# gt1/daccord

Hardware: AMD Instinct MI355X
Metric: corrected Mbase/s (whole node), synthetic 20x PacBio piles (higher is better)
Workload: dtype u64+f64; 1 GPU; BASELINE.json configs[1] (10k A-reads x 10 kb x 20x, k=14, one MI355X): synthetic 10000 A-reads x 10000 b x 20x, 15% error (ins 80/del 13.3/sub 6.7), k=14, w=40, a=10, tspace=100; piles_total=10000, piles_rank0=10000, overlaps_rank0=319252, windows_rank0=9969965, trace_blocks_rank0=17906701, corrected_bases_total=90715992

## Files before the change

### daccord_amd/_structs.py

```python
import ctypes as C

U64MAX = 0xFFFFFFFFFFFFFFFF


class DaccParams(C.Structure):
    _fields_ = [
        ("w", C.c_uint32), ("a", C.c_uint32), ("klow", C.c_uint32), ("khigh", C.c_uint32),
        ("minfilterfreq", C.c_int32), ("maxfilterfreq", C.c_int32), ("minwindowcov", C.c_uint32),
        ("maxalign", C.c_uint64), ("eminrate", C.c_uint64), ("minlen", C.c_uint64),
        ("producefull", C.c_int32), ("tspace", C.c_int32), ("device", C.c_int32), ("verbose", C.c_int32),
    ]


class DaccOverlap(C.Structure):
    _fields_ = [
        ("aread", C.c_int32), ("bread", C.c_int32), ("flags", C.c_uint32),
        ("abpos", C.c_int32), ("aepos", C.c_int32), ("bbpos", C.c_int32), ("bepos", C.c_int32),
        ("diffs", C.c_int32), ("tlen", C.c_int32), ("reserved", C.c_uint32), ("trace_off", C.c_uint64),
    ]


class DaccPile(C.Structure):
    _fields_ = [("aread", C.c_int32), ("novl", C.c_uint32), ("first_ovl", C.c_uint64)]


class DaccFragment(C.Structure):
    _fields_ = [("aread", C.c_int32), ("first", C.c_uint32), ("last", C.c_uint32), ("len", C.c_uint32),
                ("seq_off", C.c_uint64)]


class DaccTiming(C.Structure):
    _fields_ = [("h2d_ms", C.c_float), ("trace_ms", C.c_float), ("window_ms", C.c_float), ("vote_ms", C.c_float),
                ("d2h_ms", C.c_float), ("total_ms", C.c_float), ("nwindows", C.c_uint64), ("nblocks", C.c_uint64),
                ("algo_bytes", C.c_uint64), ("tier_ms", C.c_float * 3), ("tier_out", C.c_uint32 * 3),
                ("first_tier", C.c_uint32), ("long_windows", C.c_uint32), ("tier0_ms", C.c_float), ("tier0_in", C.c_uint32),
                ("tier0_out", C.c_uint32), ("tier7_ms", C.c_float), ("tier7_in", C.c_uint32), ("tier7_out", C.c_uint32), ("pad_", C.c_uint32),
                ("long_first_tier", C.c_uint32), ("tier10_ms", C.c_float), ("tier10_out", C.c_uint32), ("tier10_ran", C.c_uint32), ("pad2_", C.c_uint32),
                ("deep_ms", C.c_float), ("deep_windows", C.c_uint32), ("deep_out", C.c_uint32), ("pad3_", C.c_uint32),
                ("last_ms", C.c_float), ("last_windows", C.c_uint32), ("last_out", C.c_uint32), ("pad4_", C.c_uint32),
                ("vdeep_ms", C.c_float), ("vdeep_windows", C.c_uint32), ("vdeep_out", C.c_uint32), ("pad5_", C.c_uint32)]


TIMING_SIZE_V1 = 128


class DaccWindowResult(C.Structure):
    _fields_ = [("pile", C.c_int32), ("y", C.c_int32), ("status", C.c_int32), ("mao", C.c_int32),
                ("elength", C.c_int32), ("k", C.c_int32), ("filterfreq", C.c_int32), ("conslen", C.c_int32),
                ("minrate", C.c_uint64), ("cons", C.c_char * 80)]


def default_params(**kw):
    p = DaccParams(w=40, a=10, klow=8, khigh=8, minfilterfreq=0, maxfilterfreq=2, minwindowcov=3,
                   maxalign=U64MAX, eminrate=U64MAX, minlen=0, producefull=0, tspace=100, device=0, verbose=0)
    for k, v in kw.items():
        if k == "k":
            p.klow = p.khigh = v
        else:
            setattr(p, k, v)
    return p
```

### daccord_amd/csrc/capi.hip

```cpp
#include <hip/hip_runtime.h>
#include <vector>
#include <string>
#include <cstring>
#include <cstdio>
#include <cstdlib>
#include <new>
#include "../../include/daccord_hip.h"
#include "batch_plan.hpp"
#include "host_tables.hpp"
#include "window_kernels.hpp"
#include "trace_kernel.hpp"
#include "vote_kernel.hpp"

using namespace dacc;


struct PrepBatch
{
	DevOvl const * ovl; uint64_t novl; uint8_t const * trace; uint32_t trace_bytes;
	uint32_t * blk_ovl; uint32_t * blk_b0;
};

__global__ void k_prep(PrepBatch B)
{
	uint64_t const o = static_cast<uint64_t>(blockIdx.x)*blockDim.x + threadIdx.x;
	if ( o >= B.novl ) return;
	DevOvl const ov = B.ovl[o];
	uint32_t b = ov.bbpos;
	for ( int32_t i = 0; i < ov.nblk; ++i )
	{
		B.blk_ovl[ov.blk0+i] = o; B.blk_b0[ov.blk0+i] = b;
		b += B.trace_bytes == 2 ? reinterpret_cast<uint16_t const *>(B.trace)[ov.trace_off+2*i+1] : B.trace[ov.trace_off+2*i+1];
	}
}

__global__ void __launch_bounds__(64) k_trace(TraceBatch B)
{
	extern __shared__ __attribute__((aligned(16))) uint8_t lds_trace[];
	TraceStoreGL st;
	st.g = B.slab + static_cast<size_t>(blockIdx.x)*traceSlabWords(B.maxcols);
	st.w = (LDSQ uint32_t *)lds_trace; st.lane = threadIdx.x;
	if ( B.work )
	{
		while ( true )
		{
			uint32_t b = 0;
			if ( threadIdx.x == 0 ) b = atomicAdd(B.work,64u);
			b = __builtin_amdgcn_readfirstlane(b);
			if ( b >= B.nblocks ) break;
			uint64_t const task = static_cast<uint64_t>(b) + threadIdx.x;
			if ( task < B.nblocks ) traceBlock(B,task,st);
		}
		return;
	}
	for ( uint64_t task = static_cast<uint64_t>(blockIdx.x)*64 + threadIdx.x; task < B.nblocks; task += static_cast<uint64_t>(gridDim.x)*64 )
		traceBlock(B,task,st);
}

template<int NW>
__global__ void __launch_bounds__(64) k_trace_wide(TraceBatch B, uint32_t const nl)
{
	extern __shared__ __attribute__((aligned(16))) uint8_t lds_trace[];
	uint32_t const slots = traceSlots(B.maxcols);
	TraceStoreW<NW> st;
	st.w = (LDSQ uint64_t *)lds_trace; st.sc = (LDSQ uint16_t *)(lds_trace + static_cast<size_t>(slots)*(2*NW)*nl*8); st.lane = threadIdx.x; st.nl = nl;
	if ( threadIdx.x < nl )
		for ( uint64_t task = static_cast<uint64_t>(blockIdx.x)*nl + threadIdx.x; task < B.nblocks; task += static_cast<uint64_t>(gridDim.x)*nl )
			traceBlockWide<NW>(B,task,st);
}

static inline uint32_t boundByArena(uint64_t grid, uint64_t const bytes, uint64_t const mingrid)
{
	uint64_t const budget = 32ull << 30;
	while ( grid > mingrid && grid*bytes > budget ) grid >>= 1;
	return static_cast<uint32_t>(grid < 1 ? 1 : grid);
}

__global__ void __launch_bounds__(256) k_prescan(DevOvl const * ovl, uint64_t novl, uint32_t const * ovl_pile, DevPile const * piles, uint32_t const * wt_b, uint32_t const * wt_e,
	uint32_t * pregen, uint32_t * pregen2, uint32_t const thr1)
{
	uint64_t const o = static_cast<uint64_t>(blockIdx.x)*4 + (threadIdx.x>>6);
	if ( o >= novl ) return;
	DevOvl const ov = ovl[o];
	uint64_t const winbase = piles[ovl_pile[o]].winbase;
	for ( uint32_t r = threadIdx.x & 63; r < ov.ny; r += 64 )
	{
		uint32_t const len = wt_e[ov.wtoff+r] - wt_b[ov.wtoff+r];
		if ( len > thr1 )
		{
			uint64_t const w = winbase + ov.y0 + r;
			uint32_t const bit = 1u << (w&31);
			atomicOr(pregen + (w>>5),bit);
			if ( len > 128u ) atomicOr(pregen2 + (w>>5),bit);
		}
	}
}
__global__ void __launch_bounds__(256) k_prescan_lists(uint32_t const * pregen, uint32_t const * pregen2, uint64_t nwindows, uint32_t * list128, uint32_t * slot1list, WindowOut * wout)
{
	uint64_t const wi = static_cast<uint64_t>(blockIdx.x)*256 + threadIdx.x;
	if ( wi*32 >= nwindows ) return;
	uint32_t m = pregen[wi]; uint32_t const m2 = pregen2[wi];
	while ( m )
	{
		uint32_t const b = static_cast<uint32_t>(__builtin_ctz(m)); m &= m-1;
		uint64_t const w = wi*32 + b;
		if ( w >= nwindows ) break;
		wout[w].status = WS_INSUFFICIENT;
		uint32_t * const dst = ((m2 >> b) & 1u) || !slot1list ? list128 : slot1list;
		uint32_t const q = atomicAdd(dst,1u); dst[1+q] = static_cast<uint32_t>(w);
	}
}

__global__ void k_check_done(WindowOut const * wout, uint64_t n, uint32_t * errflag, DevPile const * piles, uint32_t npiles, uint8_t * pilebad)
{
	uint64_t const i = static_cast<uint64_t>(blockIdx.x)*blockDim.x + threadIdx.x;
	if ( i >= n ) return;
	uint32_t const st = wout[i].status;
	if ( st == WS_RETRY ) atomicOr(errflag,1u);
	if ( st == WS_OVERFLOW )
	{
		uint32_t lo = 0, hi = npiles;
		while ( hi-lo > 1 ) { uint32_t const mid = (lo+hi)>>1; if ( piles[mid].winbase <= i ) lo = mid; else hi = mid; }
		pilebad[lo] = 1;
	}
}

__global__ void k_count_deeper(uint32_t const * in, uint32_t const * handon, WindowOut const * wout, uint32_t const mins, uint32_t * out)
{
	uint32_t const nin = in[0], nout = handon[0];
	uint32_t a = 0, b = 0;
	for ( uint32_t i = blockIdx.x*blockDim.x + threadIdx.x; i < nin; i += gridDim.x*blockDim.x ) a += static_cast<uint32_t>(wout[in[1+i]].mao) > mins;
	for ( uint32_t i = blockIdx.x*blockDim.x + threadIdx.x; i < nout; i += gridDim.x*blockDim.x ) b += static_cast<uint32_t>(wout[handon[1+i]].mao) > mins;
	if ( a ) atomicAdd(out,a);
	if ( b ) atomicAdd(out+1,b);
}
__global__ void k_collect_overflow(WindowOut const * wout, uint64_t n, uint32_t * list)
{
	uint64_t const i = static_cast<uint64_t>(blockIdx.x)*blockDim.x + threadIdx.x;
	if ( i < n && wout[i].status == WS_OVERFLOW ) { uint32_t const q = atomicAdd(list,1u); list[1+q] = static_cast<uint32_t>(i); }
}

template<bool MAXOP>
__device__ __forceinline__ uint32_t block_scan_excl(uint32_t const v, uint32_t * part4, uint32_t & total)
{
	uint32_t const wave = threadIdx.x >> 6;
	uint32_t x = v;
	if ( MAXOP ) { DACC_DPP_SCAN(x,DACC_OP_MAX,0u) } else { DACC_DPP_SCAN(x,DACC_OP_ADD,0u) }
	uint32_t excl = __shfl_up(x,1,64); if ( (threadIdx.x & 63) == 0 ) excl = 0;
	__syncthreads();
	if ( (threadIdx.x & 63) == 63 ) part4[wave] = x;
	__syncthreads();
	uint32_t base = 0, tot = 0;
	#pragma unroll
	for ( uint32_t i = 0; i < 4; ++i )
	{
		uint32_t const t = part4[i];
		if ( i < wave ) base = MAXOP ? (t > base ? t : base) : (base + t);
		tot = MAXOP ? (t > tot ? t : tot) : (tot + t);
	}
	total = tot;
	return MAXOP ? (excl > base ? excl : base) : (base + excl);
}

__global__ void __launch_bounds__(256) k_classify(WindowBatch B, uint32_t * small, uint32_t * mid, uint32_t * big, uint32_t const t0inst, uint32_t const t7inst)
{
	__shared__ uint32_t part4[4]; __shared__ uint32_t base3[3];
	uint64_t const w = static_cast<uint64_t>(blockIdx.x)*256 + threadIdx.x;
	uint32_t cls = 3;
	if ( w < B.nwindows && !(B.pregen && ((B.pregen[w>>5] >> (w&31)) & 1)) )
	{
		cls = classifyWindow(B,w,t0inst,t7inst);
		B.wout[w].status = WS_INSUFFICIENT;
	}
	uint32_t tot0, tot1, tot2;
	uint32_t const p0 = block_scan_excl<false>(cls == 0 ? 1u : 0u,part4,tot0);
	__syncthreads();
	uint32_t const p1 = block_scan_excl<false>(cls == 1 ? 1u : 0u,part4,tot1);
	__syncthreads();
	uint32_t const p2 = block_scan_excl<false>(cls == 2 ? 1u : 0u,part4,tot2);
	if ( threadIdx.x == 0 ) { base3[0] = tot0 ? atomicAdd(small,tot0) : 0u; base3[1] = tot1 ? atomicAdd(big,tot1) : 0u; base3[2] = tot2 ? atomicAdd(mid,tot2) : 0u; }
	__syncthreads();
	if ( cls == 0 ) small[1+base3[0]+p0] = static_cast<uint32_t>(w);
	if ( cls == 1 ) big[1+base3[1]+p1] = static_cast<uint32_t>(w);
	if ( cls == 2 ) mid[1+base3[2]+p2] = static_cast<uint32_t>(w);
}


enum { VOTE_STAGE = 48 };
__device__ __forceinline__ VoteTile vote_stage(VoteBatch const & B, DevPile const & pile, uint32_t const p0, uint32_t const np, uint8_t * lds)
{
	VoteTile VT; VT.stage = (LDSQ uint8_t const *)lds; VT.y0 = 0; VT.n = 0;
	uint32_t const a = B.P.a, w = B.P.w, nwin = pile.nwin;
	if ( ! nwin ) return VT;
	uint32_t const plast = (p0+255 < np) ? (p0+255) : (np-1);
	uint32_t const ylo = (p0 > w) ? ((p0-w + a-1)/a) : 0;
	uint32_t yhi = plast / a; if ( yhi > nwin-1 ) yhi = nwin-1;
	__syncthreads();
	if ( ylo <= yhi && yhi-ylo+1 <= VOTE_STAGE && !DACC_WIDE_W(w) )
	{
		VT.y0 = ylo; VT.n = yhi-ylo+1;
		uint4 const * src = reinterpret_cast<uint4 const *>(B.wrec + (pile.winbase+ylo)*WREC);
		uint4 * dst = reinterpret_cast<uint4 *>(lds);
		for ( uint32_t i = threadIdx.x; i < VT.n*(WREC/16); i += 256 ) dst[i] = src[i];
	}
	__syncthreads();
	return VT;
}
__global__ void __launch_bounds__(256) k_vote(VoteBatch B)
{
	__shared__ uint32_t part4[4];
	__shared__ __attribute__((aligned(16))) uint8_t stage[VOTE_STAGE*WREC];
	uint32_t const pi = blockIdx.x;
	DevPile const pile = B.piles[pi];
	uint32_t const np = pileNpos(pile);
	uint32_t const tid = threadIdx.x;
	if ( B.pilebad && B.pilebad[pi] ) { if ( tid == 0 ) B.nfrag[pi] = 0; return; }
	for ( uint32_t t0 = 0; t0 < np; t0 += 256 )
	{
		VoteTile const VT = vote_stage(B,pile,t0,np,stage);
		if ( t0+tid < np ) votePass1(B,pile,t0+tid,VT);
	}
	__syncthreads();
	uint32_t run0 = 0;
	for ( uint32_t t0 = 0; t0 < np; t0 += 256 )
	{
		VoteTile const VT = vote_stage(B,pile,t0,np,stage);
		uint32_t const p = t0+tid;
		uint32_t const n = p < np ? votePass2(B,pile,p,0,VT) : 0u;
		uint32_t tot; uint32_t const ex = block_scan_excl<false>(n,part4,tot);
		if ( p < np ) { B.oc[pile.posbase+p] = n; B.ocs[pile.posbase+p] = run0 + ex; }
		run0 += tot;
	}
	uint32_t const total = run0;
	bool const fits = total <= 2*np+64;
	if ( !fits && tid == 0 ) atomicOr(B.errflag,2u);
	uint64_t const symbase = 2*pile.posbase + 64ull*pi;
	if ( fits )
		for ( uint32_t t0 = 0; t0 < np; t0 += 256 )
		{
			VoteTile const VT = vote_stage(B,pile,t0,np,stage);
			uint32_t const p = t0+tid;
			if ( p < np ) votePass2(B,pile,p,B.outsym+symbase+B.ocs[pile.posbase+p],VT);
		}
	__syncthreads();
	uint32_t const chunk = (np + 255)/256;
	uint32_t const p0 = tid*chunk < np ? tid*chunk : np, p1 = (p0+chunk < np) ? (p0+chunk) : np;
	uint8_t const * has = B.has + pile.posbase;
	uint32_t laststart = 0; bool open = false;
	for ( uint32_t p = p0; p < p1; ++p )
		if ( has[p] && (p == 0 || !has[p-1]) ) laststart = p+1;
	uint32_t dummy;
	uint32_t const instart = block_scan_excl<true>(laststart,part4,dummy);
	(void)open;
	uint32_t cur = instart;
	uint32_t nfr = 0;
	for ( int pass = 0; pass < 2; ++pass )
	{
		uint32_t fbase = 0, ftot = 0;
		if ( pass == 1 ) { fbase = block_scan_excl<false>(nfr,part4,ftot); if ( tid == 0 ) B.nfrag[pi] = fits ? ftot : 0; if ( !fits ) break; }
		cur = instart; uint32_t k = 0;
		VoteFragment * F = B.frags + B.fragbase[pi];
		for ( uint32_t p = p0; p < p1; ++p )
		{
			if ( ! has[p] ) continue;
			if ( p == 0 || !has[p-1] ) cur = p+1;
			if ( p+1 == np || !has[p+1] )
			{
				uint32_t const first = cur-1, q = p;
				if ( q-first >= 100 )
				{
					uint32_t const so = B.ocs[pile.posbase+first];
					uint32_t const eo = B.ocs[pile.posbase+q] + B.oc[pile.posbase+q];
					uint32_t const len = eo-so;
					if ( B.P.producefull || len >= B.P.minlen )
					{
						if ( pass == 1 ) { VoteFragment & f = F[fbase+k]; f.first = first; f.last = q; f.len = len; f.pad = 0; f.off = symbase + so; }
						++k;
					}
				}
			}
		}
		nfr = k;
	}
}


namespace {

template<typename T>
struct DevBuf
{
	T * p; size_t cap;
	DevBuf() : p(0), cap(0) {}
	hipError_t ensure(size_t n)
	{
		if ( n <= cap ) return hipSuccess;
		if ( p ) { hipFree(p); p = 0; cap = 0; }
		hipError_t const e = hipMalloc(reinterpret_cast<void **>(&p),n*sizeof(T));
		if ( e == hipSuccess ) cap = n;
		return e;
	}
	void release() { if ( p ) hipFree(p); p = 0; cap = 0; }
};

template<typename T>
struct HostBuf
{
	T * p; size_t cap; bool pinned;
	HostBuf() : p(0), cap(0), pinned(false) {}
	hipError_t ensure(size_t n)
	{
		if ( n <= cap ) return hipSuccess;
		release();
		hipError_t e = hipHostMalloc(reinterpret_cast<void **>(&p),n*sizeof(T),hipHostMallocDefault);
		if ( e == hipSuccess ) { cap = n; pinned = true; return e; }
		(void)hipGetLastError();
		p = static_cast<T *>(std::malloc(n*sizeof(T)));
		if ( !p ) return hipErrorOutOfMemory;
		cap = n; pinned = false;
		return hipSuccess;
	}
	void release() { if ( p ) { if ( pinned ) hipHostFree(p); else std::free(p); } p = 0; cap = 0; pinned = false; }
};

}

struct dacc_ctx
{
	dacc_params par;
	int device;
	hipStream_t stream; hipStream_t stream2; hipEvent_t evFirstTier, evEarlyGeneric, evPrescan;
	hipEvent_t ev[6]; hipEvent_t evslot[TIER_NSLOTS];
	std::string err;
	bool haveprofile, havedb, havebatch;
	double est_cor;
	HostTables H;
	DevTables T; DevParams P;
	DevBuf<double> d_dpnorm, d_dpsq; DevBuf<uint64_t> d_vs; DevBuf<uint16_t> d_first, d_size, d_suplo, d_suphi; DevBuf<uint32_t> d_klim;
	DevBuf<uint8_t> d_bps; DevBuf<uint64_t> d_boff; DevBuf<uint32_t> d_rlen;
	std::vector<uint32_t> h_rlen;
	BatchPlan BP;
	DevBuf<DevPile> d_piles; DevBuf<DevOvl> d_ovl; DevBuf<uint32_t> d_ovl_pile; DevBuf<uint8_t> d_trace;
	DevBuf<uint32_t> d_blk_ovl, d_blk_b0, d_wt_b, d_wt_e;
	DevBuf<uint8_t> d_wrec; DevBuf<WindowOut> d_wout; DevBuf<uint8_t> d_arena;
	DevBuf<uint8_t> d_has, d_oc, d_outsym, d_pilebad; DevBuf<uint16_t> d_ld0; DevBuf<uint32_t> d_ocs, d_nfrag, d_err;
	DevBuf<VoteFragment> d_frags; DevBuf<uint64_t> d_fragbase; DevBuf<uint64_t> d_prof;
	DevBuf<uint64_t> d_vst; DevBuf<uint32_t> d_tab32; DevBuf<uint8_t> d_gslab, d_lastslab , d_vdeepslab ; DevBuf<uint32_t> d_retry[TIER_NSLOTS], d_work, d_gearly, d_pregen, d_pregen2, d_pregenlist; DevBuf<uint8_t> d_arena2; DevBuf<uint64_t> d_trslab; DevBuf<uint32_t> d_small; DevBuf<uint64_t> d_hand; DevBuf<uint32_t> d_handctr; uint32_t handcap; uint64_t handwant, nruns; bool nohand, oom; bool tier7_adapt_off; int env_t7adapt; int env_trdyn;
	TierSwitches sw; TierPipeline TP;
	struct Stage { bool ran; uint32_t grid; DevBuf<uint32_t> handon; hipEvent_t done; uint32_t const * in;  } st[TIER_NSTAGES];
	uint32_t nlong[2];
	uint32_t retry_grid, early_grid; int sched;
	uint32_t tr_grid, tr_lds, tr_words, tr_lanes, trace_bytes, win_grid;
	int env_sched, env_dbgretry;
	std::vector<uint32_t> retry_flags;
	std::vector<dacc_fragment> frags; std::string bases;
	std::vector<int32_t> pile_status; std::vector<std::string> pile_errors; std::string pile_errors_joined;
	std::vector<uint32_t> h_nfrag; std::vector<VoteFragment> h_frags; HostBuf<uint8_t> h_outsym;
	dacc_timing timing;
};

#define HIPCHK(call) do { hipError_t const e_ = (call); if ( e_ != hipSuccess ) { c->err = std::string(#call) + ": " + hipGetErrorString(e_); if ( e_ == hipErrorOutOfMemory ) c->oom = true; return DACC_EHIP; } } while (0)

template<typename T>
static int upload(dacc_ctx * c, DevBuf<T> & b, T const * src, size_t n)
{
	HIPCHK(b.ensure(n ? n : 1));
	if ( n ) HIPCHK(hipMemcpyAsync(b.p,src,n*sizeof(T),hipMemcpyHostToDevice,c->stream));
	return DACC_OK;
}

template<typename F> static int guarded(dacc_ctx * c, F const & f)
{
	try { return f(); }
	catch ( std::bad_alloc const & ) { if ( c ) { try { c->err = "out of host memory"; } catch ( ... ) {} } return DACC_ENOMEM; }
	catch ( std::exception const & ex ) { if ( c ) { try { c->err = std::string("host side failed: ") + ex.what(); } catch ( ... ) {} } return DACC_EINTERNAL; }
	catch ( ... ) { if ( c ) { try { c->err = "host side failed: unknown exception"; } catch ( ... ) {} } return DACC_EINTERNAL; }
}

extern "C" {

int dacc_device_count(void)
{
	int ndev = 0;
	if ( hipGetDeviceCount(&ndev) != hipSuccess || ndev < 0 ) return 0;
	return ndev;
}

int dacc_create(dacc_ctx ** out, dacc_params const * p)
{
	if ( !out || !p ) return DACC_EINVAL;
	*out = 0;
	if ( p->klow < 3 || p->khigh > 16 || p->klow > p->khigh || !p->w || !p->a || p->w > DACC_WMAX || p->minfilterfreq < 0 ||
	     p->maxfilterfreq < p->minfilterfreq || p->tspace <= 0 || p->tspace > 512 )
		return DACC_EINVAL;
	if ( readTierSwitches().conflict() ) return DACC_EINVAL;
	int ndev = 0;
	if ( hipGetDeviceCount(&ndev) != hipSuccess || ndev <= 0 || p->device < 0 || p->device >= ndev )
		return DACC_ENODEV;
	if ( hipSetDevice(p->device) != hipSuccess ) return DACC_ENODEV;
	dacc_ctx * c = new (std::nothrow) dacc_ctx;
	if ( !c ) return DACC_ENOMEM;
	c->par = *p; c->device = p->device; c->haveprofile = c->havedb = c->havebatch = false; c->est_cor = 0; c->nlong[0] = c->nlong[1] = 0; c->handcap = 0; c->handwant = 0; c->nruns = 0; c->nohand = false; c->oom = false;
	std::memset(&c->timing,0,sizeof(c->timing));
	c->retry_grid = c->early_grid = c->win_grid = 0; c->tier7_adapt_off = false; c->sched = 0;
	c->tr_grid = c->tr_lds = c->tr_words = c->tr_lanes = c->trace_bytes = 0;
	{
		c->sw = readTierSwitches();
		char const * sc = getenv("DACC_SCHED"); c->env_sched = sc ? atoi(sc) : 1;
		{ char const * td = getenv("DACC_TRACE_DYN"); c->env_trdyn = !(td && td[0] == '0'); }
		char const * ta = getenv("DACC_T7_ADAPT"); c->env_t7adapt = !(ta && ta[0] == '0');
		char const * dr = getenv("DACC_DEBUG_RETRY"); c->env_dbgretry = (dr && dr[0] == '1');
	}
	if ( hipStreamCreate(&c->stream) != hipSuccess ) { delete c; return DACC_EHIP; }
	{ int lo = 0, hi = 0; hipDeviceGetStreamPriorityRange(&lo,&hi); if ( hipStreamCreateWithPriority(&c->stream2,hipStreamNonBlocking,hi) != hipSuccess ) { delete c; return DACC_EHIP; } }
	hipEventCreateWithFlags(&c->evFirstTier,hipEventDisableTiming); hipEventCreateWithFlags(&c->evEarlyGeneric,hipEventDisableTiming); hipEventCreateWithFlags(&c->evPrescan,hipEventDisableTiming);
	for ( int i = 0; i < 6; ++i ) hipEventCreate(&c->ev[i]);
	for ( int i = 0; i < TIER_NSLOTS; ++i ) hipEventCreate(&c->evslot[i]);
	for ( int i = 0; i < TIER_NSTAGES; ++i ) { hipEventCreate(&c->st[i].done); c->st[i].ran = false; c->st[i].grid = 0; c->st[i].in = 0; }
	*out = c;
	return DACC_OK;
}

void dacc_destroy(dacc_ctx * c)
{
	if ( !c ) return;
	hipSetDevice(c->device);
	hipStreamSynchronize(c->stream); hipStreamSynchronize(c->stream2);
	c->d_dpnorm.release(); c->d_dpsq.release(); c->d_vs.release(); c->d_first.release(); c->d_size.release(); c->d_suplo.release(); c->d_suphi.release(); c->d_klim.release();
	c->d_bps.release(); c->d_boff.release(); c->d_rlen.release();
	c->d_piles.release(); c->d_ovl.release(); c->d_ovl_pile.release(); c->d_trace.release(); c->d_blk_ovl.release(); c->d_blk_b0.release(); c->d_wt_b.release(); c->d_wt_e.release();
	c->d_wrec.release(); c->d_wout.release(); c->d_arena.release();
	c->h_outsym.release(); c->d_pilebad.release(); c->d_has.release(); c->d_oc.release(); c->d_outsym.release(); c->d_ld0.release(); c->d_ocs.release(); c->d_nfrag.release(); c->d_err.release(); c->d_frags.release(); c->d_fragbase.release(); c->d_prof.release(); c->d_vst.release(); c->d_tab32.release(); c->d_gslab.release(); c->d_lastslab.release(); c->d_vdeepslab.release(); for ( int i = 0; i < 3; ++i ) c->d_retry[i].release(); c->d_work.release(); c->d_gearly.release(); c->d_pregen.release(); c->d_pregen2.release(); c->d_pregenlist.release(); c->d_arena2.release(); c->d_trslab.release(); c->d_hand.release(); c->d_handctr.release();
	for ( int i = 0; i < 6; ++i ) hipEventDestroy(c->ev[i]);
	hipStreamDestroy(c->stream); hipStreamDestroy(c->stream2); hipEventDestroy(c->evFirstTier); hipEventDestroy(c->evEarlyGeneric); hipEventDestroy(c->evPrescan); for ( int i = 0; i < TIER_NSLOTS; ++i ) hipEventDestroy(c->evslot[i]);
	c->d_small.release(); for ( int i = 0; i < TIER_NSTAGES; ++i ) { hipEventDestroy(c->st[i].done); c->st[i].handon.release(); }
	delete c;
}

char const * dacc_last_error(dacc_ctx * c) { return c ? c->err.c_str() : "null context"; }

static int dacc_set_error_profile_body(dacc_ctx * c, double p_i, double p_d, double est_cor)
{
	if ( !c ) return DACC_EINVAL;
	if ( !(p_i >= 0 && p_i < 1 && p_d >= 0 && p_d < 1 && est_cor >= 0 && est_cor <= 1) ) { c->err = "error profile out of range"; return DACC_EINVAL; }
	hipSetDevice(c->device);
	buildHostTables(c->H,c->par.w,p_i,p_d,est_cor,c->par.klow,c->par.khigh,4200);
	c->est_cor = est_cor;
	int rc;
	if ( (rc = upload(c,c->d_dpnorm,c->H.dpnorm.data(),c->H.dpnorm.size())) ) return rc;
	if ( (rc = upload(c,c->d_dpsq,c->H.dpsq.data(),c->H.dpsq.size())) ) return rc;
	if ( (rc = upload(c,c->d_vs,c->H.dpsq_vs.data(),c->H.dpsq_vs.size())) ) return rc;
	if ( (rc = upload(c,c->d_vst,c->H.dpsq_vst.data(),c->H.dpsq_vst.size())) ) return rc;
	if ( (rc = upload(c,c->d_tab32,c->H.tab32.data(),c->H.tab32.size())) ) return rc;
	if ( (rc = upload(c,c->d_first,c->H.dpsq_first.data(),c->H.dpsq_first.size())) ) return rc;
	if ( (rc = upload(c,c->d_size,c->H.dpsq_size.data(),c->H.dpsq_size.size())) ) return rc;
	if ( (rc = upload(c,c->d_suplo,c->H.suplo.data(),c->H.suplo.size())) ) return rc;
	if ( (rc = upload(c,c->d_suphi,c->H.suphi.data(),c->H.suphi.size())) ) return rc;
	if ( (rc = upload(c,c->d_klim,c->H.klim.data(),c->H.klim.size())) ) return rc;
	HIPCHK(hipStreamSynchronize(c->stream));
	DevTables & T = c->T;
	T.nrows = c->H.nrows; T.nsup = c->H.nsup; T.kln = c->H.kln; T.pad = 0;
	T.dpnorm = c->d_dpnorm.p; T.dpsq = c->d_dpsq.p; T.dpsq_vs = c->d_vs.p; T.dpsq_first = c->d_first.p; T.dpsq_size = c->d_size.p;
	T.suplo = c->d_suplo.p; T.suphi = c->d_suphi.p; T.klim = c->d_klim.p;
	dacc_params const & p = c->par;
	DevParams & P = c->P;
	P.w = p.w; P.a = p.a; P.klow = p.klow; P.khigh = p.khigh; P.minff = p.minfilterfreq; P.maxff = p.maxfilterfreq;
	P.minwindowcov = p.minwindowcov; P.checklim = (est_cor != 0.0); P.maxalign = p.maxalign; P.eminrate = p.eminrate;
	P.tspace = p.tspace; P.producefull = p.producefull; P.minlen = p.minlen;
	c->haveprofile = true;
	return DACC_OK;
}

int dacc_debug_tables(dacc_ctx * c, uint64_t * out, uint64_t cap, uint64_t * n, uint64_t klimit_n)
{
	if ( !c || !n ) return DACC_EINVAL;
	if ( !c->haveprofile ) return DACC_ESTATE;
	std::vector<uint64_t> B; serialiseHostTables(c->H,B,klimit_n);
	*n = B.size();
	if ( out ) std::memcpy(out,B.data(),8*std::min<uint64_t>(cap,B.size()));
	return DACC_OK;
}

static int dacc_load_db_body(dacc_ctx * c, uint8_t const * bps, uint64_t bps_bytes, uint64_t const * boff, uint32_t const * rlen, uint64_t nreads)
{
	if ( !c || !bps || !boff || !rlen || !nreads ) return DACC_EINVAL;
	hipSetDevice(c->device);
	for ( uint64_t i = 0; i < nreads; ++i )
		if ( boff[i] + (rlen[i]+3)/4 > bps_bytes ) { c->err = "read store offsets exceed the buffer"; return DACC_EINVAL; }
	int rc;
	HIPCHK(c->d_bps.ensure(bps_bytes+16));
	HIPCHK(hipMemsetAsync(c->d_bps.p,0,bps_bytes+16,c->stream));
	HIPCHK(hipMemcpyAsync(c->d_bps.p,bps,bps_bytes,hipMemcpyHostToDevice,c->stream));
	if ( (rc = upload(c,c->d_boff,boff,nreads)) ) return rc;
	if ( (rc = upload(c,c->d_rlen,rlen,nreads)) ) return rc;
	HIPCHK(hipStreamSynchronize(c->stream));
	c->h_rlen.assign(rlen,rlen+nreads);
	c->havedb = true;
	return DACC_OK;
}

static int runDevice(dacc_ctx * c)
{
	BatchPlan & BP = c->BP; TierPipeline & TP = c->TP;
	hipStream_t const s = c->stream;
	static bool const dbgsync = getenv("DACC_DEBUG_SYNC") && getenv("DACC_DEBUG_SYNC")[0] == '1';
	auto const mark = [&](char const * what) { if ( dbgsync ) { hipError_t const e = hipStreamSynchronize(s); std::fprintf(stderr,"[dacc] %s: %s\n",what,hipGetErrorString(e)); std::fflush(stderr); } };
	if ( c->nruns && c->handwant > c->handcap && !c->nohand )
	{
		uint64_t cap = c->handwant;
		{ size_t fr = 0, tot = 0; if ( hipMemGetInfo(&fr,&tot) == hipSuccess ) { uint64_t const lim = (static_cast<uint64_t>(fr)/2) / (static_cast<uint64_t>(c->TP.handwords)*8ull); if ( cap > lim ) cap = lim; } else (void)hipGetLastError(); }
		while ( cap && c->d_hand.ensure(static_cast<size_t>(cap)*c->TP.handwords) != hipSuccess ) { (void)hipGetLastError(); cap = cap > 65536 ? cap/2 : 0; }
		c->handcap = static_cast<uint32_t>(cap); c->handwant = cap;
	}
	++c->nruns;
	HIPCHK(hipMemsetAsync(c->d_err.p,0,4*sizeof(uint32_t),s));
	HIPCHK(hipEventRecord(c->ev[0],s));
	if ( BP.ovl.size() )
	{
		PrepBatch PB; PB.ovl = c->d_ovl.p; PB.novl = BP.ovl.size(); PB.trace = c->d_trace.p; PB.trace_bytes = c->trace_bytes; PB.blk_ovl = c->d_blk_ovl.p; PB.blk_b0 = c->d_blk_b0.p;
		hipLaunchKernelGGL(k_prep,dim3((BP.ovl.size()+255)/256),dim3(256),0,s,PB);
	}
	if ( BP.nblocks )
	{
		TraceBatch TB;
		TB.P = c->P; TB.bps = c->d_bps.p; TB.boff = c->d_boff.p; TB.rlen = c->d_rlen.p;
		TB.piles = c->d_piles.p; TB.ovl = c->d_ovl.p; TB.ovl_pile = c->d_ovl_pile.p; TB.trace = c->d_trace.p;
		TB.blk_ovl = c->d_blk_ovl.p; TB.blk_b0 = c->d_blk_b0.p; TB.nblocks = BP.nblocks; TB.wt_b = c->d_wt_b.p; TB.wt_e = c->d_wt_e.p;
		TB.maxcols = BP.maxcols; TB.trace_bytes = c->trace_bytes; TB.errflag = c->d_err.p + 2; TB.slab = c->d_trslab.p;
		TB.work = (c->env_trdyn && BP.nblocks < 0xFFFFFF00ull) ? c->d_work.p + WORK_TRACE : static_cast<uint32_t *>(0);
		if ( TB.work ) HIPCHK(hipMemsetAsync(TB.work,0,sizeof(uint32_t),s));
		if ( c->tr_words == 2 ) hipLaunchKernelGGL(k_trace,dim3(c->tr_grid),dim3(64),c->tr_lds,s,TB);
		else if ( c->tr_words == 4 ) hipLaunchKernelGGL(k_trace_wide<4>,dim3(c->tr_grid),dim3(64),c->tr_lds,s,TB,c->tr_lanes);
		else hipLaunchKernelGGL(k_trace_wide<8>,dim3(c->tr_grid),dim3(64),c->tr_lds,s,TB,c->tr_lanes);
	}
	mark("prep + trace");
	HIPCHK(hipEventRecord(c->ev[1],s));
	if ( BP.nwindows )
	{
		WindowBatch WB;
		WB.P = c->P; WB.T = c->T; WB.C = BP.caps; WB.bps = c->d_bps.p; WB.boff = c->d_boff.p; WB.rlen = c->d_rlen.p;
		WB.piles = c->d_piles.p; WB.npiles = BP.piles.size(); WB.ovl = c->d_ovl.p; WB.wt_b = c->d_wt_b.p; WB.wt_e = c->d_wt_e.p;
		WB.nwindows = BP.nwindows; WB.wrec = c->d_wrec.p; WB.wout = c->d_wout.p; WB.arena = c->d_arena.p; WB.prof = c->d_prof.p;
		WB.pregen = 0;
		for ( uint32_t i = 0; i < TIER_NSTAGES; ++i ) c->st[i].ran = false;
		if ( TP.usefast && TP.anytier() )
		{
			HIPCHK(hipMemsetAsync(c->d_pregen.p,0,((BP.nwindows+31)/32+1)*sizeof(uint32_t),s));
			HIPCHK(hipMemsetAsync(c->d_pregen2.p,0,((BP.nwindows+31)/32+1)*sizeof(uint32_t),s));
			HIPCHK(hipMemsetAsync(c->d_pregenlist.p,0,sizeof(uint32_t),s));
			for ( int i = 0; i < TIER_NSLOTS; ++i ) HIPCHK(hipMemsetAsync(c->d_retry[i].p,0,sizeof(uint32_t),s));
			if ( BP.ovl.size() )
			{
				hipLaunchKernelGGL(k_prescan,dim3((BP.ovl.size()+3)/4),dim3(256),0,s,c->d_ovl.p,static_cast<uint64_t>(BP.ovl.size()),c->d_ovl_pile.p,c->d_piles.p,c->d_wt_b.p,c->d_wt_e.p,c->d_pregen.p,c->d_pregen2.p,TP.widetier ? 128u : 64u);
				hipLaunchKernelGGL(k_prescan_lists,dim3(((BP.nwindows+31)/32+255)/256),dim3(256),0,s,c->d_pregen.p,c->d_pregen2.p,static_cast<uint64_t>(BP.nwindows),c->d_pregenlist.p,
					TP.slot1_long ? c->d_retry[0].p : static_cast<uint32_t *>(0),c->d_wout.p);
			}
			HIPCHK(hipEventRecord(c->evPrescan,s));
			FastBatch FL; FL.W = WB; FL.W.arena = c->d_arena2.p; FL.W.prof = 0; FL.W.pregen = 0; FL.F = BP.ftierL; FL.dpsq_vst = c->d_vst.p; FL.retry = 0; FL.gearly = 0; FL.gslab = 0; FL.gstride = 0; FL.tab32 = c->d_tab32.p; FL.hand = 0; FL.handctr = 0; FL.handcap = 0; FL.handwords = 0;
#if defined(DACC_LEDGER)
			FL.ledger = 0;
#endif
			if ( !TP.ok[ID_LONG] ) FL.F.ldsbytes = 0;
			auto const launchLong = [&](uint32_t const * const lst, uint32_t & nlist, hipEvent_t const filled) -> int
			{
				nlist = 0;
				HIPCHK(hipStreamWaitEvent(c->stream2,filled,0));
				HIPCHK(hipMemcpyAsync(&nlist,lst,sizeof(uint32_t),hipMemcpyDeviceToHost,c->stream2));
				HIPCHK(hipStreamSynchronize(c->stream2));
				if ( !nlist ) return DACC_OK;
				uint32_t const grid = nlist < c->early_grid ? nlist : c->early_grid;
				(void)hipGetLastError();
				hipLaunchKernelGGL(k_window_long,dim3(grid),dim3(64),FL.F.ldsbytes,c->stream2,FL,c->d_err.p,lst);
				if ( FL.F.ldsbytes && hipGetLastError() != hipSuccess )
				{
					TP.ok[ID_LONG] = false; FL.F.ldsbytes = 0;
					hipLaunchKernelGGL(k_window_long,dim3(grid),dim3(64),0,c->stream2,FL,c->d_err.p,lst);
				}
				return DACC_OK;
			};
			c->nlong[0] = c->nlong[1] = 0;
			WB.pregen = c->d_pregen.p;
			HIPCHK(hipMemsetAsync(c->d_gearly.p,0,sizeof(uint32_t),s));
			HIPCHK(hipMemsetAsync(c->d_handctr.p,0,sizeof(uint32_t),s));
			bool early = false;
			HIPCHK(hipMemsetAsync(c->d_work.p,0,WORK_WORDS*sizeof(uint32_t),s));
			auto const work = [&](uint32_t const off) { return (c->sched&1) ? c->d_work.p+off : static_cast<uint32_t *>(0); };
			uint32_t const * list = 0; int lastslot = -1;
			FastBatch FZ;
			for ( uint32_t slot = 0; slot < TIER_NSLOTS; ++slot )
			{
				if ( TP.slotok(slot) )
				{
					int const m = TIER_MAIN[slot];
					FastBatch FB; FB.W = WB; FB.F = BP.stageCaps(m); FB.dpsq_vst = c->d_vst.p; FB.retry = c->d_retry[slot].p;
					if ( (slot > 0 && TP.late_long) || TP.widetier ) FB.W.pregen = c->d_pregen2.p;
					FB.gslab = c->d_gslab.p; FB.gstride = FB.F.gbytes; FB.tab32 = c->d_tab32.p;
					FB.hand = c->handcap ? c->d_hand.p : static_cast<uint64_t *>(0); FB.handctr = c->d_handctr.p; FB.handcap = c->handcap; FB.handwords = TP.handwords;
#if defined(DACC_LEDGER)
					{ char const * lm = getenv("DACC_LEDGER_MASK"); FB.ledger = lm ? static_cast<uint32_t>(strtoul(lm,0,0)) : 0u; }
#endif
					FB.gearly = early ? static_cast<uint32_t *>(0) : c->d_gearly.p;
					int fr[TIER_NSTAGES]; uint32_t nfr = 0;
					for ( int i = 0; i < m; ++i ) if ( TIER_CHAIN[i].slot == slot && TP.ok[i] && !((TIER_CHAIN[i].flags & STAGE_ADAPTIVE) && c->tier7_adapt_off) ) fr[nfr++] = i;
					bool const classed = nfr && (TIER_CHAIN[fr[0]].flags & STAGE_PREPASS);
					if ( classed ) HIPCHK(hipMemsetAsync(c->d_small.p,0,sizeof(uint32_t),s));
					for ( uint32_t k = 0; k < nfr; ++k ) HIPCHK(hipMemsetAsync(c->st[fr[k]].handon.p,0,sizeof(uint32_t),s));
					uint32_t const * in = list;
					if ( classed )
					{
						uint32_t * const mid = c->st[fr[0]].handon.p, * const big = c->st[fr[nfr-1]].handon.p;
						hipLaunchKernelGGL(k_classify,dim3((BP.nwindows+255)/256),dim3(256),0,s,WB,c->d_small.p,mid,big,c->sw.t0inst,nfr > 1 ? c->sw.t7inst : 0u);
						if ( nfr > 1 ) { HIPCHK(hipMemcpyAsync(c->d_work.p+WORK_PRE_MID,mid,sizeof(uint32_t),hipMemcpyDeviceToDevice,s)); HIPCHK(hipMemcpyAsync(c->d_work.p+WORK_PRE_BIG,big,sizeof(uint32_t),hipMemcpyDeviceToDevice,s)); }
						in = c->d_small.p;
					}
					for ( uint32_t k = 0; k < nfr; ++k )
					{
						dacc_ctx::Stage & S = c->st[fr[k]];
						FastBatch FF = FB; FF.F = BP.stageCaps(fr[k]); FF.retry = S.handon.p; FF.gstride = FF.F.gbytes;
						hipLaunchKernelGGL(fastKernel(TP.tier[fr[k]]),dim3(S.grid),dim3(64),FF.F.gmem ? 0u : FF.F.ldsbytes,s,FF,in,work(TIER_CHAIN[fr[k]].work));
						HIPCHK(hipEventRecord(S.done,s)); S.ran = true; S.in = in;
						in = S.handon.p;
					}
					hipLaunchKernelGGL(fastKernel(TP.tier[m]),dim3(c->st[m].grid),dim3(64),FB.F.gmem ? 0u : FB.F.ldsbytes,s,FB,in,work(TIER_CHAIN[m].work));
					list = c->d_retry[slot].p; lastslot = static_cast<int>(slot);
					if ( !early )
					{
						early = true;
						HIPCHK(hipEventRecord(c->evFirstTier,s));
					}
					FZ = FB;
				}
				hipEventRecord(c->evslot[slot],s);
			}
			uint32_t const * const slotlist = list;
			if ( TP.ok[ID_LAST] && list && lastslot >= 0 )
			{
				dacc_ctx::Stage & S = c->st[ID_LAST];
				FZ.F = BP.stageCaps(ID_LAST); FZ.retry = S.handon.p; FZ.gearly = 0; FZ.gslab = c->d_lastslab.p; FZ.gstride = FZ.F.gbytes;
				FZ.W.pregen = (TP.late_long || TP.widetier) ? c->d_pregen2.p : c->d_pregen.p;
				HIPCHK(hipMemsetAsync(S.handon.p,0,sizeof(uint32_t),s));
				hipLaunchKernelGGL(fastKernel(TP.tier[ID_LAST]),dim3(S.grid),dim3(64),0,s,FZ,list,work(TIER_CHAIN[ID_LAST].work));
				HIPCHK(hipEventRecord(S.done,s)); S.ran = true; S.in = list;
				list = S.handon.p;
			}
			if ( TP.ok[ID_VDEEP] && list && lastslot >= 0 )
			{
				dacc_ctx::Stage & S = c->st[ID_VDEEP];
				FZ.F = BP.stageCaps(ID_VDEEP); FZ.retry = S.handon.p; FZ.gearly = 0; FZ.gslab = c->d_vdeepslab.p; FZ.gstride = FZ.F.gbytes;
				FZ.W.pregen = (TP.late_long || TP.widetier) ? c->d_pregen2.p : c->d_pregen.p;
				HIPCHK(hipMemsetAsync(S.handon.p,0,sizeof(uint32_t),s));
				hipLaunchKernelGGL(fastKernel(TP.tier[ID_VDEEP]),dim3(S.grid),dim3(64),0,s,FZ,list,work(TIER_CHAIN[ID_VDEEP].work));
				HIPCHK(hipEventRecord(S.done,s)); S.ran = true; S.in = list;
				list = S.handon.p;
			}
			if ( c->env_dbgretry && slotlist )
			{
				uint32_t const * const list = slotlist;
				HIPCHK(hipStreamSynchronize(s));
				uint32_t n = 0; HIPCHK(hipMemcpy(&n,list,sizeof(uint32_t),hipMemcpyDeviceToHost));
				std::vector<uint32_t> idx(n); if ( n ) HIPCHK(hipMemcpy(idx.data(),list+1,n*sizeof(uint32_t),hipMemcpyDeviceToHost));
				c->retry_flags.clear();
				for ( uint32_t i = 0; i < n; ++i ) { WindowOut o; HIPCHK(hipMemcpy(&o,c->d_wout.p+idx[i],sizeof(WindowOut),hipMemcpyDeviceToHost)); c->retry_flags.push_back(idx[i]); c->retry_flags.push_back(o.flags); c->retry_flags.push_back(o.mao); c->retry_flags.push_back(static_cast<uint32_t>(o.filterfreq)); }
			}
			hipLaunchKernelGGL(k_window,dim3(c->retry_grid),dim3(64),0,s,WB,c->d_err.p,list,(c->sched&2) ? c->d_work.p+WORK_GENERIC : static_cast<uint32_t *>(0));
			{ int const rc = launchLong(static_cast<uint32_t const *>(c->d_pregenlist.p),c->nlong[0],c->evPrescan); if ( rc ) return rc; }
			if ( early ) { int const rc = launchLong(static_cast<uint32_t const *>(c->d_gearly.p),c->nlong[1],c->evFirstTier); if ( rc ) return rc; }
			HIPCHK(hipEventRecord(c->evEarlyGeneric,c->stream2));
			HIPCHK(hipStreamWaitEvent(s,c->evEarlyGeneric,0));
		}
		else
			{ HIPCHK(hipMemsetAsync(c->d_work.p,0,WORK_WORDS*sizeof(uint32_t),s)); hipLaunchKernelGGL(k_window,dim3(c->win_grid),dim3(64),0,s,WB,c->d_err.p,static_cast<uint32_t const *>(0),(c->sched&2) ? c->d_work.p+WORK_GENERIC : static_cast<uint32_t *>(0)); mark("k_window (all windows)"); }
	}
	HIPCHK(hipEventRecord(c->ev[2],s));
	uint32_t herr[4] = {0,0,0,0};
	size_t const symbytes = 2*BP.npos + 64*BP.piles.size() + 64;
	c->h_nfrag.resize(BP.piles.size()); c->h_frags.resize(BP.nfragslots+1); HIPCHK(c->h_outsym.ensure(symbytes));
	auto voteAndFetch = [&]() -> int
	{
		HIPCHK(hipMemsetAsync(c->d_pilebad.p,0,BP.piles.size()+1,s));
		if ( BP.nwindows ) hipLaunchKernelGGL(k_check_done,dim3((BP.nwindows+255)/256),dim3(256),0,s,c->d_wout.p,BP.nwindows,c->d_err.p+3,c->d_piles.p,static_cast<uint32_t>(BP.piles.size()),c->d_pilebad.p);
		if ( BP.piles.size() )
		{
			VoteBatch VB;
			VB.P = c->P; VB.bps = c->d_bps.p; VB.boff = c->d_boff.p; VB.rlen = c->d_rlen.p; VB.piles = c->d_piles.p; VB.npiles = BP.piles.size();
			VB.wrec = c->d_wrec.p; VB.has = c->d_has.p; VB.ld0 = c->d_ld0.p; VB.oc = c->d_oc.p; VB.ocs = c->d_ocs.p; VB.outsym = c->d_outsym.p;
			VB.frags = c->d_frags.p; VB.fragbase = c->d_fragbase.p; VB.nfrag = c->d_nfrag.p; VB.errflag = c->d_err.p + 1; VB.pilebad = c->d_pilebad.p;
			mark("k_check_done");
			hipLaunchKernelGGL(k_vote,dim3(BP.piles.size()),dim3(256),0,s,VB);
			mark("k_vote");
		}
		HIPCHK(hipEventRecord(c->ev[3],s));
		HIPCHK(hipGetLastError());
		HIPCHK(hipMemcpyAsync(herr,c->d_err.p,sizeof(herr),hipMemcpyDeviceToHost,s));
		if ( BP.piles.size() )
		{
			HIPCHK(hipMemcpyAsync(c->h_nfrag.data(),c->d_nfrag.p,BP.piles.size()*sizeof(uint32_t),hipMemcpyDeviceToHost,s));
			HIPCHK(hipMemcpyAsync(c->h_frags.data(),c->d_frags.p,BP.nfragslots*sizeof(VoteFragment),hipMemcpyDeviceToHost,s));
			HIPCHK(hipMemcpyAsync(c->h_outsym.p,c->d_outsym.p,symbytes,hipMemcpyDeviceToHost,s));
		}
		HIPCHK(hipEventRecord(c->ev[4],s));
		HIPCHK(hipStreamSynchronize(s));
		return DACC_OK;
	};
	{ int const rc = voteAndFetch(); if ( rc ) return rc; }
	auto const ranOf = [&](TierId const id) { return c->st[id].ran ? &c->st[id] : static_cast<dacc_ctx::Stage *>(0); };
	dacc_ctx::Stage * const f0 = ranOf(ID_T0), * const f7 = ranOf(ID_T7), * const fD = ranOf(ID_DENSE), * const fX = ranOf(ID_DEEP);
	for ( int i = 0; i < 3; ++i ) c->timing.tier_out[i] = 0;
	if ( TP.usefast && BP.nwindows ) for ( int i = 0; i < 3; ++i ) if ( TP.slotok(i) ) HIPCHK(hipMemcpy(&c->timing.tier_out[i],c->d_retry[i].p,sizeof(uint32_t),hipMemcpyDeviceToHost));
	c->timing.tier10_out = 0;
	if ( fD ) HIPCHK(hipMemcpy(&c->timing.tier10_out,fD->handon.p,sizeof(uint32_t),hipMemcpyDeviceToHost));
	c->timing.tier0_in = 0; c->timing.tier0_out = 0; c->timing.tier7_in = 0; c->timing.tier7_out = 0;
	if ( TP.usefast && BP.nwindows && TP.anytier() )
	{
		uint32_t const n1 = c->nlong[0], n2 = c->nlong[1];
		c->timing.long_windows = n1 + n2; c->timing.long_first_tier = n2;
		if ( f0 )
		{
			uint32_t nsmall = 0, nbig = 0, nmid = 0;
			HIPCHK(hipMemcpy(&nsmall,c->d_small.p,sizeof(uint32_t),hipMemcpyDeviceToHost)); HIPCHK(hipMemcpy(&nbig,(f7 ? f7 : f0)->handon.p,sizeof(uint32_t),hipMemcpyDeviceToHost));
			if ( f7 ) HIPCHK(hipMemcpy(&nmid,f0->handon.p,sizeof(uint32_t),hipMemcpyDeviceToHost));
			c->timing.tier0_in = nsmall;
			if ( !f7 )
			{
				uint64_t const big0 = BP.nwindows - std::min<uint64_t>(BP.nwindows,static_cast<uint64_t>(nsmall) + n1);
				c->timing.tier0_out = nbig > big0 ? static_cast<uint32_t>(nbig - big0) : 0u;
			}
			else
			{
				uint32_t pre[2] = {0,0};
				HIPCHK(hipMemcpy(pre,c->d_work.p+WORK_PRE_MID,2*sizeof(uint32_t),hipMemcpyDeviceToHost));
				uint32_t const t7out = nbig > pre[1] ? nbig - pre[1] : 0u;
				c->timing.tier0_out = nmid > pre[0] ? nmid - pre[0] : 0u;
				c->timing.tier7_in = nmid; c->timing.tier7_out = t7out;
				if ( c->env_t7adapt && nmid >= 4096 && static_cast<uint64_t>(t7out)*5 > nmid ) c->tier7_adapt_off = true;
			}
		}
	}
	for ( int attempt = 0; herr[0] && !herr[1] && !herr[2] && attempt < 3; ++attempt )
	{
		growArenaCaps(BP.caps,c->par.w);
		Arena Atmp; BP.caps.bytes = arena_carve(Atmp,0,BP.caps,c->par.w);
		uint32_t const g = boundByArena(c->retry_grid < 64 ? c->retry_grid : 64,BP.caps.bytes,4);
		c->retry_grid = g; c->win_grid = g; if ( c->early_grid > g ) c->early_grid = g;
		HIPCHK(c->d_arena.ensure(static_cast<size_t>(g)*BP.caps.bytes));
		if ( TP.usefast ) HIPCHK(c->d_arena2.ensure(static_cast<size_t>(c->early_grid)*BP.caps.bytes));
		HIPCHK(c->d_gearly.ensure(BP.nwindows+2)); HIPCHK(c->d_pregenlist.ensure(BP.nwindows+2)); HIPCHK(c->d_pregen.ensure((BP.nwindows+31)/32+2)); HIPCHK(c->d_pregen2.ensure((BP.nwindows+31)/32+2));
		HIPCHK(hipMemsetAsync(c->d_err.p,0,4*sizeof(uint32_t),s));
		HIPCHK(hipMemsetAsync(c->d_gearly.p,0,sizeof(uint32_t),s));
		hipLaunchKernelGGL(k_collect_overflow,dim3((BP.nwindows+255)/256),dim3(256),0,s,c->d_wout.p,BP.nwindows,c->d_gearly.p);
		mark("k_collect_overflow");
		if ( dbgsync ) std::fprintf(stderr,"[dacc] scratch retry %d: grid %u, arena %llu bytes per wavefront\n",attempt,g,static_cast<unsigned long long>(BP.caps.bytes));
		WindowBatch WB;
		WB.P = c->P; WB.T = c->T; WB.C = BP.caps; WB.bps = c->d_bps.p; WB.boff = c->d_boff.p; WB.rlen = c->d_rlen.p;
		WB.piles = c->d_piles.p; WB.npiles = BP.piles.size(); WB.ovl = c->d_ovl.p; WB.wt_b = c->d_wt_b.p; WB.wt_e = c->d_wt_e.p;
		WB.nwindows = BP.nwindows; WB.wrec = c->d_wrec.p; WB.wout = c->d_wout.p; WB.arena = c->d_arena.p; WB.prof = 0; WB.pregen = 0;
		hipLaunchKernelGGL(k_window,dim3(g),dim3(64),0,s,WB,c->d_err.p,static_cast<uint32_t const *>(c->d_gearly.p),static_cast<uint32_t *>(0));
		mark("k_window (scratch retry)");
		int const rc = voteAndFetch(); if ( rc ) return rc;
	}
	c->timing.deep_windows = 0; c->timing.deep_out = 0; c->timing.pad3_ = 0;
	c->timing.last_windows = 0; c->timing.last_out = 0; c->timing.pad4_ = 0;
	if ( dacc_ctx::Stage const * const fZ = ranOf(ID_LAST) )
	{
		uint32_t nin = 0, nout = 0;
		HIPCHK(hipMemcpy(&nin,fZ->in,sizeof(uint32_t),hipMemcpyDeviceToHost)); HIPCHK(hipMemcpy(&nout,fZ->handon.p,sizeof(uint32_t),hipMemcpyDeviceToHost));
		c->timing.last_out = nout; c->timing.last_windows = nin > nout ? nin - nout : 0u;
	}
	c->timing.vdeep_windows = 0; c->timing.vdeep_out = 0; c->timing.pad5_ = 0;
	if ( dacc_ctx::Stage const * const fV = ranOf(ID_VDEEP) )
	{
		HIPCHK(hipMemsetAsync(c->d_work.p+WORK_VDEEP_COUNT,0,2*sizeof(uint32_t),s));
		hipLaunchKernelGGL(k_count_deeper,dim3(64),dim3(256),0,s,fV->in,static_cast<uint32_t const *>(fV->handon.p),c->d_wout.p,static_cast<uint32_t>(VDEEP_MINS),c->d_work.p+WORK_VDEEP_COUNT);
		uint32_t cnt[2] = {0,0};
		HIPCHK(hipMemcpyAsync(cnt,c->d_work.p+WORK_VDEEP_COUNT,sizeof(cnt),hipMemcpyDeviceToHost,s));
		HIPCHK(hipStreamSynchronize(s));
		c->timing.vdeep_out = cnt[1]; c->timing.vdeep_windows = cnt[0] > cnt[1] ? cnt[0] - cnt[1] : 0u;
	}
	if ( fX && fX->in )
	{
		HIPCHK(hipMemsetAsync(c->d_work.p+WORK_DEEP_COUNT,0,2*sizeof(uint32_t),s));
		hipLaunchKernelGGL(k_count_deeper,dim3(64),dim3(256),0,s,fX->in,static_cast<uint32_t const *>(fX->handon.p),c->d_wout.p,static_cast<uint32_t>(FastTier<12>::mins),c->d_work.p+WORK_DEEP_COUNT);
		uint32_t cnt[2] = {0,0};
		HIPCHK(hipMemcpyAsync(cnt,c->d_work.p+WORK_DEEP_COUNT,sizeof(cnt),hipMemcpyDeviceToHost,s));
		HIPCHK(hipStreamSynchronize(s));
		c->timing.deep_out = cnt[1]; c->timing.deep_windows = cnt[0] > cnt[1] ? cnt[0] - cnt[1] : 0u;
	}
	c->pile_status = BP.pile_status; c->pile_errors = BP.pile_errors;
	if ( herr[0] && BP.piles.size() )
	{
		std::vector<uint8_t> bad(BP.piles.size());
		HIPCHK(hipMemcpy(bad.data(),c->d_pilebad.p,bad.size(),hipMemcpyDeviceToHost));
		for ( size_t pi = 0; pi < bad.size(); ++pi )
			if ( bad[pi] )
			{
				c->pile_status[pi] = DACC_ENOTSUP;
				if ( c->pile_errors.size() < 64 ) c->pile_errors.push_back("read " + std::to_string(BP.piles[pi].aread) + ": window kernel scratch capacity exceeded (depth / graph size), read skipped");
			}
	}
	if ( herr[3] ) { c->err = "internal error: a window was handed on between engines and never processed"; return DACC_EHIP; }
	if ( herr[1] ) { c->err = "vote kernel capacity exceeded"; return DACC_ENOTSUP; }
	if ( herr[2] ) { c->err = "trace kernel capacity exceeded (a tspace block longer than the column vectors or a B span beyond the column store)"; return DACC_ENOTSUP; }
	c->frags.clear(); c->bases.clear();
	uint64_t nbases = 0;
	for ( uint64_t pi = 0; pi < BP.piles.size(); ++pi )
		for ( uint32_t f = 0; f < c->h_nfrag[pi]; ++f ) nbases += c->h_frags[BP.fragbase[pi]+f].len;
	c->bases.reserve(nbases);
	for ( uint64_t pi = 0; pi < BP.piles.size(); ++pi )
		for ( uint32_t f = 0; f < c->h_nfrag[pi]; ++f )
		{
			VoteFragment const & F = c->h_frags[BP.fragbase[pi]+f];
			dacc_fragment g; g.aread = BP.piles[pi].aread; g.first = F.first; g.last = F.last; g.len = F.len; g.seq_off = c->bases.size();
			c->bases.append(reinterpret_cast<char const *>(c->h_outsym.p)+F.off,F.len);
			c->frags.push_back(g);
		}
	float ms = 0;
	hipEventElapsedTime(&ms,c->ev[0],c->ev[1]); c->timing.trace_ms = ms;
	hipEventElapsedTime(&ms,c->ev[1],c->ev[2]); c->timing.window_ms = ms;
	for ( int i = 0; i < 3; ++i ) c->timing.tier_ms[i] = 0;
	if ( TP.usefast && BP.nwindows ) for ( int i = 0; i < 3; ++i ) { hipEventElapsedTime(&ms,i ? c->evslot[i-1] : c->ev[1],c->evslot[i]); c->timing.tier_ms[i] = ms; }
	c->timing.tier0_ms = 0; c->timing.tier7_ms = 0; c->timing.pad_ = 0; c->timing.tier10_ms = 0; c->timing.tier10_ran = fD ? 1u : 0u;
	if ( f0 ) { hipEventElapsedTime(&ms,c->ev[1],f0->done); c->timing.tier0_ms = ms; }
	if ( f7 ) { hipEventElapsedTime(&ms,f0->done,f7->done); c->timing.tier7_ms = ms; }
	if ( fD ) { hipEventElapsedTime(&ms,c->evslot[1],fD->done); c->timing.tier10_ms = ms; }
	c->timing.deep_ms = 0; c->timing.last_ms = 0; c->timing.vdeep_ms = 0;
	if ( dacc_ctx::Stage const * const fZ = ranOf(ID_LAST) ) { hipEventElapsedTime(&ms,c->evslot[TIER_NSLOTS-1],fZ->done); c->timing.last_ms = ms; }
	if ( dacc_ctx::Stage const * const fV = ranOf(ID_VDEEP) ) { dacc_ctx::Stage const * const fZ = ranOf(ID_LAST); hipEventElapsedTime(&ms,fZ ? fZ->done : c->evslot[TIER_NSLOTS-1],fV->done); c->timing.vdeep_ms = ms; }
	if ( fX ) { hipEventElapsedTime(&ms,fD ? fD->done : c->evslot[1],fX->done); c->timing.deep_ms = ms; }
	hipEventElapsedTime(&ms,c->ev[2],c->ev[3]); c->timing.vote_ms = ms;
	hipEventElapsedTime(&ms,c->ev[3],c->ev[4]); c->timing.d2h_ms = ms;
	hipEventElapsedTime(&ms,c->ev[0],c->ev[3]); c->timing.total_ms = ms;
	c->timing.first_tier = (TP.usefast && BP.deep) ? 4u : 1u;
	c->timing.nwindows = BP.nwindows; c->timing.nblocks = BP.nblocks; c->timing.algo_bytes = BP.algo_bytes + nbases;
	return DACC_OK;
}

static int dacc_submit_piles_body(dacc_ctx * c, dacc_pile const * piles, uint64_t npiles, dacc_overlap const * ovl, uint64_t novl,
	void const * trace, uint64_t ntrace, int trace_bytes)
{
	if ( !c ) return DACC_EINVAL;
	if ( !c->haveprofile || !c->havedb ) { c->err = "dacc_set_error_profile and dacc_load_db must precede dacc_submit_piles"; return DACC_ESTATE; }
	if ( (npiles && !piles) || (novl && (!ovl || !trace)) ) return DACC_EINVAL;
	hipSetDevice(c->device);
	c->havebatch = false;
	BatchPlan & BP = c->BP;
	int rc = BP.plan(c->par,piles,npiles,ovl,novl,trace,ntrace,trace_bytes,c->h_rlen.data(),c->h_rlen.size(),c->err,c->H.nrows,c->H.nsup);
	if ( rc ) return rc;
	hipStream_t const s = c->stream;
	HIPCHK(c->d_err.ensure(4));
	HIPCHK(c->d_prof.ensure(DACC_PROFW*4096)); HIPCHK(hipMemsetAsync(c->d_prof.p,0,DACC_PROFW*4096*sizeof(uint64_t),s));
	HIPCHK(hipEventRecord(c->ev[5],s));
	if ( (rc = upload(c,c->d_piles,BP.piles.data(),BP.piles.size())) ) return rc;
	if ( (rc = upload(c,c->d_ovl,BP.ovl.data(),BP.ovl.size())) ) return rc;
	if ( (rc = upload(c,c->d_ovl_pile,BP.ovl_pile.data(),BP.ovl_pile.size())) ) return rc;
	if ( (rc = upload(c,c->d_trace,static_cast<uint8_t const *>(trace),ntrace*trace_bytes)) ) return rc;
	if ( (rc = upload(c,c->d_fragbase,BP.fragbase.data(),BP.fragbase.size())) ) return rc;
	HIPCHK(c->d_blk_ovl.ensure(BP.nblocks+1)); HIPCHK(c->d_blk_b0.ensure(BP.nblocks+1));
	HIPCHK(c->d_wt_b.ensure(BP.nwt+1)); HIPCHK(c->d_wt_e.ensure(BP.nwt+1));
	{
		c->trace_bytes = trace_bytes;
		c->tr_words = (c->par.tspace <= 128 && BP.maxcols <= 928) ? 2 : (c->par.tspace <= 256 ? 4 : 8);
		c->tr_lanes = 64;
		if ( c->tr_words == 2 ) c->tr_lds = TRACE2_LDS;
		else
		{
			uint32_t const perlane = c->tr_words == 4 ? traceWideBytesPerLane<4>(BP.maxcols) : traceWideBytesPerLane<8>(BP.maxcols);
			while ( c->tr_lanes > 8 && static_cast<uint64_t>(c->tr_lanes)*perlane > 160*1024 ) c->tr_lanes >>= 1;
			c->tr_lds = c->tr_lanes*perlane;
		}
		if ( c->tr_lds > 160*1024 ) { c->err = "a trace block spans too many B bases for the trace kernel's LDS column store"; return DACC_ENOTSUP; }
		if ( c->tr_lds > 64*1024 )
		{
			if ( c->tr_words == 2 ) HIPCHK(hipFuncSetAttribute(reinterpret_cast<const void *>(k_trace),hipFuncAttributeMaxDynamicSharedMemorySize,c->tr_lds));
			else if ( c->tr_words == 4 ) HIPCHK(hipFuncSetAttribute(reinterpret_cast<const void *>(k_trace_wide<4>),hipFuncAttributeMaxDynamicSharedMemorySize,c->tr_lds));
			else HIPCHK(hipFuncSetAttribute(reinterpret_cast<const void *>(k_trace_wide<8>),hipFuncAttributeMaxDynamicSharedMemorySize,c->tr_lds));
		}
		uint64_t percu = (160*1024) / ((((c->tr_lds ? c->tr_lds : 1) + 1279u)/1280u)*1280u); if ( percu > (c->tr_words == 2 ? 20u : 8u) ) percu = (c->tr_words == 2 ? 20u : 8u); if ( percu < 1 ) percu = 1;
		if ( char const * e = getenv("DACC_TR_PERCU") ) { uint64_t const v = strtoull(e,0,10); if ( v >= 1 && v <= 32 ) percu = v; }
		uint64_t g = (BP.nblocks+c->tr_lanes-1)/c->tr_lanes, gmax = 256*percu*(c->tr_words == 2 ? 1 : 4);
		if ( g > gmax ) g = gmax;
		if ( g < 1 ) g = 1;
		c->tr_grid = g;
		if ( c->tr_words == 2 )
		{
			uint64_t const slabbytes = static_cast<uint64_t>(traceSlabWords(BP.maxcols))*sizeof(uint64_t);
			while ( g > 256 && g*slabbytes > (192ull<<20) ) g -= 256;
			c->tr_grid = g;
			HIPCHK(c->d_trslab.ensure(static_cast<size_t>(g)*traceSlabWords(BP.maxcols)));
		}
	}
	Arena Atmp; BP.caps.bytes = arena_carve(Atmp,0,BP.caps,c->par.w);
	uint64_t wg = ((BP.nwindows+7)/8)*8;
	uint64_t const maxwg = 256*8;
	if ( wg > maxwg ) wg = maxwg;
	if ( wg < 8 ) wg = 8;
	c->sched = c->env_sched;
	bool fits32 = true;
	for ( size_t i = 0; i < c->H.dpsq_vst.size(); ++i ) if ( c->H.dpsq_vst[i] >> 32 ) fits32 = false;
	c->TP = resolveTiers(c->sw,!c->sw.nofast && fits32,BP.deep,BP.wide,c->H.nrows,c->H.nsup,c->par.w,[&](uint32_t const id) -> FastCaps & { return BP.stageCaps(id); },BP.maxstrings(c->par));
	TierPipeline const & TP = c->TP;
	if ( TP.usefast )
	{
		for ( int t = 0; t < TIER_NSLOTS; ++t ) HIPCHK(c->d_retry[t].ensure(BP.nwindows+2));
		for ( uint32_t i = 0; i < TIER_NSTAGES; ++i )
		{
			FastCaps const & F = BP.stageCaps(i);
			c->st[i].grid = F.gmem ? tierGridGmem(F.gbytes,BP.nwindows) : tierGrid(F.ldsbytes,BP.nwindows);
			if ( !TP.ok[i] || TIER_CHAIN[i].role == ROLE_LONG ) continue;
			if ( TIER_CHAIN[i].role == ROLE_LAST )
			{
				DevBuf<uint8_t> & slab = i == ID_VDEEP ? c->d_vdeepslab : c->d_lastslab;
				hipError_t e = c->st[i].handon.ensure(BP.nwindows+2);
				if ( e == hipSuccess ) e = slab.ensure(static_cast<size_t>(c->st[i].grid)*F.gbytes + 256);
				if ( e == hipErrorOutOfMemory ) { (void)hipGetLastError(); slab.release(); c->TP.ok[i] = false; }
				else HIPCHK(e);
				continue;
			}
			if ( TIER_CHAIN[i].role == ROLE_FRONT ) HIPCHK(c->st[i].handon.ensure(BP.nwindows+2));
			if ( TIER_CHAIN[i].flags & STAGE_PREPASS ) HIPCHK(c->d_small.ensure(BP.nwindows+2));
			if ( F.gbytes ) HIPCHK(c->d_gslab.ensure(static_cast<size_t>(c->st[i].grid)*F.gbytes + 256));
			if ( !F.gmem && F.ldsbytes > 64*1024 ) HIPCHK(hipFuncSetAttribute(reinterpret_cast<const void *>(fastKernel(TP.tier[i])),hipFuncAttributeMaxDynamicSharedMemorySize,F.ldsbytes));
		}
		{
			uint64_t cap = BP.nwindows/3 + 4096; uint64_t const maxcap = (16ull<<30) / (static_cast<uint64_t>(TP.handwords)*8ull);
			if ( cap > maxcap ) cap = maxcap;
			if ( c->par.klow != c->par.khigh ) cap = 0;
			if ( c->nohand ) cap = 0;
			if ( !TP.handover ) cap = 0;
			c->handwant = cap;
			HIPCHK(c->d_handctr.ensure(4));
			if ( c->d_hand.cap < static_cast<size_t>(cap)*TP.handwords ) c->handcap = static_cast<uint32_t>(c->d_hand.cap / TP.handwords);
			else c->handcap = static_cast<uint32_t>(cap);
		}
		if ( TP.ok[ID_LONG] && BP.ftierL.ldsbytes > 64*1024 ) HIPCHK(hipFuncSetAttribute(reinterpret_cast<const void *>(k_window_long),hipFuncAttributeMaxDynamicSharedMemorySize,BP.ftierL.ldsbytes));
		c->retry_grid = boundByArena(wg < 512 ? wg : 512,BP.caps.bytes,8);
		c->win_grid = c->retry_grid;
		c->early_grid = c->retry_grid < 256 ? c->retry_grid : 256;
		while ( c->early_grid > 16 && static_cast<uint64_t>(c->early_grid)*BP.caps.bytes > (8ull<<30) ) c->early_grid >>= 1;
		HIPCHK(c->d_gearly.ensure(BP.nwindows+2)); HIPCHK(c->d_pregenlist.ensure(BP.nwindows+2)); HIPCHK(c->d_pregen.ensure((BP.nwindows+31)/32+2)); HIPCHK(c->d_pregen2.ensure((BP.nwindows+31)/32+2));
		HIPCHK(c->d_arena2.ensure(static_cast<size_t>(c->early_grid)*BP.caps.bytes));
		HIPCHK(c->d_work.ensure(WORK_WORDS));
		HIPCHK(c->d_arena.ensure(static_cast<size_t>(c->retry_grid)*BP.caps.bytes));
	}
	else
	{
		c->win_grid = boundByArena(wg,BP.caps.bytes,8);
		c->retry_grid = c->win_grid; c->early_grid = 0;
		HIPCHK(c->d_work.ensure(WORK_WORDS));
		HIPCHK(c->d_arena.ensure(static_cast<size_t>(c->win_grid)*BP.caps.bytes));
	}
	HIPCHK(c->d_wrec.ensure((BP.nwindows+1)*static_cast<size_t>(DACC_WREC_OF(c->par.w)))); HIPCHK(c->d_wout.ensure(BP.nwindows+1));
	HIPCHK(c->d_has.ensure(BP.npos+1)); HIPCHK(c->d_oc.ensure(BP.npos+1)); HIPCHK(c->d_ld0.ensure(BP.npos+1)); HIPCHK(c->d_ocs.ensure(BP.npos+1));
	HIPCHK(c->d_outsym.ensure(2*BP.npos + 64*BP.piles.size() + 64));
	HIPCHK(c->d_nfrag.ensure(BP.piles.size()+1)); HIPCHK(c->d_frags.ensure(BP.nfragslots+1)); HIPCHK(c->d_pilebad.ensure(BP.piles.size()+1));
	hipEvent_t h2dend; hipEventCreate(&h2dend); hipEventRecord(h2dend,s);
	rc = runDevice(c);
	float ms = 0; hipEventElapsedTime(&ms,c->ev[5],h2dend); c->timing.h2d_ms = ms; hipEventDestroy(h2dend);
	if ( rc ) return rc;
	c->havebatch = true;
	return DACC_OK;
}

static int dacc_rerun_resident_body(dacc_ctx * c)
{
	if ( !c ) return DACC_EINVAL;
	if ( !c->havebatch ) { c->err = "no resident batch"; return DACC_ESTATE; }
	hipSetDevice(c->device);
	return runDevice(c);
}

int dacc_collect(dacc_ctx * c, dacc_fragment const ** frags, uint64_t * nfrags, char const ** bases, uint64_t * nbases)
{
	if ( !c || !frags || !nfrags || !bases || !nbases ) return DACC_EINVAL;
	if ( !c->havebatch ) return DACC_ESTATE;
	*frags = c->frags.data(); *nfrags = c->frags.size(); *bases = c->bases.data(); *nbases = c->bases.size();
	return DACC_OK;
}

void dacc_release(dacc_ctx * c) { if ( c ) { c->frags.clear(); c->bases.clear(); } }

static_assert(offsetof(dacc_timing,deep_ms) == DACC_TIMING_SIZE_V1,"dacc_last_timing fills the record in front of deep_ms");
static_assert(offsetof(dacc_timing,vdeep_ms) == 160 && sizeof(dacc_timing) == 176,"the very deep stage's fields are appended behind last_*");
int dacc_last_timing(dacc_ctx * c, dacc_timing * t)
{
	if ( !c || !t ) return DACC_EINVAL;
	std::memcpy(static_cast<void *>(t),&c->timing,DACC_TIMING_SIZE_V1);
	return DACC_OK;
}
int dacc_last_timing2(dacc_ctx * c, dacc_timing * t, size_t size)
{
	if ( !c || !t ) return DACC_EINVAL;
	std::memcpy(static_cast<void *>(t),&c->timing,size < sizeof(dacc_timing) ? size : sizeof(dacc_timing));
	return DACC_OK;
}

static int dacc_debug_profile_rows(dacc_ctx * c, uint64_t * out, int const from, int const n)
{
	if ( !c || !out ) return DACC_EINVAL;
	if ( !c->havebatch ) return DACC_ESTATE;
	hipSetDevice(c->device);
	{
		std::vector<uint64_t> H(DACC_PROFW*4096);
		HIPCHK(hipMemcpy(H.data(),c->d_prof.p,DACC_PROFW*4096*sizeof(uint64_t),hipMemcpyDeviceToHost));
		for ( int i = 0; i < n; ++i ) out[i] = 0;
		for ( int b = 0; b < 4096; ++b ) for ( int i = 0; i < n; ++i ) { uint64_t const v = H[DACC_PROFW*b+from+i]; if ( from+i == 29 ) out[i] = std::max(out[i],v); else out[i] += v; }
	}
	return DACC_OK;
}
int dacc_debug_profile(dacc_ctx * c, uint64_t * out32) { return dacc_debug_profile_rows(c,out32,0,32); }
int dacc_debug_profile_fine(dacc_ctx * c, uint64_t * out96) { return dacc_debug_profile_rows(c,out96,32,96); }

int dacc_debug_retry(dacc_ctx * c, uint32_t * out, uint64_t cap, uint64_t * n)
{
	if ( !c || !n ) return DACC_EINVAL;
	*n = c->retry_flags.size();
	if ( out ) std::memcpy(out,c->retry_flags.data(),sizeof(uint32_t)*std::min<uint64_t>(cap,c->retry_flags.size()));
	return DACC_OK;
}

int dacc_pile_status(dacc_ctx * c, int32_t * out, uint64_t cap, uint64_t * n)
{
	if ( !c || !n ) return DACC_EINVAL;
	*n = c->pile_status.size();
	if ( out ) std::memcpy(out,c->pile_status.data(),sizeof(int32_t)*std::min<uint64_t>(cap,c->pile_status.size()));
	return DACC_OK;
}
char const * dacc_pile_errors(dacc_ctx * c)
{
	if ( !c ) return "";
	c->pile_errors_joined.clear();
	for ( size_t i = 0; i < c->pile_errors.size(); ++i ) { c->pile_errors_joined += c->pile_errors[i]; c->pile_errors_joined += '\n'; }
	return c->pile_errors_joined.c_str();
}

int dacc_debug_windows(dacc_ctx * c, dacc_window_result * out, uint64_t cap, uint64_t * nwin)
{
	if ( !c || !nwin ) return DACC_EINVAL;
	if ( !c->havebatch ) return DACC_ESTATE;
	BatchPlan & BP = c->BP;
	*nwin = BP.nwindows;
	if ( !out ) return DACC_OK;
	hipSetDevice(c->device);
	size_t const wrecb = DACC_WREC_OF(c->par.w);
	std::vector<WindowOut> wout(BP.nwindows); std::vector<uint8_t> wrec(BP.nwindows*wrecb);
	if ( BP.nwindows )
	{
		HIPCHK(hipMemcpy(wout.data(),c->d_wout.p,BP.nwindows*sizeof(WindowOut),hipMemcpyDeviceToHost));
		HIPCHK(hipMemcpy(wrec.data(),c->d_wrec.p,BP.nwindows*wrecb,hipMemcpyDeviceToHost));
	}
	uint64_t i = 0;
	for ( uint64_t pi = 0; pi < BP.piles.size() && i < cap; ++pi )
		for ( uint32_t y = 0; y < BP.piles[pi].nwin && i < cap; ++y, ++i )
		{
			uint64_t const wdx = BP.piles[pi].winbase+y;
			WindowOut const & o = wout[wdx];
			dacc_window_result r; std::memset(&r,0,sizeof(r));
			r.pile = pi; r.y = y; r.status = o.status; r.mao = o.mao; r.elength = o.elength; r.k = o.k;
			r.filterfreq = (o.status == WS_OK) ? o.filterfreq : 0; r.conslen = o.conslen; r.minrate = o.minrate;
			if ( o.status == WS_OK )
			{
				uint8_t const * rec = wrec.data() + wdx*wrecb;
				uint32_t const w = c->P.w; bool const wide = DACC_WIDE_W(w);
				uint8_t const * sym = wide ? rec+2+2*(w+2) : rec+1+(w+2);
				uint32_t const nsym = wide ? (rec[2+2*(w+1)] | (static_cast<uint32_t>(rec[3+2*(w+1)])<<8)) : rec[1+(w+1)];
				uint32_t cl = 0;
				for ( uint32_t q = 0; q < nsym && cl < 79; ++q ) if ( sym[q] < 4 ) r.cons[cl++] = "ACGT"[sym[q]];
			}
			out[i] = r;
		}
	return DACC_OK;
}


int dacc_set_error_profile(dacc_ctx * c, double p_i, double p_d, double est_cor) { return guarded(c,[&]() { return dacc_set_error_profile_body(c,p_i,p_d,est_cor); }); }
int dacc_load_db(dacc_ctx * c, uint8_t const * bps, uint64_t bps_bytes, uint64_t const * boff, uint32_t const * rlen, uint64_t nreads) { return guarded(c,[&]() { return dacc_load_db_body(c,bps,bps_bytes,boff,rlen,nreads); }); }
int dacc_plan_only(dacc_params const * par, uint32_t const * rlen, uint64_t nreads, dacc_pile const * piles, uint64_t npiles, dacc_overlap const * ovl, uint64_t novl,
	void const * trace, uint64_t ntrace, int trace_bytes, uint64_t * nwindows, uint64_t * nblocks)
{
	if ( !par || !rlen || (!piles && npiles) ) return DACC_EINVAL;
	try
	{
		BatchPlan BP; std::string err;
		int const rc = BP.plan(*par,piles,npiles,ovl,novl,trace,ntrace,trace_bytes,rlen,nreads,err);
		if ( nwindows ) *nwindows = BP.nwindows;
		if ( nblocks ) *nblocks = BP.nblocks;
		return rc;
	}
	catch ( std::bad_alloc const & ) { return DACC_ENOMEM; }
	catch ( ... ) { return DACC_EINTERNAL; }
}

static bool dacc_drop_hand(dacc_ctx * c)
{
	if ( !c || !c->oom ) return false;
	c->oom = false;
	if ( !c->d_hand.p ) return false;
	(void)hipGetLastError(); hipSetDevice(c->device); (void)hipDeviceSynchronize(); (void)hipGetLastError();
	c->d_hand.release(); c->handcap = 0; c->handwant = 0; c->nohand = true;
	return true;
}
int dacc_submit_piles(dacc_ctx * c, dacc_pile const * piles, uint64_t npiles, dacc_overlap const * ovl, uint64_t novl, void const * trace, uint64_t ntrace, int trace_bytes)
{
	if ( c ) c->oom = false;
	int rc = guarded(c,[&]() { return dacc_submit_piles_body(c,piles,npiles,ovl,novl,trace,ntrace,trace_bytes); });
	if ( rc == DACC_EHIP && dacc_drop_hand(c) ) rc = guarded(c,[&]() { return dacc_submit_piles_body(c,piles,npiles,ovl,novl,trace,ntrace,trace_bytes); });
	return rc;
}
int dacc_rerun_resident(dacc_ctx * c)
{
	if ( c ) c->oom = false;
	int rc = guarded(c,[&]() { return dacc_rerun_resident_body(c); });
	if ( rc == DACC_EHIP && dacc_drop_hand(c) ) rc = guarded(c,[&]() { return dacc_rerun_resident_body(c); });
	return rc;
}

}
```

### daccord_amd/csrc/daccord_hip_main.cpp

```cpp
#include <cstdio>
#include <cstdlib>
#include <cstring>
#include <cmath>
#include <cstdint>
#include <string>
#include <vector>
#include <algorithm>
#include <fstream>
#include <sstream>
#include <iostream>
#include <thread>
#include <mutex>
#include <condition_variable>
#include <deque>
#include <chrono>
#include <sys/stat.h>
#include <unistd.h>
#include "../../include/daccord_hip.h"
#include "../../include/daccord_io.h"

namespace {

struct Options
{
// ... 162 lines not shown

	Db A, B2; openDb(o.pos[1],A);
	bool const twodb = o.pos.size() > 2;
	if ( twodb && o.vard ) die("vard option is not supported for asymmetric (DB1 != DB2) alignments");
	std::vector<uint8_t> bps; std::vector<uint64_t> boff; std::vector<uint32_t> rlen;
	uint64_t nA = 0;
	if ( twodb )
	{
		openDb(o.pos[2],B2);
		bps.assign(A.bps,A.bps+A.nbytes); bps.insert(bps.end(),B2.bps,B2.bps+B2.nbytes);
		boff.assign(A.boff,A.boff+A.n); for ( uint64_t i = 0; i < B2.n; ++i ) boff.push_back(B2.boff[i]+A.nbytes);
		rlen.assign(A.rlen,A.rlen+A.n); rlen.insert(rlen.end(),B2.rlen,B2.rlen+B2.n);
		nA = A.n;
	}
	uint8_t const * const pbps = twodb ? bps.data() : A.bps; uint64_t const nbps = twodb ? bps.size() : A.nbytes;
	uint64_t const * const pboff = twodb ? boff.data() : A.boff; uint32_t const * const prlen = twodb ? rlen.data() : A.rlen;
	uint64_t const nreads = twodb ? rlen.size() : A.n;
	Db const & DB2 = twodb ? B2 : A;
	uint64_t tot = 0; for ( uint64_t i = 0; i < DB2.n; ++i ) tot += DB2.rlen[i];
	uint64_t const avgrl = DB2.n ? tot/DB2.n : 0;

	int64_t minaread = 0, toparead = 0;
	{
		char ebuf[256]; ebuf[0] = 0;
		if ( dacc_read_interval(lasmin,lasmax,o.haveJ ? o.Jtext.c_str() : 0,o.haveI ? o.Itext.c_str() : 0,&minaread,&toparead,ebuf,sizeof(ebuf)) ) die(ebuf);
	}
	int64_t const maxaread = toparead - 1;
	if ( o.V ) std::fprintf(stderr,"[V] minaread=%lld toparead=%lld\n",static_cast<long long>(minaread),static_cast<long long>(toparead));

	if ( novl && lasmax >= static_cast<int64_t>(A.n) )
		die("A read id " + std::to_string(lasmax) + " of " + lasfn + " is beyond the " + std::to_string(A.n) + " reads of " + o.pos[1] + ": the .las does not belong to this database");
	if ( o.vard && !avgrl ) die("--vard needs a database with reads (average read length is zero)");
	uint64_t const nB = twodb ? B2.n : A.n;

	struct Batch { std::vector<dacc_overlap> sel; std::vector<dacc_pile> spiles; std::vector<uint8_t> trace; uint64_t ntrace = 0; bool end = false; std::string err; uint64_t seq = 0; };
	std::vector<dacc_overlap> tmp;
	auto loadBatch = [&](int64_t const b0, int64_t const b1, bool const lowest, Batch & B) -> void
	{
		dacc_pile const * piles = 0; uint64_t npiles = 0; dacc_overlap const * ovl = 0; uint64_t no = 0; void const * trace = 0; uint64_t ntrace = 0;
		B.sel.clear(); B.spiles.clear(); B.trace.clear(); B.ntrace = 0; B.err.clear();
		if ( dacc_las_piles(las,b0,b1,&piles,&npiles,&ovl,&no,&trace,&ntrace) ) { B.err = std::string("las: ") + dacc_las_error(las); return; }
		for ( uint64_t z = 0; z < no; ++z )
			if ( static_cast<uint64_t>(ovl[z].bread) >= nB )
			{ B.err = "B read id " + std::to_string(ovl[z].bread) + " (A read " + std::to_string(ovl[z].aread) + ") is beyond the " + std::to_string(nB) + " reads of the database"; return; }
		for ( uint64_t i = 0; i < npiles; ++i )
		{
			uint64_t const rl = prlen[piles[i].aread];
			uint64_t const lmaxinput = o.vard ? std::max<uint64_t>(std::max<uint64_t>(2*o.vard,1),
				static_cast<uint64_t>((2.0*static_cast<double>(o.vard)*static_cast<double>(rl)/static_cast<double>(avgrl))+0.5)) : o.D;
			tmp.resize(std::max<uint64_t>(piles[i].novl,1)); uint64_t nout = 0;
			int const rc = lowest ? dacc_pile_select_lowest(ovl+piles[i].first_ovl,piles[i].novl,tbytes,lmaxinput,tmp.data(),&nout)
			                      : dacc_pile_select(ovl+piles[i].first_ovl,piles[i].novl,tbytes,lmaxinput,tmp.data(),&nout);
			if ( rc ) { B.err = "pile selection failed"; return; }
			dacc_pile q; q.aread = piles[i].aread; q.novl = nout; q.first_ovl = B.sel.size();
			for ( uint64_t z = 0; z < nout; ++z ) { dacc_overlap v = tmp[z]; v.bread += nA; B.sel.push_back(v); }
			B.spiles.push_back(q);
		}
		B.trace.assign(static_cast<uint8_t const *>(trace),static_cast<uint8_t const *>(trace) + ntrace*static_cast<uint64_t>(tbytes));
		B.ntrace = ntrace;
	};

	double prof[3] = {0,0,0};
	std::string const eproffn = o.E.empty() ? (lasfn + ".eprof") : o.E;
	bool have = false;
	if ( !o.eprof.empty() )
	{
		std::string s = o.eprof; for ( size_t i = 0; i < s.size(); ++i ) if ( s[i] == ',' ) s[i] = ' ';
		std::istringstream is(s); if ( !(is >> prof[0] >> prof[1] >> prof[2]) ) die("--eprof needs three numbers: p_i,p_d,est_cor");
		have = true;
	}
	else
	{
		struct stat se, sl;
		bool const exists = ::stat(eproffn.c_str(),&se) == 0;
		bool const older = exists && ::stat(lasfn.c_str(),&sl) == 0 &&
			( se.st_mtim.tv_sec < sl.st_mtim.tv_sec || (se.st_mtim.tv_sec == sl.st_mtim.tv_sec && se.st_mtim.tv_nsec < sl.st_mtim.tv_nsec) );
		if ( exists && !(older && !o.keepeprof) )
		{
			bool bin = false;
			if ( !readProfile(eproffn,prof,&bin) ) die("cannot parse the error profile " + eproffn + " (three numbers p_i p_d est_cor as text, or the reference's 48-byte binary profile)");
			if ( o.V ) std::fprintf(stderr,"[V] error profile %s read (%s)\n",eproffn.c_str(),bin ? "reference binary form" : "text");
			have = true;
		}
	}
	if ( o.deepprofileonly )
	{
		int64_t const top = std::min<int64_t>(toparead,minaread+4096);
		dacc_eprof * ep = 0;
		if ( dacc_eprof_create(&ep,tspace,pbps,pboff,prlen,nreads,twodb ? 1 : 0) ) die("error distribution estimate: out of memory");
		dacc_eprof_set_deep(ep,1);
		unsigned int hw = std::thread::hardware_concurrency(); if ( !hw ) hw = 1; if ( hw > 64 ) hw = 64;
		Batch EB;
		for ( int64_t b0 = minaread; b0 < top; b0 += 256 )
		{
			loadBatch(b0,std::min<int64_t>(top,b0+256),true,EB);
			if ( !EB.err.empty() ) die(EB.err);
			if ( EB.spiles.empty() ) continue;
			if ( dacc_eprof_add(ep,EB.spiles.data(),EB.spiles.size(),EB.sel.data(),EB.sel.size(),EB.trace.data(),EB.ntrace,tbytes,o.d,hw) ) die("error distribution estimate failed (out of memory)");
		}
		uint32_t const * dv = 0; uint64_t dn = 0;
		dacc_eprof_deep(ep,&dv,&dn);
		double const dcnt = static_cast<double>(dn);
		uint64_t i = 0;
		while ( i < dn )
		{
			uint64_t j = i; while ( j < dn && dv[j] == dv[i] ) ++j;
			std::printf("[deep]\t%g\t%g\n",dv[i]/4294967295.0,static_cast<double>(j)/dcnt);
			i = j;
		}
		dacc_eprof_destroy(ep);
		dacc_las_close(las); dacc_db_close(A.h); if ( twodb ) dacc_db_close(B2.h);
		return EXIT_SUCCESS;
	}
	if ( !have && !(minaread <= maxaread) )
	{
		if ( o.V ) std::fprintf(stderr,"[V] empty read interval, nothing to do\n");
		dacc_las_close(las); dacc_db_close(A.h); if ( twodb ) dacc_db_close(B2.h);
		return EXIT_SUCCESS;
	}
	if ( !have )
	{
		auto const te0 = std::chrono::steady_clock::now();
		int64_t const top = std::min<int64_t>(toparead,minaread+1024);
		uint64_t counts[4] = {0,0,0,0}; uint64_t usable = 0, unusable = 0; double eavg = 0, edif = 0;
		dacc_eprof * ep = 0;
		if ( dacc_eprof_create(&ep,tspace,pbps,pboff,prlen,nreads,twodb ? 1 : 0) ) die("error profile estimation: out of memory");
		unsigned int hw = std::thread::hardware_concurrency(); if ( !hw ) hw = 1; if ( hw > 64 ) hw = 64;
		Batch EB;
		for ( int64_t b0 = minaread; b0 < top; b0 += 256 )
		{
			loadBatch(b0,std::min<int64_t>(top,b0+256),true,EB);
			if ( !EB.err.empty() ) die(EB.err);
			if ( EB.spiles.empty() ) continue;
			if ( dacc_eprof_add(ep,EB.spiles.data(),EB.spiles.size(),EB.sel.data(),EB.sel.size(),EB.trace.data(),EB.ntrace,tbytes,o.d,hw) ) die("error profile estimation failed (out of memory)");
		}
		{
			uint64_t nskip = 0, nseen = 0;
			dacc_eprof_skipped(ep,&nskip,&nseen);
			if ( nskip ) std::fprintf(stderr,"[E] error profile estimation: %llu of %llu piles left out (malformed overlap or trace records)\n",static_cast<unsigned long long>(nskip),static_cast<unsigned long long>(nseen));
			if ( nseen && 2*nskip > nseen ) die("error profile estimation: most piles of the sample have malformed overlap records -- does the .las belong to this database?");
		}
		if ( dacc_eprof_finish(ep,counts,&usable,&unusable,&eavg,&edif,prof) ) die("error profile estimation found no usable window; give --eprof<p_i,p_d,est_cor>");
		dacc_eprof_destroy(ep);
		std::fprintf(stderr,"usable=%llu unusable=%llu eavg=%g edif=%g\n",static_cast<unsigned long long>(usable),static_cast<unsigned long long>(unusable),eavg,edif);
		std::fprintf(stderr,"AlignmentStatistics(matches=%llu,mismatches=%llu,insertions=%llu,deletions=%llu)\n",
			static_cast<unsigned long long>(counts[0]),static_cast<unsigned long long>(counts[1]),static_cast<unsigned long long>(counts[2]),static_cast<unsigned long long>(counts[3]));
		if ( o.V ) std::fprintf(stderr,"[V] error profile estimated on %u host threads in %.2f s\n",hw,std::chrono::duration<double>(std::chrono::steady_clock::now()-te0).count());
		std::string const tmpfn = eproffn + ".tmp." + std::to_string(static_cast<long long>(::getpid()));
		{
			std::ofstream out(tmpfn.c_str(),std::ios::binary);
			if ( o.binaryeprof ) out << encodeProfileBinary(counts,eavg,edif);
			else { char buf[128]; std::snprintf(buf,sizeof(buf),"%.17g %.17g %.17g\n",prof[0],prof[1],prof[2]); out << buf; }
			out.flush();
			if ( !out ) { std::remove(tmpfn.c_str()); die("cannot write the error profile " + tmpfn); }
		}
		if ( std::rename(tmpfn.c_str(),eproffn.c_str()) != 0 ) { std::remove(tmpfn.c_str()); die("cannot rename " + tmpfn + " to " + eproffn); }
	}
	if ( o.V ) std::fprintf(stderr,"[V] p_i=%.17g p_d=%.17g est_cor=%.17g\n",prof[0],prof[1],prof[2]);
	if ( o.eprofonly ) return EXIT_SUCCESS;

	dacc_params p; std::memset(&p,0,sizeof(p));
	p.w = o.w; p.a = o.a; p.klow = o.klow; p.khigh = o.khigh; p.minfilterfreq = o.minff; p.maxfilterfreq = o.maxff; p.minwindowcov = o.m;
	p.maxalign = o.d; p.eminrate = o.e; p.minlen = o.l; p.producefull = o.f ? 1 : 0; p.tspace = tspace; p.device = o.device; p.verbose = o.V;
	if ( o.loaderonly )
	{
		int const nwork = o.gpus;
		int64_t const batch = static_cast<int64_t>(o.batch);
		std::mutex mu; std::condition_variable cv; std::deque<Batch *> loaded, freeb; std::vector<Batch> bslots(2*nwork);
		for ( size_t i = 0; i < bslots.size(); ++i ) freeb.push_back(&bslots[i]);
		double load_s = 0, wait_s = 0, plan_s = 0; uint64_t npl = 0, nov = 0, abases = 0, nwin = 0, nbat = 0; std::string fatal;
		auto const t0 = std::chrono::steady_clock::now();
		std::thread loader([&]() {
			uint64_t seq = 0;
			for ( int64_t b0 = minaread; ; b0 += batch )
			{
				Batch * B;
				auto const tw = std::chrono::steady_clock::now();
				{ std::unique_lock<std::mutex> lk(mu); cv.wait(lk,[&]{ return !freeb.empty(); }); B = freeb.front(); freeb.pop_front(); }
				auto const tl = std::chrono::steady_clock::now();
				B->end = !(b0 < toparead); B->seq = seq++;
				if ( !B->end ) loadBatch(b0,std::min(toparead,b0+batch),false,*B);
				auto const te = std::chrono::steady_clock::now();
				bool const stop = B->end || !B->err.empty();
				{
					std::lock_guard<std::mutex> lk(mu);
					wait_s += std::chrono::duration<double>(tl-tw).count(); load_s += std::chrono::duration<double>(te-tl).count();
					if ( !B->end ) { npl += B->spiles.size(); nov += B->sel.size(); for ( size_t i = 0; i < B->spiles.size(); ++i ) abases += prlen[B->spiles[i].aread]; }
					loaded.push_back(B);
				}
				cv.notify_all();
				if ( stop ) break;
			}
		});
		bool stopall = false;
		auto const consumer = [&]()
		{
			while ( true )
			{
				Batch * B = 0;
				{
					std::unique_lock<std::mutex> lk(mu);
					cv.wait(lk,[&]{ return stopall || !loaded.empty(); });
					if ( stopall && loaded.empty() ) return;
					B = loaded.front(); loaded.pop_front();
					if ( B->end || !B->err.empty() ) { stopall = true; if ( !B->err.empty() && fatal.empty() ) fatal = B->err; }
				}
				cv.notify_all();
				if ( !B->end && B->err.empty() && !B->spiles.empty() )
				{
					auto const tp = std::chrono::steady_clock::now();
					uint64_t w = 0, nb = 0;
					int const rc = dacc_plan_only(&p,prlen,nreads,B->spiles.data(),B->spiles.size(),B->sel.data(),B->sel.size(),B->trace.data(),B->ntrace,tbytes,&w,&nb);
					double const dt = std::chrono::duration<double>(std::chrono::steady_clock::now()-tp).count();
					std::lock_guard<std::mutex> lk(mu);
					if ( rc && fatal.empty() ) fatal = "planner failed (" + std::to_string(rc) + ")";
					plan_s += dt; nwin += w; ++nbat;
				}
				{ std::lock_guard<std::mutex> lk(mu); freeb.push_back(B); }
				cv.notify_all();
			}
		};
		std::vector<std::thread> cons; for ( int g = 0; g < nwork; ++g ) cons.emplace_back(consumer);
		loader.join(); for ( size_t g = 0; g < cons.size(); ++g ) cons[g].join();
		double const tot = std::chrono::duration<double>(std::chrono::steady_clock::now()-t0).count();
		if ( !fatal.empty() ) die(fatal);
		std::fprintf(stderr,"[L] host side only: %llu piles (%llu selected overlaps, %llu A-read bases, %llu windows) in %llu batches of %llu A reads, %.3f s wall\n"
			"[L] loader thread: %.3f s reading + selecting = %.0f piles/s = %.1f Mbase/s of A reads; %.3f s waiting for a free batch slot\n"
			"[L] %d planner thread(s) standing in for the device workers: %.3f s in dacc_plan_only in total = %.0f piles/s per worker\n",
			static_cast<unsigned long long>(npl),static_cast<unsigned long long>(nov),static_cast<unsigned long long>(abases),static_cast<unsigned long long>(nwin),
			static_cast<unsigned long long>(nbat),static_cast<unsigned long long>(o.batch),tot,
			load_s,load_s > 0 ? npl/load_s : 0.0,load_s > 0 ? abases/load_s/1e6 : 0.0,wait_s,
			nwork,plan_s,plan_s > 0 ? npl/plan_s : 0.0);
		return EXIT_SUCCESS;
	}

	int const nwork = o.gpus;
	std::vector<dacc_ctx *> ctxs(nwork,static_cast<dacc_ctx *>(0));
	{
		int const ndev = dacc_device_count();
		if ( ndev <= 0 || o.device >= ndev ) die("no usable HIP device " + std::to_string(o.device) + " (" + std::to_string(ndev) + " visible)");
		int const span = ndev - o.device;
		for ( int g = 0; g < nwork; ++g )
		{
			dacc_params pg = p; pg.device = o.device + g % span;
			int const rc = dacc_create(&ctxs[g],&pg);
			if ( rc ) die("dacc_create failed (" + std::to_string(rc) + ") for worker " + std::to_string(g) + " on device " + std::to_string(pg.device) + " of " + std::to_string(ndev));
			if ( dacc_load_db(ctxs[g],pbps,nbps,pboff,prlen,nreads) ) die(std::string("load db: ") + dacc_last_error(ctxs[g]));
			if ( dacc_set_error_profile(ctxs[g],prof[0],prof[1],prof[2]) ) die(std::string("error profile: ") + dacc_last_error(ctxs[g]));
			if ( o.V && nwork > 1 ) std::fprintf(stderr,"[V] device worker %d on HIP device %d\n",g,pg.device);
		}
	}

	int64_t const batch = static_cast<int64_t>(o.batch);
	struct Out { std::vector<dacc_fragment> fr; std::string bases; uint64_t seq = 0; bool end = false; };
	std::mutex mu; std::condition_variable cv;
	std::deque<Batch *> loaded; std::deque<Batch *> freeb; std::deque<Out *> outs; std::deque<Out *> freeo;
	std::vector<Batch> bslots(2*nwork); std::vector<Out> oslots(2*nwork+1);
	for ( size_t i = 0; i < bslots.size(); ++i ) freeb.push_back(&bslots[i]);
	for ( size_t i = 0; i < oslots.size(); ++i ) freeo.push_back(&oslots[i]);
	auto const t0 = std::chrono::steady_clock::now();
	std::thread loader([&]() {
		uint64_t seq = 0;
		for ( int64_t b0 = minaread; ; b0 += batch )
		{
			Batch * B;
			{ std::unique_lock<std::mutex> lk(mu); cv.wait(lk,[&]{ return !freeb.empty(); }); B = freeb.front(); freeb.pop_front(); }
			B->end = !(b0 < toparead); B->seq = seq++;
			if ( !B->end ) loadBatch(b0,std::min(toparead,b0+batch),false,*B);
			bool const stop = B->end || !B->err.empty();
			{ std::lock_guard<std::mutex> lk(mu); loaded.push_back(B); }
			cv.notify_all();
			if ( stop ) break;
		}
	});
	uint64_t well = 0, totalbases = 0;
	std::thread writer([&]() {
		std::string rec; uint64_t nextseq = 0;
		while ( true )
		{
			Out * O = 0;
			{
				std::unique_lock<std::mutex> lk(mu);
				cv.wait(lk,[&]{ for ( size_t i = 0; i < outs.size(); ++i ) if ( outs[i]->seq == nextseq ) return true; return false; });
				for ( size_t i = 0; i < outs.size(); ++i ) if ( outs[i]->seq == nextseq ) { O = outs[i]; outs.erase(outs.begin()+i); break; }
			}
			++nextseq;
			if ( O->end ) break;
			rec.clear();
			for ( size_t i = 0; i < O->fr.size(); ++i )
			{
				dacc_fragment const & f = O->fr[i];
				char hdr[160];
				std::snprintf(hdr,sizeof(hdr),">%d/%llu/%u_%u A=[%u,%u]\n",f.aread+1,static_cast<unsigned long long>(well++),f.first,f.first+f.len,f.first,f.last);
				rec += hdr;
				for ( uint32_t q = 0; q < f.len; q += 80 ) { rec.append(O->bases.data()+f.seq_off+q,std::min<uint32_t>(80,f.len-q)); rec += '\n'; }
			}
			std::fwrite(rec.data(),1,rec.size(),stdout);
			{ std::lock_guard<std::mutex> lk(mu); freeo.push_back(O); }
			cv.notify_all();
		}
	});
	std::string fatal; bool stopall = false;
	double gpu_s = 0; uint64_t nbatches = 0;
	struct { uint64_t nwindows, tier_out[3], deep_windows, deep_out, last_windows, last_out, vdeep_windows, vdeep_out; double window_ms, tier_ms[3], deep_ms, last_ms, vdeep_ms; } tstat = {};
	auto const deviceWorker = [&](int const g)
	{
		dacc_ctx * const ctx = ctxs[g];
		while ( true )
		{
			Batch * B = 0;
			{
				std::unique_lock<std::mutex> lk(mu);
				cv.wait(lk,[&]{ return stopall || !loaded.empty(); });
				if ( stopall ) return;
				B = loaded.front();
				if ( B->end || !B->err.empty() ) stopall = true;
				loaded.pop_front();
			}
			cv.notify_all();
			std::string err = B->err;
			bool const end = B->end; uint64_t const seq = B->seq;
			Out * O;
			{ std::unique_lock<std::mutex> lk(mu); cv.wait(lk,[&]{ return !freeo.empty(); }); O = freeo.front(); freeo.pop_front(); }
			O->fr.clear(); O->bases.clear(); O->seq = seq; O->end = end || !err.empty();
			if ( err.empty() && !end && !B->spiles.empty() )
			{
				auto const tb0 = std::chrono::steady_clock::now();
				if ( dacc_submit_piles(ctx,B->spiles.data(),B->spiles.size(),B->sel.data(),B->sel.size(),B->trace.data(),B->ntrace,tbytes) )
					err = std::string("batch failed: ") + dacc_last_error(ctx);
				else
				{
					double const dt = std::chrono::duration<double>(std::chrono::steady_clock::now()-tb0).count();
					{ char const * pe = dacc_pile_errors(ctx); if ( pe && *pe ) std::fprintf(stderr,"[E] skipped reads:\n%s",pe); }
					dacc_fragment const * fr = 0; uint64_t nf = 0; char const * bases = 0; uint64_t nb = 0;
					if ( dacc_collect(ctx,&fr,&nf,&bases,&nb) ) err = std::string("collect: ") + dacc_last_error(ctx);
					else
					{
						O->fr.assign(fr,fr+nf); O->bases.assign(bases,nb);
						dacc_release(ctx);
						dacc_timing tm; std::memset(&tm,0,sizeof(tm));
						bool const havetm = dacc_last_timing2(ctx,&tm,sizeof(tm)) == DACC_OK;
						std::lock_guard<std::mutex> lk(mu); gpu_s += dt; ++nbatches; totalbases += nb;
						if ( havetm )
						{
							tstat.nwindows += tm.nwindows; tstat.window_ms += tm.window_ms; tstat.deep_ms += tm.deep_ms; tstat.deep_windows += tm.deep_windows; tstat.deep_out += tm.deep_out;
							tstat.last_ms += tm.last_ms; tstat.last_windows += tm.last_windows; tstat.last_out += tm.last_out;
							tstat.vdeep_ms += tm.vdeep_ms; tstat.vdeep_windows += tm.vdeep_windows; tstat.vdeep_out += tm.vdeep_out;
							for ( int i = 0; i < 3; ++i ) { tstat.tier_out[i] += tm.tier_out[i]; tstat.tier_ms[i] += tm.tier_ms[i]; }
						}
					}
				}
			}
			bool last;
			{
				std::lock_guard<std::mutex> lk(mu);
				if ( !err.empty() ) { if ( fatal.empty() ) fatal = err; stopall = true; O->end = true; O->fr.clear(); O->bases.clear(); }
				last = O->end;
				outs.push_back(O); freeb.push_back(B);
			}
			cv.notify_all();
			if ( last ) return;
		}
	};
	std::vector<std::thread> workers;
	for ( int g = 1; g < nwork; ++g ) workers.emplace_back(deviceWorker,g);
	deviceWorker(0);
	for ( size_t i = 0; i < workers.size(); ++i ) workers[i].join();
	writer.join();
	if ( !fatal.empty() ) { std::fflush(stdout); std::fprintf(stderr,"[E] %s\n",fatal.c_str()); std::_Exit(EXIT_FAILURE); }
	loader.join();
	std::fflush(stdout);
	if ( o.V )
	{
		double const el = std::chrono::duration<double>(std::chrono::steady_clock::now()-t0).count();
		std::fprintf(stderr,"[V] %llu corrected bases in %.2f s end to end (load + select + plan + GPU + FASTA) = %.3f Mbase/s; %llu batches, %.2f s in dacc_submit_piles%s\n",
			static_cast<unsigned long long>(totalbases),el,el > 0 ? totalbases/el/1e6 : 0.0,static_cast<unsigned long long>(nbatches),gpu_s,
			nwork > 1 ? (" (summed over " + std::to_string(nwork) + " device workers)").c_str() : "");
		std::fprintf(stderr,"[V] %llu windows, window kernels %.1f ms: tier slots %.1f / %.1f / %.1f ms handed on %llu / %llu / %llu windows (the last to the last stage); "
			"deep-window tier (97 ... 250 strings) %.1f ms, %llu windows finished, %llu handed on; "
			"last stage (layout in device memory) %.1f ms, %llu windows finished, %llu handed on; "
			"very deep stage (251 ... 1000 strings) %.1f ms, %llu windows finished, %llu handed on to the generic engine\n",
			static_cast<unsigned long long>(tstat.nwindows),tstat.window_ms,tstat.tier_ms[0],tstat.tier_ms[1],tstat.tier_ms[2],
			static_cast<unsigned long long>(tstat.tier_out[0]),static_cast<unsigned long long>(tstat.tier_out[1]),static_cast<unsigned long long>(tstat.tier_out[2]),
			tstat.deep_ms,static_cast<unsigned long long>(tstat.deep_windows),static_cast<unsigned long long>(tstat.deep_out),
			tstat.last_ms,static_cast<unsigned long long>(tstat.last_windows),static_cast<unsigned long long>(tstat.last_out),
			tstat.vdeep_ms,static_cast<unsigned long long>(tstat.vdeep_windows),static_cast<unsigned long long>(tstat.vdeep_out));
	}
	for ( int g = 0; g < nwork; ++g ) dacc_destroy(ctxs[g]);
	dacc_las_close(las); dacc_db_close(A.h); if ( twodb ) dacc_db_close(B2.h);
	return EXIT_SUCCESS;
}
```

### daccord_amd/csrc/dev_types.hpp

```cpp
#ifndef DACC_DEV_TYPES_HPP
#define DACC_DEV_TYPES_HPP
#include <stdint.h>

namespace dacc {

struct DevTables
{
	int32_t nrows;
	int32_t nsup;
	int32_t kln;
	int32_t pad;
	double const * dpnorm;
	double const * dpsq;
	uint64_t const * dpsq_vs;
	uint16_t const * dpsq_first;
	uint16_t const * dpsq_size;
	uint16_t const * suplo;
	uint16_t const * suphi;
	uint32_t const * klim;
};

struct DevParams
{
	uint32_t w, a, klow, khigh;
	int32_t minff, maxff;
	uint32_t minwindowcov;
	int32_t checklim;
	uint64_t maxalign, eminrate;
	int32_t tspace;
	int32_t producefull;
	uint64_t minlen;
};

struct DevOvl
{
	int32_t bread; uint32_t flags;
	int32_t abpos, aepos, bbpos, bepos;
	uint32_t ekey;
	int32_t y0, ny;
	int32_t nblk;
	uint64_t wtoff;
	uint64_t blk0;
	uint64_t trace_off;
};

struct DevPile
{
	int32_t aread; uint32_t novl;
	uint64_t first_ovl;
	uint32_t l;
	uint32_t nwin;
	uint64_t winbase;
	uint64_t posbase;
	uint32_t rl;
	uint32_t pad;
};

struct ArenaCaps
{
	uint32_t maxs;
	uint32_t precap;
	uint32_t nodecap;
	uint32_t fcap;
	uint32_t strcap;
	uint32_t linkcap;
	uint32_t sfcap;
	uint32_t rlcap;
	uint32_t poolcap;
	uint32_t blcap;
	uint32_t conscap;
	uint32_t lstr;
	uint64_t bytes;
};

enum { LSTR = 256 };
enum { LPW = LSTR/64 };
enum { LSTRMAX = 4096 };
enum { WREC = 256 };
enum { MAXCONS = 96 };
enum { WRECW = 640 };
enum { MAXCONSW = 224 };
#define DACC_WIDE_W(w_) ((w_) > 64u)
#define DACC_WREC_OF(w_) (DACC_WIDE_W(w_) ? static_cast<uint32_t>(::dacc::WRECW) : static_cast<uint32_t>(::dacc::WREC))
#define DACC_MAXCONS_OF(w_) (DACC_WIDE_W(w_) ? static_cast<uint32_t>(::dacc::MAXCONSW) : static_cast<uint32_t>(::dacc::MAXCONS))
#define DACC_WMAX 128u

enum { WS_INSUFFICIENT = 0, WS_OK = 1, WS_FAILED = 2, WS_OVERFLOW = 3 };

}
#endif
```

### daccord_amd/csrc/fast_window.hpp

```cpp
#ifndef DACC_FAST_WINDOW_HPP
#define DACC_FAST_WINDOW_HPP
#include "wave.hpp"
#include "dev_types.hpp"
#include "arena.hpp"
#include "window_main.hpp"
#include "tier_pipeline.hpp"

namespace dacc {

enum { WS_RETRY = 4 };
enum { FNOPAR = 0xFF };
enum { FSEQCAP = 48 };

struct FSI { uint64_t w; uint16_t left, right, current, path; };
struct FCC { uint64_t w; uint32_t o, l; };

template<int TIER> struct FastTier;
#if !defined(DACC_RCH01)
#define DACC_RCH01 2
#endif
template<> struct FastTier<1> { typedef uint8_t id_t; typedef uint8_t sid_t; enum : uint32_t { smax = 250, gw = 1, wcapg = 1024, rch = DACC_RCH01, fch = 4, fnw = 2, fnc = 40, idmax = 250, rpstcap = 256, lstr = 64, maxs = 32, precap = 1024, ncap = 776, scap = 112, lcap = 960, wcap = 1024, rccap = 144, fcap = 192, siqcap = 56, blcap = 96, seqcap = 32, psiq = 8, consrow = 64, lscrids = 2048, wide = 0, mins = 0, gmem = 0 }; };
template<> struct FastTier<0> { typedef uint8_t id_t; typedef uint8_t sid_t; enum : uint32_t { smax = 250, gw = 1, wcapg = 768, rch = DACC_RCH01, fch = 4, fnw = 2, fnc = 32, idmax = 250, rpstcap = 256, lstr = 64, maxs = 28, precap = 576, ncap = 524, scap = 88, lcap = 640, wcap = 768, rccap = 96, fcap = 128, siqcap = 56, blcap = 96, seqcap = 32, psiq = 8, consrow = 64, lscrids = 2048, wide = 0, mins = 0, gmem = 0 }; };
template<> struct FastTier<7> { typedef uint8_t id_t; typedef uint8_t sid_t; enum : uint32_t { smax = 250, gw = 1, wcapg = 896, rch = DACC_RCH01, fch = 4, fnw = 2, fnc = 32, idmax = 250, rpstcap = 256, lstr = 64, maxs = 28, precap = 704, ncap = 640, scap = 104, lcap = 800, wcap = 896, rccap = 112, fcap = 148, siqcap = 56, blcap = 96, seqcap = 32, psiq = 8, consrow = 64, lscrids = 2048, wide = 0, mins = 0, gmem = 0 }; };
#if !defined(DACC_T2_NCAP)
#define DACC_T2_NCAP 1536
#endif
#if !defined(DACC_T2_LCAP)
#define DACC_T2_LCAP 2032
#endif
template<> struct FastTier<2> { typedef uint8_t id_t; typedef uint8_t sid_t; enum : uint32_t { smax = 250, gw = 1, wcapg = 3072, rch = 4, fch = 4, fnw = 4, fnc = 64, idmax = 250, rpstcap = 256, lstr = 64, maxs = 96, precap = 2048, ncap = DACC_T2_NCAP, scap = 232, lcap = DACC_T2_LCAP, wcap = 3072, rccap = 256, fcap = 192, siqcap = 96, blcap = 96, seqcap = 48, psiq = 10, consrow = 96, lscrids = 2560, wide = 0, mins = 0, gmem = 0 }; };
template<> struct FastTier<6> { typedef uint8_t id_t; typedef uint8_t sid_t; enum : uint32_t { smax = 250, gw = 1, wcapg = 2048, rch = 2, fch = 8, fnw = 3, fnc = 40, idmax = 250, rpstcap = 256, lstr = 128, maxs = 40, precap = 1024, ncap = 1024, scap = 248, lcap = 1280, wcap = 2048, rccap = 256, fcap = 256, siqcap = 96, blcap = 96, seqcap = 48, psiq = 10, consrow = 96, lscrids = 2560, wide = 0, mins = 0, gmem = 0 }; };

template<> struct FastTier<3> { typedef uint16_t id_t; typedef uint16_t sid_t; enum : uint32_t { smax = 1000, gw = 1, wcapg = 8192, rch = 8, fch = 16, fnw = 4, fnc = 72, idmax = 4000, rpstcap = 768, lstr = 128, maxs = 96, precap = 4096, ncap = 2048, scap = 1024, lcap = 4096, wcap = 8192, rccap = 2048, fcap = 512, siqcap = 256, blcap = 128, seqcap = 48, psiq = 10, consrow = 96, lscrids = 2560, wide = 0, mins = 0, gmem = 0 }; };

template<> struct FastTier<4> { typedef uint8_t id_t; typedef uint8_t sid_t; enum : uint32_t { smax = 250, gw = 1, wcapg = 608, rch = 4, fch = 4, fnw = 2, fnc = 40, idmax = 250, rpstcap = 256, lstr = 64, maxs = 96, precap = 2048, ncap = 256, scap = 48, lcap = 256, wcap = 608, rccap = 128, fcap = 96, siqcap = 56, blcap = 96, seqcap = 48, psiq = 10, consrow = 96, lscrids = 2560, wide = 0, mins = 0, gmem = 0 }; };

template<> struct FastTier<5> { typedef uint16_t id_t; typedef uint8_t sid_t; enum : uint32_t { smax = 250, gw = 0, wcapg = 0, rch = 8, fch = 16, fnw = 4, fnc = 72, idmax = 4000, rpstcap = 768, lstr = 128, maxs = 64, precap = 4096, ncap = 1792, scap = 250, lcap = 2048, wcap = 2040, rccap = 512, fcap = 512, siqcap = 256, blcap = 128, seqcap = 48, psiq = 10, consrow = 96, lscrids = 2560, wide = 0, mins = 0, gmem = 0 }; };

template<> struct FastTier<8> { typedef uint16_t id_t; typedef uint8_t sid_t; enum : uint32_t { smax = 250, gw = 1, wcapg = 6144, rch = 4, fch = 8, fnw = 4, fnc = 64, idmax = 4000, rpstcap = 768, lstr = 128, maxs = 40, precap = 3072, ncap = 2304, scap = 248, lcap = 3072, wcap = 6144, rccap = 640, fcap = 512, siqcap = 96, blcap = 128, seqcap = 96, psiq = 10, consrow = 128, lscrids = 2560, wide = 1, mins = 0, gmem = 0 }; };

template<> struct FastTier<9> { typedef uint16_t id_t; typedef uint16_t sid_t; enum : uint32_t { smax = 500, gw = 1, wcapg = 8192, rch = 16, fch = 16, fnw = 4, fnc = 72, idmax = 4000, rpstcap = 768, lstr = 128, maxs = 64, precap = 4096, ncap = 3072, scap = 512, lcap = 4096, wcap = 8192, rccap = 2048, fcap = 1024, siqcap = 256, blcap = 128, seqcap = 96, psiq = 10, consrow = 128, lscrids = 2560, wide = 1, mins = 0, gmem = 0 }; };

template<> struct FastTier<10> { typedef uint16_t id_t; typedef uint8_t sid_t; enum : uint32_t { smax = 250, gw = 1, wcapg = 6144, rch = 4, fch = 8, fnw = 4, fnc = 64, idmax = 4000, rpstcap = 768, lstr = 128, maxs = 64, precap = 2560, ncap = 2048, scap = 248, lcap = 3072, wcap = 6144, rccap = 896, fcap = 512, siqcap = 128, blcap = 128, seqcap = 48, psiq = 10, consrow = 96, lscrids = 2560, wide = 0, mins = 0, gmem = 0 }; };

template<> struct FastTier<11> { typedef uint16_t id_t; typedef uint8_t sid_t; enum : uint32_t { smax = 250, gw = 1, wcapg = 4096, rch = 4, fch = 8, fnw = 4, fnc = 72, idmax = 4000, rpstcap = 768, lstr = 128, maxs = 96, precap = 4096, ncap = 1536, scap = 248, lcap = 2048, wcap = 4096, rccap = 640, fcap = 384, siqcap = 128, blcap = 128, seqcap = 48, psiq = 10, consrow = 96, lscrids = 2560, wide = 0, mins = 0, gmem = 0 }; };

template<> struct FastTier<12> { typedef uint16_t id_t; typedef uint16_t sid_t; enum : uint32_t { smax = 1000, gw = 1, wcapg = 8192, rch = 8, fch = 16, fnw = 4, fnc = 72, idmax = 4000, rpstcap = 768, lstr = 128, maxs = 250, precap = 8192, ncap = 2048, scap = 1024, lcap = 4096, wcap = 8192, rccap = 2048, fcap = 512, siqcap = 256, blcap = 128, seqcap = 48, psiq = 10, consrow = 96, lscrids = 2560, wide = 0, mins = 96, gmem = 0 }; };

template<> struct FastTier<13> { typedef uint16_t id_t; typedef uint16_t sid_t; enum : uint32_t { smax = 2000, gw = 1, wcapg = 16384, rch = 16, fch = 16, fnw = 4, fnc = 72, idmax = 4000, rpstcap = 768, lstr = 128, maxs = 250, precap = 16384, ncap = 4096, scap = 2048, lcap = 8192, wcap = 16384, rccap = 4096, fcap = 1024, siqcap = 512, blcap = 128, seqcap = 48, psiq = 10, consrow = 96, lscrids = 4096, wide = 0, mins = 0, gmem = 1 }; };
template<> struct FastTier<14> { typedef uint16_t id_t; typedef uint16_t sid_t; enum : uint32_t { smax = 1000, gw = 1, wcapg = 16384, rch = 16, fch = 16, fnw = 4, fnc = 72, idmax = 4000, rpstcap = 768, lstr = 128, maxs = 250, precap = 16384, ncap = 6144, scap = 1024, lcap = 8192, wcap = 16384, rccap = 4096, fcap = 2048, siqcap = 512, blcap = 128, seqcap = 96, psiq = 10, consrow = 128, lscrids = 4096, wide = 1, mins = 0, gmem = 1 }; };
template<> struct FastTier<15> { typedef uint16_t id_t; typedef uint16_t sid_t; enum : uint32_t { smax = 2000, gw = 1, wcapg = 32768, rch = 16, fch = 16, fnw = 4, fnc = 72, idmax = 4000, rpstcap = 768, lstr = 128, maxs = 1000, precap = 16384, ncap = 4096, scap = 2048, lcap = 8192, wcap = 32768, rccap = 4096, fcap = 1024, siqcap = 512, blcap = 128, seqcap = 48, psiq = 10, consrow = 96, lscrids = 4096, wide = 0, mins = 250, gmem = 1 }; };

static_assert(FastTier<15>::mins == VDEEP_MINS && FastTier<13>::maxs == VDEEP_MINS,"the very deep stage takes what the last stage refuses at its string count");

HDEV constexpr uint32_t fcpow2(uint32_t v) { uint32_t p = 1; while ( p < v ) p <<= 1; return p; }
HDEV constexpr uint32_t fcmax(uint32_t a, uint32_t b) { return a > b ? a : b; }
template<bool W, typename A, typename B> struct FWideSel { typedef A type; };
template<typename A, typename B> struct FWideSel<false,A,B> { typedef B type; };

#define FLD(name,type,count,start) \
	static constexpr uint32_t o_##name = (start); \
	static constexpr uint32_t e_##name = (o_##name + static_cast<uint32_t>(sizeof(type))*static_cast<uint32_t>(count) + 7u) & ~7u; \
	HDEV LDSQ type * name() const { return reinterpret_cast<LDSQ type *>(base + o_##name); }

template<typename CT, bool GW = (CT::gw != 0)> struct FastLds;

template<typename CT>
struct FastLds<CT,false>
{
	LDSQ uint8_t * base;
	static constexpr uint32_t keycap = fcpow2(CT::maxs < 2 ? 2 : CT::maxs);
	static constexpr bool wides = false; static constexpr uint32_t fqmax = 255u, icap = CT::precap;
	static_assert(CT::maxs <= 256,"the legacy layout has 8 bit node frequencies and string ids");
	static_assert((CT::precap & (CT::precap-1)) == 0,"precap must be a power of two: the bitonic sorts pad to one");
	static_assert(sizeof(typename CT::id_t) > 1 || (CT::fcap <= 256 && CT::rccap <= 256),"pool slots are recorded as id_t (pout)");
	static_assert(CT::blcap <= 128 && (CT::blcap & 7) == 0,"base length buckets: two 64 bit occupancy words, cleared 8 at a time");
	static_assert(CT::lstr == 64 || CT::lstr == 128,"string stride: one or two 64 bit words per pattern mask");
	static constexpr uint32_t pw = CT::lstr/64;
	typedef uint8_t sid_t;
	static_assert(sizeof(typename CT::sid_t) == 1,"16 bit stretch ids need the gw layout");
	FLD(str,uint8_t,CT::maxs*CT::lstr,0)
	FLD(slen,uint8_t,CT::maxs,e_str)
	FLD(peq,uint64_t,CT::maxs*4*pw,e_slen)
	FLD(ipos,uint8_t,CT::precap,e_peq)
	FLD(irpos,uint8_t,CT::precap,e_ipos)
	FLD(nv,uint32_t,CT::ncap,e_irpos)
	FLD(nps,uint16_t,CT::ncap+1,e_nv)
	FLD(nfreq,uint8_t,CT::ncap,e_nps)
	FLD(succ0,uint16_t,CT::ncap,e_nfreq)
	FLD(sinfo,uint16_t,CT::ncap,e_succ0)
	FLD(npred,uint8_t,CT::ncap,e_sinfo)
	FLD(nrange,uint32_t,CT::ncap,e_npred)
	FLD(mfirst,uint64_t,keycap,e_nrange)
	FLD(mlast,uint64_t,keycap,e_mfirst)
	FLD(suplo8,uint8_t,FSUPCAP,e_mlast)
	FLD(suphi8,uint8_t,FSUPCAP,e_suplo8)
	FLD(vrem,uint8_t,8,e_suphi8)
	FLD(vadd,uint8_t,8,e_vrem)
	FLD(vapos,uint8_t,8,e_vadd)
	FLD(vfn,uint16_t,8,e_vapos)
	FLD(vln,uint16_t,8,e_vfn)
	FLD(sstack,uint16_t,3*24,e_vln)
	FLD(chain,uint8_t,64,e_sstack)
	FLD(midpar,uint16_t,8,e_chain)
	FLD(midA,uint8_t,8,e_midpar)
	FLD(midB,uint8_t,8,e_midA)
	static constexpr uint32_t ubase = e_midB;
	FLD(pre,uint64_t,CT::precap,ubase)
	FLD(lastk,uint64_t,keycap,e_pre)
	static constexpr uint32_t uA = e_lastk;
	FLD(sfirst,uint16_t,CT::scap,ubase)
	FLD(slast,uint16_t,CT::scap,e_sfirst)
	FLD(sslen,uint16_t,CT::scap,e_slast)
	FLD(slink,uint16_t,CT::scap,e_sslen)
	FLD(maskF,uint64_t,CT::scap,e_slink)
	FLD(maskR,uint64_t,CT::scap,e_maskF)
	FLD(woffF,uint16_t,CT::scap,e_maskR)
	FLD(woffR,uint16_t,CT::scap,e_woffF)
	FLD(links,uint16_t,CT::lcap,e_woffR)
	FLD(wF_lo,uint32_t,CT::wcap,e_links)
	FLD(wF1_lo,uint32_t,CT::wcap,e_wF_lo)
	FLD(wFl_lo,uint32_t,CT::wcap,e_wF1_lo)
	FLD(wR_lo,uint32_t,CT::wcap,e_wFl_lo)
	FLD(wR1_lo,uint32_t,CT::wcap,e_wR_lo)
	FLD(wF_hi,uint16_t,CT::wcap,e_wR1_lo)
	FLD(wR_hi,uint16_t,CT::wcap,e_wF_hi)
	FLD(wF1_hi,uint8_t,CT::wcap,e_wR_hi)
	FLD(wFl_hi,uint8_t,CT::wcap,e_wF1_hi)
	FLD(wR1_hi,uint8_t,CT::wcap,e_wFl_hi)
	FLD(lhead,uint8_t,CT::ncap,e_wR1_hi)
	FLD(lord,uint32_t,CT::scap,e_lhead)
	FLD(ppos,uint8_t,CT::scap,e_lord)
	FLD(fkmer,uint32_t,CT::fnc,e_ppos)
	FLD(lkmer,uint32_t,CT::fnc,e_fkmer)
	FLD(fnode,uint16_t,CT::fnc,e_lkmer)
	FLD(lnode,uint16_t,CT::fnc,e_fnode)
	FLD(parF,uint8_t,CT::fnc,e_lnode)
	FLD(posF,uint8_t,CT::fnc,e_parF)
	FLD(parL,uint8_t,CT::fnc,e_posF)
	FLD(posL,uint8_t,CT::fnc,e_parL)
	FLD(pieF,uint8_t,CT::fnc,e_posL)
	FLD(pieL,uint8_t,CT::fnc,e_pieF)
	static constexpr uint32_t consmax = MAXCONS;
	static_assert(CT::wide == 0,"the wide tier needs the gw layout");
	FLD(bestL,uint8_t,MAXCONS,e_pieL)
	FLD(cdh,FCC,16,e_bestL)
	static_assert(uA <= o_cdh,"the model table copy (from o_cdh on) is loaded for gap filling while the instance array is live");
	FLD(cseq,uint8_t,18*CT::seqcap,e_cdh)
	FLD(ch,FCC,16,e_cseq)
	FLD(acc,FCC,16,e_ch)
	FLD(accerr,uint32_t,16,e_acc)
	FLD(canderr,uint8_t,16*CT::maxs,e_accerr)
	FLD(consL,uint8_t,16*CT::consrow,e_canderr)
	static constexpr uint32_t lscrbytes = static_cast<uint32_t>(CT::lscrids)*static_cast<uint32_t>(sizeof(typename CT::id_t));
	FLD(lscr,uint8_t,lscrbytes,e_cseq)
	FLD(siq,FSI,CT::siqcap,e_cseq)
	static_assert(sizeof(FSI)*CT::siqcap <= lscrbytes,"the serial score interval heap shares the lane scratch");
	static constexpr uint32_t pbase = fcmax(e_consL,e_lscr);
	FLD(rc_w,uint64_t,CT::rccap,pbase)
	FLD(rc_parent,typename CT::id_t,CT::rccap,e_rc_w)
	FLD(rc_stretch,uint8_t,CT::rccap,e_rc_parent)
	FLD(rc_pos,uint8_t,CT::rccap,e_rc_stretch)
	FLD(rc_len,uint8_t,CT::rccap,e_rc_pos)
	FLD(rc_baselen,uint8_t,CT::rccap,e_rc_len)
	FLD(rc_acc,typename CT::id_t,CT::rccap,e_rc_baselen)
	FLD(rc_ord,typename CT::id_t,CT::rccap,e_rc_acc)
	FLD(rc_arw,typename CT::id_t,CT::rccap,e_rc_ord)
	FLD(rc_sbl,uint8_t,CT::rccap,e_rc_arw)
	FLD(rc_front,uint32_t,CT::rccap,e_rc_sbl)
	FLD(rbase,uint16_t,CT::fnc+1,e_rc_front)
	FLD(rn,uint16_t,CT::fnc+1,e_rbase)
	FLD(rmaxw,uint64_t,CT::fnc+1,e_rn)
	FLD(rtmask,uint64_t,CT::fnc+1,e_rmaxw)
	FLD(rfmask,uint64_t,CT::fnc+1,e_rtmask)
	FLD(f_w,uint64_t,CT::fcap,e_rfmask)
	FLD(f_parent,typename CT::id_t,CT::fcap,e_f_w)
	FLD(f_stretch,uint8_t,CT::fcap,e_f_parent)
	FLD(f_pos,uint8_t,CT::fcap,e_f_stretch)
	FLD(f_baselen,uint8_t,CT::fcap,e_f_pos)
	FLD(f_len,uint8_t,CT::fcap,e_f_baselen)
	FLD(fp_id,typename CT::id_t,CT::fcap,e_f_len)
	FLD(fp_cl,uint8_t,CT::fcap,e_fp_id)
	FLD(fp_front,uint32_t,CT::fcap,e_fp_cl)
	FLD(fp_adj,uint64_t,CT::fcap,e_fp_front)
	FLD(fchb,uint8_t,8*CT::fnw*(CT::fnc+1),e_fp_adj)
	FLD(fnp,uint16_t,CT::fnc+1,e_fchb)
	FLD(ffm,uint64_t,CT::fnc+1,e_fnp)
	FLD(ftm,uint64_t,CT::fnc+1,e_ffm)
	FLD(fmx,uint64_t,CT::fnc+1,e_ftm)
	FLD(pout,typename CT::id_t,32*32,e_fmx)
	FLD(poutn,uint8_t,64,e_pout)
	FLD(ctr,uint32_t,4,e_poutn)
	FLD(rchx,uint8_t,32,e_ctr)
	static constexpr uint32_t upool = e_rchx;
	FLD(rchb,uint8_t,(CT::fnc < 64 ? CT::fnc : 64u)*32,o_fchb)
	static_assert(e_rchb <= o_pout,"reverse chunk lists must fit the per first k-mer tables");
	FLD(tfirst,uint16_t,CT::scap,pbase)
	FLD(tlast,uint16_t,CT::scap,e_tfirst)
	FLD(tslen,uint16_t,CT::scap,e_tlast)
	FLD(tlink,uint16_t,CT::scap,e_tslen)
	FLD(skey,uint64_t,fcpow2(CT::scap),e_tlink)
	static constexpr uint32_t uraw = e_skey;
	FLD(alpv,uint64_t,MAXCONS+1,pbase)
	FLD(almv,uint64_t,MAXCONS+1,e_alpv)
	FLD(albot,uint16_t,MAXCONS+1,e_almv)
	FLD(alops,uint8_t,2*MAXCONS+2*64+8,e_albot)
	static constexpr uint32_t ualn = e_alops;
	static constexpr uint32_t uend = fcmax(fcmax(uA,uraw),fcmax(upool,ualn));
	FLD(gfbuf,uint64_t,(pbase-uA)/8,uA)
	static constexpr uint32_t gfcap = (pbase-uA)/8;
	static constexpr uint32_t taskbytes = ((2*CT::scap+2)*2 + 2*(2*CT::scap) + 15u) & ~15u;
	FLD(toff,uint16_t,2*CT::scap+2,upool-taskbytes)
	FLD(ulo,uint8_t,2*CT::scap,e_toff)
	FLD(uhi,uint8_t,2*CT::scap,e_ulo)
	FLD(tab,uint32_t,(upool-taskbytes-o_cdh)/4,o_cdh)
	static constexpr uint32_t tabcap = (upool-taskbytes-o_cdh)/4;
	HDEV static uint32_t bytes(uint32_t const, uint32_t const) { return (uend + 15u) & ~15u; }
	static_assert(6u*CT::ncap + 16u <= e_wR1_hi - o_wF_lo,"scratch tables of the stretch walk must fit the weight arrays");
	static_assert(CT::wcap*4 >= CT::ncap*2,"interior node table must fit the weight array it borrows");
	static_assert(2u*CT::ncap + CT::scap + 8u <= 4u*CT::wcap,"reachability scratch must fit the first weight array");
	HDEV LDSQ uint32_t * xcnt32() const { return reinterpret_cast<LDSQ uint32_t *>(base + o_wF_lo); }
	HDEV LDSQ uint16_t * xstep() const { return reinterpret_cast<LDSQ uint16_t *>(base + ((e_wR1_hi - 2u*CT::ncap) & ~7u)); }
	HDEV LDSQ uint16_t * xwtmp() const { return reinterpret_cast<LDSQ uint16_t *>(base + o_wF_lo); }
	static constexpr uint32_t xnslot = (((e_wR1_hi - 2u*CT::ncap) & ~7u) - o_wF_lo) / 128u;
	HDEV LDSQ uint16_t * xsid() const { return reinterpret_cast<LDSQ uint16_t *>(base + o_wR_lo); }
	HDEV LDSQ uint8_t * xspos() const { return reinterpret_cast<LDSQ uint8_t *>(base + o_wR1_lo); }
	HDEV LDSQ uint8_t * xreach() const { return reinterpret_cast<LDSQ uint8_t *>(base + o_wF_lo); }
};

template<typename CT>
struct FastLds<CT,true>
{
	LDSQ uint8_t * base;
	static constexpr uint32_t keycap = fcpow2(CT::maxs < 2 ? 2 : CT::maxs);
	static_assert(sizeof(typename CT::id_t) > 1 || (CT::fcap <= 256 && CT::rccap <= 256),"pool slots are recorded as id_t (pout)");
	static_assert(CT::blcap <= 128 && (CT::blcap & 7) == 0,"base length buckets: two 64 bit occupancy words, cleared 8 at a time");
	static_assert(CT::lstr == 64 || CT::lstr == 128,"the gw layout holds strings of up to 64 bases in one word per pattern mask, of up to 128 in two (round 6)");
	static constexpr uint32_t pw = CT::lstr/64;
	typedef typename CT::sid_t sid_t;
	static constexpr bool wides = CT::maxs > 256;
	static constexpr uint32_t fqmax = wides ? 1023u : 255u;
	static constexpr uint32_t icap = wides ? 4u*CT::precap : CT::precap;
	typedef typename FWideSel<wides,uint16_t,uint8_t>::type nfreq_t;
	typedef typename FWideSel<wides,uint32_t,uint16_t>::type nps_t;
	static_assert(fqmax <= (1u << (8u*sizeof(nfreq_t))) - 1u,"a node frequency holds fqmax");
	static_assert(icap <= (sizeof(nps_t) == 2 ? 65535u : 0xFFFFFFFFu),"nps[nn] = npre <= icap must fit a first-instance offset");
	FLD(slen,uint8_t,CT::maxs,0)
	static constexpr uint32_t supcap = CT::wide ? static_cast<uint32_t>(FSUPCAPW) : static_cast<uint32_t>(FSUPCAP);
	FLD(suplo8,uint8_t,supcap,e_slen)
	FLD(suphi8,uint8_t,supcap,e_suplo8)
	FLD(vrem,uint8_t,8,e_suphi8)
	FLD(vadd,uint8_t,8,e_vrem)
	FLD(vapos,uint8_t,8,e_vadd)
	FLD(vfn,uint16_t,8,e_vapos)
	FLD(vln,uint16_t,8,e_vfn)
	FLD(sstack,uint16_t,3*24,e_vln)
	FLD(chain,uint8_t,64,e_sstack)
	FLD(midpar,uint16_t,8,e_chain)
	FLD(midA,uint8_t,8,e_midpar)
	FLD(midB,uint8_t,8,e_midA)
	FLD(nv,uint32_t,CT::ncap,e_midB)
	FLD(npred,sid_t,CT::ncap,e_nv)
	static constexpr uint32_t consmax = CT::wide ? 128u : static_cast<uint32_t>(MAXCONS);
	static constexpr uint32_t alw = CT::wide ? 2u : 1u;
	FLD(bestL,uint8_t,consmax,e_npred)
	static constexpr uint32_t sbase = (e_bestL + 15u) & ~15u;
	FLD(peq,uint64_t,CT::maxs*4*pw,sbase)
	FLD(ipos,uint8_t,icap,e_peq)
	FLD(irpos,uint8_t,icap,e_ipos)
	FLD(nps,nps_t,CT::ncap+1,e_irpos)
	FLD(nfreq,nfreq_t,CT::ncap,e_nps)
	FLD(succ0,uint16_t,CT::ncap,e_nfreq)
	FLD(sinfo,uint16_t,CT::ncap,e_succ0)
	FLD(nrange,uint32_t,CT::ncap,e_sinfo)
	FLD(mfirst,uint64_t,keycap,e_nrange)
	FLD(mlast,uint64_t,keycap,e_mfirst)
	static constexpr uint32_t send = (e_mlast + 15u) & ~15u;
	static constexpr uint32_t sbytes = send - sbase;
	FLD(rc_w,uint64_t,CT::rccap,sbase)
	FLD(rc_parent,typename CT::id_t,CT::rccap,e_rc_w)
	FLD(rc_stretch,sid_t,CT::rccap,e_rc_parent)
	FLD(rc_pos,uint8_t,CT::rccap,e_rc_stretch)
	FLD(rc_len,uint8_t,CT::rccap,e_rc_pos)
	FLD(rc_baselen,uint8_t,CT::rccap,e_rc_len)
	FLD(rc_acc,typename CT::id_t,CT::rccap,e_rc_baselen)
	FLD(rc_ord,typename CT::id_t,CT::rccap,e_rc_acc)
	FLD(rc_arw,typename CT::id_t,CT::rccap,e_rc_ord)
	FLD(rc_sbl,uint8_t,CT::rccap,e_rc_arw)
	FLD(rc_front,uint32_t,CT::rccap,e_rc_sbl)
	FLD(rbase,uint16_t,CT::fnc+1,e_rc_front)
	FLD(rn,uint16_t,CT::fnc+1,e_rbase)
	FLD(rmaxw,uint64_t,CT::fnc+1,e_rn)
	FLD(rtmask,uint64_t,CT::fnc+1,e_rmaxw)
	FLD(rfmask,uint64_t,CT::fnc+1,e_rtmask)
	FLD(f_w,uint64_t,CT::fcap,e_rfmask)
	FLD(f_parent,typename CT::id_t,CT::fcap,e_f_w)
	FLD(f_stretch,sid_t,CT::fcap,e_f_parent)
	FLD(f_pos,uint8_t,CT::fcap,e_f_stretch)
	FLD(f_baselen,uint8_t,CT::fcap,e_f_pos)
	FLD(f_len,uint8_t,CT::fcap,e_f_baselen)
	FLD(fp_id,typename CT::id_t,CT::fcap,e_f_len)
	FLD(fp_cl,uint8_t,CT::fcap,e_fp_id)
	FLD(fp_front,uint32_t,CT::fcap,e_fp_cl)
	FLD(fp_adj,uint64_t,CT::fcap,e_fp_front)
	FLD(fchb,uint8_t,8*CT::fnw*(CT::fnc+1),e_fp_adj)
	FLD(fnp,uint16_t,CT::fnc+1,e_fchb)
	FLD(ffm,uint64_t,CT::fnc+1,e_fnp)
	FLD(ftm,uint64_t,CT::fnc+1,e_ffm)
	FLD(fmx,uint64_t,CT::fnc+1,e_ftm)
// ... 2826 lines not shown
							else mode = PM_PEND | (nm <= PSIQ ? nm : 15u);
						}
						L.poutn()[t] = mode;
					}
					uint32_t tot; wv_scan_excl(((mode & 0xF0u) == PM_PEND && (mode & 0x0Fu) != 15u) ? (mode & 0x0Fu) : 0u,tot);
					ntask += tot;
				}
				wv_sync();
				LDSQ uint16_t * const TL = reinterpret_cast<LDSQ uint16_t *>(L.pout());
				enum : uint32_t { TLCAP = 32u*32u*static_cast<uint32_t>(sizeof(id_t))/2u };
				bool const flat = ntask != 0 && ntask <= TLCAP;
				if ( flat )
				{
					uint32_t tb = 0;
					for ( uint32_t t0 = 0; t0 < nround; t0 += WSZ )
					{
						uint32_t const t = t0 + lane;
						uint32_t const mode = t < nround ? L.poutn()[t] : static_cast<uint32_t>(PM_SKIP);
						uint32_t const nm = ((mode & 0xF0u) == PM_PEND && (mode & 0x0Fu) != 15u) ? (mode & 0x0Fu) : 0u;
						uint32_t tot; uint32_t const pre = tb + wv_scan_excl(nm,tot);
						for ( uint32_t j = 0; j < nm; ++j ) TL[pre+j] = static_cast<uint16_t>(t | (j << 6));
						tb += tot;
					}
					wv_sync();
					for ( uint32_t q0 = 0; q0 < ntask; q0 += WSZ )
					{
						uint32_t const q = q0 + lane;
						if ( q < ntask )
						{
							uint32_t const en = TL[q], t = en & 63u, j = en >> 6;
							uint32_t const p = p0 + t;
							uint32_t pfi, pli; pairFL(p,pfi,pli); pfi += fstart;
							ChunkList<FNW> FC; forwardTreeLoad(FC,pfi);
							if ( !intervalTask(FC,L.rbase()[pli],L.rn()[pli],lmin,lmax,HH + PSIQ*t + j) ) L.poutn()[t] = PM_SERIAL;
						}
					}
					wv_sync();
				}
				for ( uint32_t t = lane; t < nround; t += WSZ )
				{
					uint32_t mode = L.poutn()[t];
					if ( (mode & 0xF0u) == PM_PEND )
					{
						uint32_t const p = p0 + t;
						uint32_t pfi, pli; pairFL(p,pfi,pli); pfi += fstart;
						ChunkList<FNW> FC; forwardTreeLoad(FC,pfi);
						uint32_t cnt;
						if ( flat && (mode & 0x0Fu) != 15u )
						{
							uint32_t const n = heapOfList(FC,L.rbase()[pli],HH + PSIQ*t,mode & 0x0Fu);
							cnt = combineLanePops(FC,L.rbase()[pli],n,16,HH + PSIQ*t,L.pout() + 2*POUTE*t,cfull,roundT0);
						}
						else cnt = combineLane(FC,L.fnp()[pfi],L.rbase()[pli],L.rn()[pli],L.rfmask()[pli],lmin,lmax,16,HH + PSIQ*t,L.pout() + 2*POUTE*t,cfull,roundT0);
						mode = cnt == 0xFF ? static_cast<uint32_t>(PM_SERIAL) : (cnt ? cnt : static_cast<uint32_t>(PM_SKIP));
						L.poutn()[t] = mode;
					}
					if ( mode != PM_SKIP ) live |= 1ull << t;
				}
				live = wv_or64(live);
				wv_sync();
				}
				PROF(*this,5)
				if ( lane == 0 ) pcount(27,1);
				uint32_t q = 0;
				while ( true )
				{
					uint32_t req = 0;
					if ( lane == 0 ) { lscrdirty = false; req = replayRound(q,nround,p0,fstart,lmin,lmax,nb == 1,live); }
					wv_sync();
					flags = wv_bcast(flags,0); if ( flags ) return false;
					req = wv_bcast(req,0);
					if ( !req ) break;
					if ( req == 2 )
					{
						uint32_t const pq = p0 + wv_bcast(q,0);
						fstart += pq/nL; pskip = pq%nL; bw = 1; restart = true;
						if ( lane == 0 ) pcount(28,1);
						break;
					}
					break;
				}
				PROF(*this,7)
			}
			if ( restart ) continue;
			fstart += nb; pskip = 0;
		}
		{ SITE_T0 materializeKept(); SITE(34) }
		{ SITE_T0 LEDGER_REP(13) restoreS(); SITE(25) }
		PROF(*this,12)
		wv_sync();
		uint32_t const nkept = wv_bcast(ncdh,0);
		{
			uint32_t tie = 0;
			for ( uint32_t c = lane; c < nkept; c += WSZ )
			{
				FCC const e = ldget(L.cdh()+c);
				uint32_t rank = 0;
				for ( uint32_t j = 0; j < nkept; ++j ) { uint64_t const wj = L.cdh()[j].w; rank += (wj > e.w) ? 1u : 0u; tie |= (wj == e.w && j != c) ? 1u : 0u; }
				ldput(L.acc()+rank,e);
			}
			tie = wv_any(tie);
			FSTAT_ADD(21,tie ? 1u : 0u); FSTAT_ADD(22,nkept ? 1u : 0u);
			wv_sync();
			if ( lane == 0 )
			{
				if ( tie )
				{
					uint32_t nch = 0;
					while ( ncdh ) { FCC const c = ldget(L.cdh()); spop<FCC,true>(L.cdh(),ncdh); spush<FCC,false>(L.ch(),nch,c); }
					while ( nch ) { ldput(L.acc()+nacc,ldget(L.ch())); ++nacc; spop<FCC,false>(L.ch(),nch); }
				}
				else { nacc = nkept; ncdh = 0; }
			}
		}
		wv_sync();
		uint32_t const nc = wv_bcast(nacc,0);
		nacc = nc;
		for ( uint32_t c = lane; c < nc; c += WSZ )
		{
			uint32_t const slot = L.acc()[c].o, n = L.acc()[c].l & 0xFF;
			uint32_t const len = decodeSeq(L.cseq()+FSEQCAP*slot,n,L.consL()+c*CONSROW);
			L.acc()[c].o = c*CONSROW; L.acc()[c].l = len;
		}
		wv_sync();
		LEDGER_REP(14)
		for ( uint32_t t = lane; t < nc*mao; t += WSZ )
		{
			uint32_t const c = t / mao, j = t - c*mao;
			L.canderr()[t] = myersDistance(j,L.consL() + L.acc()[c].o,L.acc()[c].l);
		}
		wv_sync();
		for ( uint32_t c = lane; c < nc; c += WSZ )
		{
			uint32_t s = 0;
			for ( uint32_t j = 0; j < mao; ++j ) s += L.canderr()[c*mao+j];
			L.accerr()[c] = s;
		}
		wv_sync();
		{
			LDSQ uint32_t * const serr = reinterpret_cast<LDSQ uint32_t *>(L.canderr());
			static_assert(16*CT::maxs >= 64 && (FastLds<CT>::o_canderr & 3) == 0,"sorted error sums borrow the candidate error bytes");
			for ( uint32_t c = lane; c < nc; c += WSZ )
			{
				uint32_t const e = L.accerr()[c];
				uint32_t rank = 0;
				for ( uint32_t j = 0; j < nc; ++j ) { uint32_t const ej = L.accerr()[j]; rank += (ej < e || (ej == e && j < c)) ? 1u : 0u; }
				ldput(L.ch()+rank,ldget(L.acc()+c));
				serr[rank] = e;
			}
			wv_sync();
			for ( uint32_t c = lane; c < nc; c += WSZ ) { ldput(L.acc()+c,ldget(L.ch()+c)); L.accerr()[c] = serr[c]; }
		}
		wv_sync();
		PROF(*this,13)
		FSTAT_MX(0,mao); FSTAT_MX(1,npre); FSTAT_MX(2,nn); FSTAT_MX(3,n0); FSTAT_MX(4,npool); FSTAT_MX(5,nlinks); FSTAT_MX(6,nwF); FSTAT_MX(7,nwR);
		FSTAT_MX(8,rstop); FSTAT_MX(9,nF); FSTAT_MX(10,nL); FSTAT_ADD(11,1); FSTAT_MX(12,nc); FSTAT_ADD(24,nc ? 0u : 1u);
#if defined(DACC_EMUL)
		if ( lane == 0 ) { FILE * f = ftrav_file(); if ( f ) { uint32_t nlv = 0; for ( uint32_t i = 0; i < nL; ++i ) nlv += L.lnode()[i] != 0xFFFF; fprintf(f,"%d %u %u %u %u %u %u %u %u %u %u %u %u\n",int(CT::maxs),mao,npre,nn,n0,npool,nF,nL,nlv,rstop,nwF,nwR,nc); fflush(f); } }
#endif
		return nc != 0;
	}

	DEV int32_t estimateLength()
	{
		int32_t maxvprodindex = -1;
		uint32_t mn = 0xFFFFFFFFu, mx = 0;
		for ( uint32_t j = lane; j < mao; j += WSZ )
		{
			uint32_t const len = L.slen()[j];
			uint32_t const lastpos = len ? len-1 : 0;
			mn = lastpos < mn ? lastpos : mn; mx = lastpos > mx ? lastpos : mx;
		}
		mn = ~wv_max(~mn); mx = wv_max(mx);
		uint32_t const supStart = mn < static_cast<uint32_t>(T.nsup) ? T.suplo[mn] : T.nrows;
		uint32_t const supEnd = mx < static_cast<uint32_t>(T.nsup) ? T.suphi[mx] : T.nrows;
		uint64_t bestbits = 0; uint32_t besti = 0xFFFFFFFFu;
		for ( uint32_t c = supStart; c < supEnd; c += WSZ )
		{
			uint32_t const i = c + lane;
			double vprod = 0.0;
			if ( i < supEnd )
			{
				double const * row = T.dpnorm + static_cast<uint64_t>(i)*T.nsup;
				vprod = 1.0;
				for ( uint32_t j = 0; j < mao; j += 4 )
				{
					uint32_t const l0 = L.slen()[j], l1 = j+1 < mao ? L.slen()[j+1] : 0, l2 = j+2 < mao ? L.slen()[j+2] : 0, l3 = j+3 < mao ? L.slen()[j+3] : 0;
					uint32_t const ns = static_cast<uint32_t>(T.nsup);
					double const r0 = (l0 && (l0-1) < ns) ? row[l0-1] : 0.0, r1 = (l1 && (l1-1) < ns) ? row[l1-1] : 0.0;
					double const r2 = (l2 && (l2-1) < ns) ? row[l2-1] : 0.0, r3 = (l3 && (l3-1) < ns) ? row[l3-1] : 0.0;
					if ( l0 ) vprod *= r0;
					if ( l1 ) vprod *= r1;
					if ( l2 ) vprod *= r2;
					if ( l3 ) vprod *= r3;
				}
			}
			union { double d; uint64_t u; } cv; cv.d = vprod;
			uint64_t const mb = wv_max64(cv.u);
			if ( mb > bestbits )
			{
				uint64_t const fi = wv_min64(cv.u == mb ? i : 0xFFFFFFFFull);
				bestbits = mb; besti = static_cast<uint32_t>(fi);
			}
		}
		union { double d; uint64_t u; } dm; dm.d = DACC_DBL_MIN;
		if ( bestbits > dm.u ) maxvprodindex = besti;
		if ( maxvprodindex == -1 )
		{
			int32_t res = -1;
			if ( lane == 0 )
			{
				uint32_t maxlen = 0;
				for ( uint32_t j = 0; j < mao; ++j ) maxlen = L.slen()[j] > maxlen ? L.slen()[j] : maxlen;
				int32_t maxoff = -1; double maxoffv = DACC_DBL_MIN;
				for ( int32_t i = 0; i < T.nrows; ++i )
				{
					uint32_t const fs = T.dpsq_first[i], sz = T.dpsq_size[i];
					double const * V = T.dpsq + static_cast<uint64_t>(i)*T.nsup;
					double sdot = 0;
					for ( uint32_t t = 0; t < sz; ++t )
					{
						uint32_t const jj = fs+t;
						if ( jj < maxlen+1 )
						{
							uint32_t cnt = 0;
							for ( uint32_t j = 0; j < mao; ++j ) cnt += (L.slen()[j] == jj);
							double const o = cnt ? static_cast<double>(cnt-1) : 0.0;
							sdot += V[jj] * o;
						}
						else break;
					}
					if ( sdot > maxoffv ) { maxoff = i; maxoffv = sdot; }
				}
				if ( maxoff != -1 && maxoffv >= 1e-3 ) res = maxoff;
			}
			maxvprodindex = static_cast<int32_t>(wv_bcast(static_cast<uint32_t>(res),0));
		}
		return maxvprodindex;
	}

	DEV uint32_t alignAndEmitWide(LDSQ uint8_t const * cons, uint32_t const n)
	{
		if constexpr ( CT::wide != 0 )
		{
		uint32_t const m = P.w;
		enum { PW = FastLds<CT>::pw };
		static_assert(PW == 2,"the A window of a wide tier has two words per pattern mask");
		LDSQ uint64_t const * PEQ = L.peq();
		uint64_t const mask1 = (m == 128) ? ~0ull : ((1ull<<(m-64))-1);
		uint64_t Pv0 = ~0ull, Mv0 = 0, Pv1 = mask1, Mv1 = 0; uint32_t score = m;
		L.alpv()[0] = Pv0; L.alpv()[1] = Pv1; L.almv()[0] = Mv0; L.almv()[1] = Mv1; L.albot()[0] = m;
		uint64_t const top = 1ull<<(m-65);
		for ( uint32_t c = 0; c < n; ++c )
		{
			uint32_t const ch = cons[c] & 3u;
			uint64_t const Eq0 = PEQ[PW*ch], Eq1 = PEQ[PW*ch+1];
			uint64_t const Xv0 = Eq0 | Mv0;
			uint64_t const Xh0 = (((Eq0 & Pv0) + Pv0) ^ Pv0) | Eq0;
			uint64_t Ph0 = Mv0 | ~(Xh0 | Pv0);
			uint64_t Mh0 = Pv0 & Xh0;
			uint64_t const phc = Ph0>>63, mhc = Mh0>>63;
			Ph0 = (Ph0<<1) | 1ull; Mh0 <<= 1;
			Pv0 = Mh0 | ~(Xv0 | Ph0);
			Mv0 = Ph0 & Xv0;
			uint64_t const Eq1c = Eq1 | mhc;
			uint64_t const Xv1 = Eq1 | Mv1;
			uint64_t const Xh1 = (((Eq1c & Pv1) + Pv1) ^ Pv1) | Eq1c;
			uint64_t Ph1 = Mv1 | ~(Xh1 | Pv1);
			uint64_t Mh1 = Pv1 & Xh1;
			if ( Ph1 & top ) ++score; else if ( Mh1 & top ) --score;
			Ph1 = (Ph1<<1) | phc; Mh1 = (Mh1<<1) | mhc;
			Pv1 = (Mh1 | ~(Xv1 | Ph1)) & mask1;
			Mv1 = (Ph1 & Xv1) & mask1;
			L.alpv()[2*c+2] = Pv0; L.alpv()[2*c+3] = Pv1; L.almv()[2*c+2] = Mv0; L.almv()[2*c+3] = Mv1; L.albot()[c+1] = score;
		}
		uint32_t i = m, j = n; uint32_t d = score; uint32_t nops = 0;
		while ( i || j )
		{
			uint32_t op = 2; bool done = false;
			if ( i && j )
			{
				uint32_t const sh = i-1;
				uint64_t const p0 = L.alpv()[2*(j-1)], p1 = L.alpv()[2*(j-1)+1], q0 = L.almv()[2*(j-1)], q1 = L.almv()[2*(j-1)+1];
				uint32_t const np_ = sh < 64 ? (dacc_popc64(p0>>sh) + dacc_popc64(p1)) : dacc_popc64(p1>>(sh-64));
				uint32_t const nm_ = sh < 64 ? (dacc_popc64(q0>>sh) + dacc_popc64(q1)) : dacc_popc64(q1>>(sh-64));
				uint32_t const dd = L.albot()[j-1] - np_ + nm_;
				uint32_t const cj = cons[j-1] & 3u;
				uint32_t const neq = ((PEQ[PW*cj + (sh>>6)] >> (sh&63u)) & 1ull) ? 0u : 1u;
				if ( dd + neq == d ) { op = neq ? 1 : 0; --i; --j; d = dd; done = true; }
			}
			if ( !done && i )
			{
				uint32_t const r = i-1;
				uint64_t const pv = L.alpv()[2*j+(r>>6)];
				if ( (pv >> (r&63u)) & 1ull ) { op = 3; --i; d = d-1; done = true; }
			}
			if ( !done ) { op = 2; --j; d = d-1; }
			L.alops()[nops++] = op;
		}
		return nops;
		}
		else return 0;
	}
	DEV uint32_t alignAndEmit(LDSQ uint8_t const * cons, uint32_t const n)
	{
		if constexpr ( CT::wide != 0 ) { if ( DACC_WIDE_W(P.w) ) return alignAndEmitWide(cons,n); }
		uint32_t const m = P.w;
		LDSQ uint64_t const * PEQ = L.peq();
		enum { PW = FastLds<CT>::pw };
		uint64_t const e0 = PEQ[0*PW], e1 = PEQ[1*PW], e2 = PEQ[2*PW], e3 = PEQ[3*PW];
		LDSQ uint64_t const * T8 = reinterpret_cast<LDSQ uint64_t const *>(cons);
		static_assert(MAXCONS <= 96 && (FastLds<CT>::o_bestL & 7) == 0,"consensus packed into three 64 bit words");
		uint64_t const mask = (m == 64) ? ~0ull : ((1ull<<m)-1);
		uint64_t Pv = mask, Mv = 0; uint32_t score = m;
		L.alpv()[0] = Pv; L.almv()[0] = Mv; L.albot()[0] = m;
		uint64_t const top = 1ull<<(m-1);
		uint64_t ck0 = 0, ck1 = 0, ck2 = 0;
		uint64_t w = n ? T8[0] : 0ull;
		for ( uint32_t c0 = 0; c0 < n; c0 += 8 )
		{
			uint64_t const wn = (c0+8 < n) ? T8[(c0>>3)+1] : 0ull;
			uint32_t const cnt = (n-c0 < 8) ? (n-c0) : 8u;
			for ( uint32_t u = 0; u < cnt; ++u )
			{
				uint32_t const c = c0+u;
				uint64_t const ch = (w >> (8*u)) & 3u;
				uint64_t const cs = ch << (2*(c&31));
				ck0 |= c < 32 ? cs : 0ull; ck1 |= (c >= 32 && c < 64) ? cs : 0ull; ck2 |= c >= 64 ? cs : 0ull;
				uint64_t const Eq = (ch & 2) ? ((ch & 1) ? e3 : e2) : ((ch & 1) ? e1 : e0);
				uint64_t const Xv = Eq | Mv;
				uint64_t const Xh = (((Eq & Pv) + Pv) ^ Pv) | Eq;
				uint64_t Ph = Mv | ~(Xh | Pv);
				uint64_t Mh = Pv & Xh;
				if ( Ph & top ) ++score; else if ( Mh & top ) --score;
				Ph = (Ph<<1) | 1ull; Mh <<= 1;
				Pv = (Mh | ~(Xv | Ph)) & mask;
				Mv = (Ph & Xv) & mask;
				L.alpv()[c+1] = Pv; L.almv()[c+1] = Mv; L.albot()[c+1] = score;
			}
			w = wn;
		}
		uint32_t i = m, j = n; uint32_t d = score; uint32_t nops = 0;
		uint64_t pvj = Pv, pv1 = 0, mv1 = 0; uint32_t bot1 = 0;
		if ( j ) { pv1 = L.alpv()[j-1]; mv1 = L.almv()[j-1]; bot1 = L.albot()[j-1]; }
		while ( i || j )
		{
			uint32_t op = 2; bool done = false; bool left = false;
			if ( i && j )
			{
				uint64_t const sh = i-1;
				uint32_t const dd = bot1 - dacc_popc64(pv1>>sh) + dacc_popc64(mv1>>sh);
				uint32_t const jj = j-1;
				uint64_t const ckw = jj < 32 ? ck0 : (jj < 64 ? ck1 : ck2);
				uint32_t const ch = static_cast<uint32_t>(ckw >> (2*(jj&31))) & 3u;
				uint64_t const Eq = (ch & 2) ? ((ch & 1) ? e3 : e2) : ((ch & 1) ? e1 : e0);
				uint32_t const neq = ((Eq >> sh) & 1) ? 0u : 1u;
				if ( dd + neq == d ) { op = neq ? 1 : 0; --i; --j; d = dd; done = true; left = true; }
			}
			if ( !done && i )
			{
				uint64_t const bit = 1ull<<(i-1);
				if ( pvj & bit ) { op = 3; --i; d = d-1; done = true; }
			}
			if ( !done ) { op = 2; --j; d = d-1; left = true; }
			if ( left )
			{
				pvj = pv1;
				if ( j ) { pv1 = L.alpv()[j-1]; mv1 = L.almv()[j-1]; bot1 = L.albot()[j-1]; }
			}
			L.alops()[nops++] = op;
		}
		return nops;
	}
	DEV void emitRecord(LDSQ uint8_t const * cons, uint32_t const nops, uint8_t * rec)
	{
		uint32_t const m = P.w;
		if constexpr ( CT::wide != 0 )
		{
			if ( DACC_WIDE_W(m) )
			{
				uint8_t * const off = rec+2; uint8_t * const sym = rec + 2 + 2*(m+2);
				if ( lane == 0 ) { rec[0] = 1; rec[1] = 0; off[0] = 0; off[1] = 0; off[2*(m+1)] = nops & 0xFFu; off[2*(m+1)+1] = nops >> 8; }
				uint32_t cbase = 0, abase = 0;
				for ( uint32_t c0 = 0; c0 < nops; c0 += WSZ )
				{
					uint32_t const q = c0 + lane;
					bool const act = q < nops;
					uint32_t const op = act ? L.alops()[nops-1-q] : 2u;
					uint32_t ctot, atot;
					uint32_t const cpos = cbase + wv_scan_flag(act && op != 3,ctot);
					uint32_t const arank = abase + wv_scan_flag(act && op != 2,atot);
					if ( act )
					{
						sym[q] = (op == 3) ? 4 : cons[cpos];
						if ( op != 2 ) { off[2*(arank+1)] = (q+1) & 0xFFu; off[2*(arank+1)+1] = (q+1) >> 8; }
					}
					cbase += ctot; abase += atot;
				}
				return;
			}
		}
		uint8_t * off = rec+1; uint8_t * sym = rec + 1 + (m+2);
		if ( lane == 0 ) { rec[0] = 1; off[0] = 0; off[m+1] = nops; }
		uint32_t cbase = 0, abase = 0;
		for ( uint32_t c0 = 0; c0 < nops; c0 += WSZ )
		{
			uint32_t const q = c0 + lane;
			bool const act = q < nops;
			uint32_t const op = act ? L.alops()[nops-1-q] : 2u;
			uint32_t ctot, atot;
			uint32_t const cpos = cbase + wv_scan_flag(act && op != 3,ctot);
			uint32_t const arank = abase + wv_scan_flag(act && op != 2,atot);
			if ( act )
			{
				sym[q] = (op == 3) ? 4 : cons[cpos];
				if ( op != 2 ) off[arank+1] = q+1;
			}
			cbase += ctot; abase += atot;
		}
	}
};

enum { FW_DONE = 0, FW_NEXT = 1, FW_GENERIC = 2 };
DEV uint32_t classifyWindow(WindowBatch const & B, uint64_t const widx, uint32_t const t0inst, uint32_t const t7inst = 0)
{
	uint32_t lo = 0, hi = B.npiles;
	while ( hi-lo > 1 ) { uint32_t const mid = (lo+hi)>>1; if ( B.piles[mid].winbase <= widx ) lo = mid; else hi = mid; }
	DevPile const pile = B.piles[lo];
	uint32_t const y = static_cast<uint32_t>(widx - pile.winbase);
	uint32_t astart, aend;
	windowInterval(pile.l,B.P.a,B.P.w,y,astart,aend);
	uint32_t const k = B.P.klow;
	uint32_t nact = 0, inst = B.P.w >= k ? (B.P.w - k + 1) : 0u;
	DevOvl const * ov = B.ovl + pile.first_ovl;
	for ( uint32_t z = 0; z < pile.novl; ++z )
		if ( ov[z].abpos <= static_cast<int32_t>(astart) && ov[z].aepos >= static_cast<int32_t>(aend) )
		{
			uint64_t const row = ov[z].wtoff + (y - ov[z].y0);
			uint32_t const len = B.wt_e[row] - B.wt_b[row];
			++nact; inst += len >= k ? (len - k + 1) : 0u;
		}
	uint64_t const nb = (B.P.maxalign > 0) ? (B.P.maxalign-1) : 0;
	uint32_t const mao = 1 + static_cast<uint32_t>(nact < nb ? nact : nb);
	if ( mao <= FastTier<0>::maxs && inst <= t0inst && B.P.w <= 63 ) return 0u;
	if ( t7inst && mao <= FastTier<7>::maxs && inst <= t7inst && B.P.w <= 63 ) return 2u;
	return 1u;
}

template<typename CT>
DEV int processWindowFast(FastBatch const & FB, uint64_t const widx, LDSQ uint8_t * lds, bool const resume = false)
{
	WindowBatch const & B = FB.W;
	FastEngine<CT> E;
#if defined(DACC_EMUL)
	{ char const * pz = getenv("DACC_EMUL_POISON"); if ( pz ) __builtin_memset(static_cast<void *>(&E),atoi(pz),sizeof(E)); }
#endif
	if ( B.pregen && ((B.pregen[widx>>5] >> (widx&31)) & 1) ) return FW_DONE;
	E.mao = 0; E.k = 0; E.kmask = 0; E.npre = E.nlast = E.nn = E.nmfirst = E.nmlast = 0; E.n0 = E.npool = E.nlinks = E.nwF = E.nwR = 0; E.nF = E.nL = 0;
	E.nsiq = E.ncdh = E.nacc = 0; E.rstop = 0; E.roundT0 = 0; E.cfree = 0; E.pvpath = E.pvrp = E.pvnf = 0; E.pvcl = 0; E.nmid = 0; E.midbase = 0; E.nLmagic = 0;
	E.T = B.T; E.P = B.P; E.nrows = FB.F.nrows; E.nsup = FB.F.nsup; E.vst = FB.dpsq_vst;
	E.gslab = 0; E.gtab = FB.tab32; E.sfresh = true; E.sdirty = false;
	if ( CT::gw )
	{
#if defined(DACC_EMUL)
		E.gslab = FB.gslab;
#else
		E.gslab = FB.gslab + static_cast<uint64_t>(blockIdx.x)*FB.gstride;
#endif
	}
	E.lane = wv_lane(); E.flags = 0; E.prof = B.prof;
#if defined(DACC_LEDGER)
	E.ledger = FB.ledger;
#endif
#if defined(DACC_PROFILE) && !defined(DACC_EMUL)
	uint64_t * const prof = E.prof;
#endif
#if defined(DACC_EMUL)
	g_fstats.clear();
#endif
	E.L.base = lds;
	FastLds<CT> const & L = E.L;
	int const lane = E.lane;
	PROF_T0
	int32_t curff = B.P.maxff;
	uint32_t hslot = 0;
	bool const handable = FB.hand != 0 && B.P.klow == B.P.khigh && CT::gw != 0;
	if ( resume && B.P.klow == B.P.khigh )
	{
		WindowOut const prev = B.wout[widx];
		if ( prev.status == WS_RETRY && prev.filterfreq <= B.P.maxff && prev.filterfreq >= B.P.minff )
		{
			curff = prev.filterfreq;
			if ( handable && prev.minrate <= FB.handcap ) hslot = static_cast<uint32_t>(prev.minrate);
		}
	}
	int32_t const startff = curff;
	#define FFAIL(code) { if ( lane == 0 ) { B.wout[widx].status = WS_RETRY; B.wout[widx].flags = ((code)<<24) | (E.flags & 0xFFFFFF); B.wout[widx].filterfreq = curff; B.wout[widx].minrate = hslot; } return ((code) == 1 || (code) == 4) ? FW_GENERIC : FW_NEXT; }

	uint32_t lo = 0, hi = B.npiles;
	while ( hi-lo > 1 ) { uint32_t const mid = (lo+hi)>>1; if ( B.piles[mid].winbase <= widx ) lo = mid; else hi = mid; }
	DevPile const pile = B.piles[lo];
	uint32_t const y = static_cast<uint32_t>(widx - pile.winbase);
	uint32_t astart, aend;
	windowInterval(pile.l,B.P.a,B.P.w,y,astart,aend);

	WindowOut out; out.status = WS_INSUFFICIENT; out.mao = 0; out.elength = 0; out.k = 0; out.filterfreq = -1; out.conslen = 0; out.minrate = 0; out.flags = 0;
	uint8_t * rec = B.wrec + widx*(CT::wide ? DACC_WREC_OF(B.P.w) : static_cast<uint32_t>(WREC));
	if ( lane == 0 ) rec[0] = 0;
	if ( B.P.w > (CT::wide ? 127u : 63u) ) { FFAIL(1) }

	DevOvl const * ov = B.ovl + pile.first_ovl;
	uint32_t nact = 0, mao = 0, toolong = 0;
	LEDGER_REPX(E,0)
	{
	nact = 0;
	for ( uint32_t c = 0; c < pile.novl; c += WSZ )
	{
		uint32_t const z = c + lane;
		uint32_t act = 0;
		if ( z < pile.novl ) act = (ov[z].abpos <= static_cast<int32_t>(astart)) && (ov[z].aepos >= static_cast<int32_t>(aend));
		uint32_t tot; uint32_t const pre = wv_scan_excl(act,tot);
		if ( act && nact+pre < CT::precap ) L.pre()[nact+pre] = (static_cast<uint64_t>(ov[z].ekey)<<32) | z;
		nact += tot;
	}
	if ( nact > CT::precap || next_pow2(nact < 2 ? 2 : nact) > CT::precap ) { FFAIL(2) }
	uint32_t const ap2 = next_pow2(nact < 2 ? 2 : nact);
	for ( uint32_t i = nact + lane; i < ap2; i += WSZ ) L.pre()[i] = ~0ull;
	wv_sync();
	wv_sort_keys<CT::precap>(L.pre(),nact);
	mao = 0;
	if ( nact )
	{
		uint64_t const nb = (B.P.maxalign > 0) ? (B.P.maxalign-1) : 0;
		mao = 1 + static_cast<uint32_t>(nact < nb ? nact : nb);
	}
	if ( mao > CT::maxs ) { FFAIL(3) }
	if constexpr ( CT::mins != 0 ) { if ( mao <= CT::mins ) { FFAIL(3) } }
	E.mao = mao; out.mao = mao;

	toolong = 0;
	if ( mao )
	{
		for ( uint32_t j = lane; j < mao; j += WSZ )
		{
			uint32_t bs, len, rl; uint64_t off; bool inv;
			if ( j == 0 ) { bs = astart; len = B.P.w; off = B.boff[pile.aread]; rl = B.rlen[pile.aread]; inv = false; }
			else
			{
				uint32_t const z = static_cast<uint32_t>(L.pre()[j-1] & 0xFFFFFFFFu);
				DevOvl const & o = ov[z];
				uint64_t const row = o.wtoff + (y - o.y0);
				bs = B.wt_b[row]; len = B.wt_e[row]-bs;
				off = B.boff[o.bread]; rl = B.rlen[o.bread]; inv = o.flags & 1;
			}
			if ( len > CT::lstr ) { toolong = 1; len = 0; }
			L.slen()[j] = len;
			L.mfirst()[j] = bs | (static_cast<uint64_t>(rl)<<32);
			L.mlast()[j] = off | (static_cast<uint64_t>(inv ? 1 : 0)<<63);
		}
		toolong = wv_any(toolong);
		wv_sync();
		for ( uint32_t j0 = 0; j0 < mao; j0 += 4 )
			for ( uint32_t p = lane; p < CT::lstr; p += WSZ )
			{
				uint8_t v0 = 0, v1 = 0, v2 = 0, v3 = 0;
				bool const a0 = p < L.slen()[j0], a1 = j0+1 < mao && p < L.slen()[j0+1], a2 = j0+2 < mao && p < L.slen()[j0+2], a3 = j0+3 < mao && p < L.slen()[j0+3];
				#define DACC_LB(u) { uint64_t const d0 = L.mfirst()[j0+u], d1 = L.mlast()[j0+u]; v##u = readBase(B.bps,d1 & 0x7FFFFFFFFFFFFFFFull,static_cast<uint32_t>(d0>>32),(d1>>63) != 0,static_cast<uint32_t>(d0)+p); }
				if ( a0 ) DACC_LB(0)
				if ( a1 ) DACC_LB(1)
				if ( a2 ) DACC_LB(2)
				if ( a3 ) DACC_LB(3)
				#undef DACC_LB
				if constexpr ( CT::gw != 0 )
				{
					enum { PW = FastLds<CT>::pw };
					uint32_t const sh0 = p - static_cast<uint32_t>(lane);
					uint32_t const wq = sh0 >> 6, sh = sh0 & 63u;
					#define DACC_PM(u) if ( j0+u < mao ) { \
						uint64_t const b0 = wv_ballot(a##u && v##u == 0) << sh, b1 = wv_ballot(a##u && v##u == 1) << sh, b2 = wv_ballot(a##u && v##u == 2) << sh, b3 = wv_ballot(a##u && v##u == 3) << sh; \
						if ( lane == 0 ) { LDSQ uint64_t * const q = L.peq() + 4*PW*(j0+u) + wq; if ( sh == 0 ) { q[0] = b0; q[PW] = b1; q[2*PW] = b2; q[3*PW] = b3; } else { q[0] |= b0; q[PW] |= b1; q[2*PW] |= b2; q[3*PW] |= b3; } } }
					DACC_PM(0) DACC_PM(1) DACC_PM(2) DACC_PM(3)
					#undef DACC_PM
				}
				else
				{
				if ( a0 ) L.str()[(j0+0)*CT::lstr+p] = v0;
				if ( a1 ) L.str()[(j0+1)*CT::lstr+p] = v1;
				if ( a2 ) L.str()[(j0+2)*CT::lstr+p] = v2;
				if ( a3 ) L.str()[(j0+3)*CT::lstr+p] = v3;
				}
			}
	}
	wv_sync();
	}
	if ( toolong ) { FFAIL(4) }
	PROF(E,0)

	int32_t elength = 0;
	if ( mao )
	{
		E.buildPeq();
		LEDGER_REPX(E,1) elength = E.estimateLength()+1;
	}
	out.elength = elength;
	PROF(E,1)

	if ( mao >= B.P.minwindowcov )
	{
		bool pathfailed = true;
		uint64_t minrate = B.P.eminrate;
		bool haveMin = false;
		uint32_t bestlen = 0;
		LDSQ uint8_t * best = L.bestL();
		for ( uint32_t k = B.P.klow; k <= B.P.khigh; ++k )
		{
			E.k = k; E.kmask = (1ull<<(2*k))-1;
			bool instvalid = false, instsaved = false, handloaded = false;
			for ( int32_t ff = startff; ff >= B.P.minff; --ff )
			{
				curff = ff;
				PROF_T0
				if ( !instvalid )
				{
					SITE_T0
					if ( instsaved ) { E.restoreInstances(); SITE(27) }
					else if ( !(hslot && !handloaded && E.loadHand(FB,hslot)) ) { LEDGER_REPX(E,2) E.buildInstances(); SITE(28) }
					else { SITE(30) }
					handloaded = true;
				}
				if ( E.flags ) { FFAIL(7) }
				PROF(E,2)
				LEDGER_REPX(E,3) E.buildNodes(ff > 1 ? ff : 1);
				E.flags = wv_or(E.flags);
				if ( E.flags ) { if ( handable ) hslot = E.saveHand(FB,hslot); FFAIL(7) }
				PROF(E,3)
				instvalid = false;
				{ bool dead_ = false; LEDGER_REPX(E,16) dead_ = (ff != 0 && E.passIsDead()); if ( dead_ ) { instvalid = true; continue; } }
				if ( CT::gw != 0 && ff > B.P.minff && !instsaved ) { SITE_T0 LEDGER_REPX(E,17) E.saveInstances(); instsaved = true; SITE(29) }
				LEDGER_REPX(E,4) E.buildSuccessors(mao);
				PROF(E,4)
				if ( ff == 0 )
				{
					E.loadTab();
					E.levelSuccessors2();
					E.flags = wv_or(E.flags);
					if ( E.flags ) { FFAIL(6) }
					E.buildNodes(1);
					E.flags = wv_or(E.flags);
					if ( E.flags ) { FFAIL(7) }
					E.buildSuccessors(mao);
					PROF(E,6)
				}
				E.flags = wv_or(E.flags);
				if ( E.flags ) { FFAIL(7) }
				uint32_t mintry = 0; bool lconsok = false;
				while ( true )
				{
					bool const consok = E.traverse(static_cast<int64_t>(elength)-4,static_cast<int64_t>(elength)+4);
					E.flags = wv_or(E.flags);
					if ( E.flags ) { FFAIL(8) }
					if ( consok )
					{
						uint64_t const err = L.accerr()[0];
						if ( err < minrate )
						{
							lconsok = true; minrate = err; haveMin = true;
							bestlen = L.acc()[0].l;
							if ( bestlen > ((CT::wide && B.P.w > 64u) ? FastLds<CT>::consmax : static_cast<uint32_t>(MAXCONS)) ) { FFAIL(9) }
							for ( uint32_t i = lane; i < bestlen; i += WSZ ) best[i] = L.consL()[L.acc()[0].o+i];
							out.k = k; out.filterfreq = ff;
							wv_sync();
						}
						else if ( haveMin ) lconsok = true;
						break;
					}
					else
					{
						if ( ++mintry >= 3 ) break;
					}
					if ( !E.addNextFromHeap() ) break;
				}
				if ( lconsok ) { pathfailed = false; break; }
			}
		}
		if ( !pathfailed )
		{
			out.status = WS_OK; out.conslen = bestlen; out.minrate = minrate;
			PROF_T0
			uint32_t nops = 0;
			LEDGER_REPX(E,15)
			{
			nops = 0;
			wv_sync();
			if ( lane == 0 ) nops = E.alignAndEmit(best,bestlen);
			wv_sync();
			nops = wv_bcast(nops,0);
			E.emitRecord(best,nops,rec);
			}
			PROF(E,14)
		}
		else out.status = WS_FAILED;
	}
	if ( lane == 0 ) B.wout[widx] = out;
	wv_sync();
#if defined(DACC_EMUL)
	fstats_dump(static_cast<int>(CT::maxs));
#endif
	return FW_DONE;
	#undef FFAIL
}

#if defined(DACC_EMUL)
#undef over
#endif
}
#endif
```

### include/daccord_hip.h

```cpp
#ifndef DACCORD_HIP_H
#define DACCORD_HIP_H

#include <stdint.h>
#include <stddef.h>

#ifdef __cplusplus
extern "C" {
#endif

#define DACC_OK          0
#define DACC_EINVAL     -1
#define DACC_ENODEV     -2
#define DACC_ENOMEM     -3
#define DACC_ESTATE     -4
#define DACC_EHIP       -5
#define DACC_ENOTSUP    -6
#define DACC_EINTERNAL  -7

typedef struct dacc_params {
	uint32_t w;
	uint32_t a;
	uint32_t klow, khigh;
	int32_t  minfilterfreq;
	int32_t  maxfilterfreq;
	uint32_t minwindowcov;
	uint64_t maxalign;
	uint64_t eminrate;
	uint64_t minlen;
	int32_t  producefull;
	int32_t  tspace;
	int32_t  device;
	int32_t  verbose;
} dacc_params;

typedef struct dacc_overlap {
	int32_t  aread, bread;
	uint32_t flags;
	int32_t  abpos, aepos, bbpos, bepos;
	int32_t  diffs;
	int32_t  tlen;
	uint32_t reserved;
	uint64_t trace_off;
} dacc_overlap;

typedef struct dacc_pile {
	int32_t  aread;
	uint32_t novl;
	uint64_t first_ovl;
} dacc_pile;

typedef struct dacc_fragment {
	int32_t  aread;
	uint32_t first, last;
	uint32_t len;
	uint64_t seq_off;
} dacc_fragment;

typedef struct dacc_ctx dacc_ctx;

int  dacc_device_count(void);
int  dacc_create(dacc_ctx **ctx, const dacc_params *params);
void dacc_destroy(dacc_ctx *ctx);

int  dacc_set_error_profile(dacc_ctx *ctx, double p_i, double p_d, double est_cor);

int  dacc_load_db(dacc_ctx *ctx, const uint8_t *bps, uint64_t bps_bytes,
                  const uint64_t *boff, const uint32_t *rlen, uint64_t nreads);

int  dacc_submit_piles(dacc_ctx *ctx,
                       const dacc_pile *piles, uint64_t npiles,
                       const dacc_overlap *ovl, uint64_t novl,
                       const void *trace, uint64_t ntrace, int trace_bytes);

int  dacc_collect(dacc_ctx *ctx, const dacc_fragment **frags, uint64_t *nfrags,
                  const char **bases, uint64_t *nbases);
void dacc_release(dacc_ctx *ctx);

const char *dacc_last_error(dacc_ctx *ctx);

int  dacc_pile_select(const dacc_overlap *in, uint64_t n, int trace_bytes, uint64_t maxinput,
                      dacc_overlap *out, uint64_t *nout);


int  dacc_pile_select_lowest(const dacc_overlap *in, uint64_t n, int trace_bytes, uint64_t maxinput,
                             dacc_overlap *out, uint64_t *nout);

typedef struct dacc_eprof dacc_eprof;
int  dacc_eprof_create(dacc_eprof **e, int32_t tspace, const uint8_t *bps, const uint64_t *boff, const uint32_t *rlen,
                       uint64_t nreads, int two_databases);
int  dacc_eprof_add(dacc_eprof *e, const dacc_pile *piles, uint64_t npiles, const dacc_overlap *ovl, uint64_t novl,
                    const void *trace, uint64_t ntrace, int trace_bytes, uint64_t maxalign, int nthreads);
int  dacc_eprof_finish(dacc_eprof *e, uint64_t counts[4], uint64_t *usable, uint64_t *unusable,
                       double *eavg, double *edif, double prof[3]);
void dacc_eprof_destroy(dacc_eprof *e);
int  dacc_eprof_skipped(dacc_eprof *e, uint64_t *skipped, uint64_t *seen);
int  dacc_eprof_set_deep(dacc_eprof *e, int on);
int  dacc_eprof_deep(dacc_eprof *e, const uint32_t **values, uint64_t *n);


typedef struct dacc_timing {
	float h2d_ms;
	float trace_ms;
	float window_ms;
	float vote_ms;
	float d2h_ms;
	float total_ms;
	uint64_t nwindows;
	uint64_t nblocks;
	uint64_t algo_bytes;
	float tier_ms[3];
	uint32_t tier_out[3];
	uint32_t first_tier;
	uint32_t long_windows;
	float tier0_ms;
	uint32_t tier0_in;
	uint32_t tier0_out;
	float tier7_ms;
	uint32_t tier7_in;
	uint32_t tier7_out;
	uint32_t pad_;
	uint32_t long_first_tier;
	float tier10_ms;
	uint32_t tier10_out;
	uint32_t tier10_ran;
	uint32_t pad2_;
	float deep_ms;
	uint32_t deep_windows;
	uint32_t deep_out;
	uint32_t pad3_;
	float last_ms;
	uint32_t last_windows;
	uint32_t last_out;
	uint32_t pad4_;
	float vdeep_ms;
	uint32_t vdeep_windows;
	uint32_t vdeep_out;
	uint32_t pad5_;
} dacc_timing;
#define DACC_TIMING_SIZE_V1 128
int  dacc_last_timing(dacc_ctx *ctx, dacc_timing *t);
int  dacc_last_timing2(dacc_ctx *ctx, dacc_timing *t, size_t size);

int  dacc_pile_status(dacc_ctx *ctx, int32_t *status, uint64_t cap, uint64_t *n);
const char *dacc_pile_errors(dacc_ctx *ctx);

int  dacc_plan_only(const dacc_params *par, const uint32_t *rlen, uint64_t nreads, const dacc_pile *piles, uint64_t npiles,
                    const dacc_overlap *ovl, uint64_t novl, const void *trace, uint64_t ntrace, int trace_bytes,
                    uint64_t *nwindows, uint64_t *nblocks);

int  dacc_rerun_resident(dacc_ctx *ctx);

typedef struct dacc_window_result {
	int32_t  pile;
	int32_t  y;
	int32_t  status;
	int32_t  mao;
	int32_t  elength;
	int32_t  k;
	int32_t  filterfreq;
	int32_t  conslen;
	uint64_t minrate;
	char     cons[80];
} dacc_window_result;
int  dacc_debug_windows(dacc_ctx *ctx, dacc_window_result *out, uint64_t cap, uint64_t *nwin);

int  dacc_debug_tables(dacc_ctx *ctx, uint64_t *out, uint64_t cap, uint64_t *n, uint64_t klimit_n);

int  dacc_debug_profile(dacc_ctx *ctx, uint64_t *out32);
int  dacc_debug_profile_fine(dacc_ctx *ctx, uint64_t *out96);

int  dacc_debug_retry(dacc_ctx *ctx, uint32_t *out, uint64_t cap, uint64_t *n);

#ifdef __cplusplus
}
#endif
#endif
```

Before: 38.30 Mbase/s.

## Defer consensus-to-A alignment from tier kernels into a separate per-window emit kernel

The serial single-lane Myers alignment and traceback of consensus against the A window used to run inside the tier window kernels while the other wave lanes waited. The tier kernels now store a pending record (the four match masks plus the consensus), and a new k_emit kernel with one thread per window does the alignment and writes the final record before the vote. This frees wave time and LDS in the tier kernels. In exchange it adds a kernel launch, more per-thread stack/register use for the DP arrays, and an extra global-memory pass over the window records. It also adds timing instrumentation for the new kernel.

```diff
diff --git a/daccord_amd/_structs.py b/daccord_amd/_structs.py
--- a/daccord_amd/_structs.py
+++ b/daccord_amd/_structs.py
@@ -38,7 +38,8 @@
                 ("long_first_tier", C.c_uint32), ("tier10_ms", C.c_float), ("tier10_out", C.c_uint32), ("tier10_ran", C.c_uint32), ("pad2_", C.c_uint32),
                 ("deep_ms", C.c_float), ("deep_windows", C.c_uint32), ("deep_out", C.c_uint32), ("pad3_", C.c_uint32),
                 ("last_ms", C.c_float), ("last_windows", C.c_uint32), ("last_out", C.c_uint32), ("pad4_", C.c_uint32),
-                ("vdeep_ms", C.c_float), ("vdeep_windows", C.c_uint32), ("vdeep_out", C.c_uint32), ("pad5_", C.c_uint32)]
+                ("vdeep_ms", C.c_float), ("vdeep_windows", C.c_uint32), ("vdeep_out", C.c_uint32),
+                ("emit_ms", C.c_float)]
 
 
 TIMING_SIZE_V1 = 128
diff --git a/daccord_amd/csrc/capi.hip b/daccord_amd/csrc/capi.hip
--- a/daccord_amd/csrc/capi.hip
+++ b/daccord_amd/csrc/capi.hip
@@ -11,6 +11,7 @@
 #include "window_kernels.hpp"
 #include "trace_kernel.hpp"
 #include "vote_kernel.hpp"
+#include "emit_record.hpp"
 
 using namespace dacc;
 
@@ -123,6 +124,13 @@
 		while ( hi-lo > 1 ) { uint32_t const mid = (lo+hi)>>1; if ( piles[mid].winbase <= i ) lo = mid; else hi = mid; }
 		pilebad[lo] = 1;
 	}
+}
+
+__global__ void __launch_bounds__(256) k_emit(uint8_t * wrec, uint64_t n, uint32_t w)
+{
+	uint64_t const i = static_cast<uint64_t>(blockIdx.x)*256 + threadIdx.x;
+	if ( i >= n || w == 0 || DACC_WIDE_W(w) ) return;
+	emitPendingRecord(wrec + i*WREC,w);
 }
 
 __global__ void k_count_deeper(uint32_t const * in, uint32_t const * handon, WindowOut const * wout, uint32_t const mins, uint32_t * out)
@@ -330,7 +338,7 @@
 	dacc_params par;
 	int device;
 	hipStream_t stream; hipStream_t stream2; hipEvent_t evFirstTier, evEarlyGeneric, evPrescan;
-	hipEvent_t ev[6]; hipEvent_t evslot[TIER_NSLOTS];
+	hipEvent_t ev[6]; hipEvent_t evEmit[2]; hipEvent_t evslot[TIER_NSLOTS];
 	std::string err;
 	bool haveprofile, havedb, havebatch;
 	double est_cor;
@@ -415,6 +423,7 @@
 	{ int lo = 0, hi = 0; hipDeviceGetStreamPriorityRange(&lo,&hi); if ( hipStreamCreateWithPriority(&c->stream2,hipStreamNonBlocking,hi) != hipSuccess ) { delete c; return DACC_EHIP; } }
 	hipEventCreateWithFlags(&c->evFirstTier,hipEventDisableTiming); hipEventCreateWithFlags(&c->evEarlyGeneric,hipEventDisableTiming); hipEventCreateWithFlags(&c->evPrescan,hipEventDisableTiming);
 	for ( int i = 0; i < 6; ++i ) hipEventCreate(&c->ev[i]);
+	for ( int i = 0; i < 2; ++i ) hipEventCreate(&c->evEmit[i]);
 	for ( int i = 0; i < TIER_NSLOTS; ++i ) hipEventCreate(&c->evslot[i]);
 	for ( int i = 0; i < TIER_NSTAGES; ++i ) { hipEventCreate(&c->st[i].done); c->st[i].ran = false; c->st[i].grid = 0; c->st[i].in = 0; }
 	*out = c;
@@ -432,6 +441,7 @@
 	c->d_wrec.release(); c->d_wout.release(); c->d_arena.release();
 	c->h_outsym.release(); c->d_pilebad.release(); c->d_has.release(); c->d_oc.release(); c->d_outsym.release(); c->d_ld0.release(); c->d_ocs.release(); c->d_nfrag.release(); c->d_err.release(); c->d_frags.release(); c->d_fragbase.release(); c->d_prof.release(); c->d_vst.release(); c->d_tab32.release(); c->d_gslab.release(); c->d_lastslab.release(); c->d_vdeepslab.release(); for ( int i = 0; i < 3; ++i ) c->d_retry[i].release(); c->d_work.release(); c->d_gearly.release(); c->d_pregen.release(); c->d_pregen2.release(); c->d_pregenlist.release(); c->d_arena2.release(); c->d_trslab.release(); c->d_hand.release(); c->d_handctr.release();
 	for ( int i = 0; i < 6; ++i ) hipEventDestroy(c->ev[i]);
+	for ( int i = 0; i < 2; ++i ) hipEventDestroy(c->evEmit[i]);
 	hipStreamDestroy(c->stream); hipStreamDestroy(c->stream2); hipEventDestroy(c->evFirstTier); hipEventDestroy(c->evEarlyGeneric); hipEventDestroy(c->evPrescan); for ( int i = 0; i < TIER_NSLOTS; ++i ) hipEventDestroy(c->evslot[i]);
 	c->d_small.release(); for ( int i = 0; i < TIER_NSTAGES; ++i ) { hipEventDestroy(c->st[i].done); c->st[i].handon.release(); }
 	delete c;
@@ -678,6 +688,9 @@
 	auto voteAndFetch = [&]() -> int
 	{
 		HIPCHK(hipMemsetAsync(c->d_pilebad.p,0,BP.piles.size()+1,s));
+		HIPCHK(hipEventRecord(c->evEmit[0],s));
+		if ( BP.nwindows ) { hipLaunchKernelGGL(k_emit,dim3((BP.nwindows+255)/256),dim3(256),0,s,c->d_wrec.p,static_cast<uint64_t>(BP.nwindows),c->par.w); mark("k_emit"); }
+		HIPCHK(hipEventRecord(c->evEmit[1],s));
 		if ( BP.nwindows ) hipLaunchKernelGGL(k_check_done,dim3((BP.nwindows+255)/256),dim3(256),0,s,c->d_wout.p,BP.nwindows,c->d_err.p+3,c->d_piles.p,static_cast<uint32_t>(BP.piles.size()),c->d_pilebad.p);
 		if ( BP.piles.size() )
 		{
@@ -766,7 +779,7 @@
 		HIPCHK(hipMemcpy(&nin,fZ->in,sizeof(uint32_t),hipMemcpyDeviceToHost)); HIPCHK(hipMemcpy(&nout,fZ->handon.p,sizeof(uint32_t),hipMemcpyDeviceToHost));
 		c->timing.last_out = nout; c->timing.last_windows = nin > nout ? nin - nout : 0u;
 	}
-	c->timing.vdeep_windows = 0; c->timing.vdeep_out = 0; c->timing.pad5_ = 0;
+	c->timing.vdeep_windows = 0; c->timing.vdeep_out = 0;
 	if ( dacc_ctx::Stage const * const fV = ranOf(ID_VDEEP) )
 	{
 		HIPCHK(hipMemsetAsync(c->d_work.p+WORK_VDEEP_COUNT,0,2*sizeof(uint32_t),s));
@@ -827,6 +840,7 @@
 	if ( dacc_ctx::Stage const * const fV = ranOf(ID_VDEEP) ) { dacc_ctx::Stage const * const fZ = ranOf(ID_LAST); hipEventElapsedTime(&ms,fZ ? fZ->done : c->evslot[TIER_NSLOTS-1],fV->done); c->timing.vdeep_ms = ms; }
 	if ( fX ) { hipEventElapsedTime(&ms,fD ? fD->done : c->evslot[1],fX->done); c->timing.deep_ms = ms; }
 	hipEventElapsedTime(&ms,c->ev[2],c->ev[3]); c->timing.vote_ms = ms;
+	hipEventElapsedTime(&ms,c->evEmit[0],c->evEmit[1]); c->timing.emit_ms = ms;
 	hipEventElapsedTime(&ms,c->ev[3],c->ev[4]); c->timing.d2h_ms = ms;
 	hipEventElapsedTime(&ms,c->ev[0],c->ev[3]); c->timing.total_ms = ms;
 	c->timing.first_tier = (TP.usefast && BP.deep) ? 4u : 1u;
@@ -980,6 +994,7 @@
 
 static_assert(offsetof(dacc_timing,deep_ms) == DACC_TIMING_SIZE_V1,"dacc_last_timing fills the record in front of deep_ms");
 static_assert(offsetof(dacc_timing,vdeep_ms) == 160 && sizeof(dacc_timing) == 176,"the very deep stage's fields are appended behind last_*");
+static_assert(offsetof(dacc_timing,emit_ms) == 172,"emit_ms is the last word of the record, where the very deep stage's pad word was");
 int dacc_last_timing(dacc_ctx * c, dacc_timing * t)
 {
 	if ( !c || !t ) return DACC_EINVAL;
@@ -1056,7 +1071,7 @@
 			dacc_window_result r; std::memset(&r,0,sizeof(r));
 			r.pile = pi; r.y = y; r.status = o.status; r.mao = o.mao; r.elength = o.elength; r.k = o.k;
 			r.filterfreq = (o.status == WS_OK) ? o.filterfreq : 0; r.conslen = o.conslen; r.minrate = o.minrate;
-			if ( o.status == WS_OK )
+			if ( o.status == WS_OK && wrec[wdx*wrecb] == WREC_FINAL )
 			{
 				uint8_t const * rec = wrec.data() + wdx*wrecb;
 				uint32_t const w = c->P.w; bool const wide = DACC_WIDE_W(w);
diff --git a/daccord_amd/csrc/daccord_hip_main.cpp b/daccord_amd/csrc/daccord_hip_main.cpp
--- a/daccord_amd/csrc/daccord_hip_main.cpp
+++ b/daccord_amd/csrc/daccord_hip_main.cpp
@@ -488,7 +488,7 @@
 	});
 	std::string fatal; bool stopall = false;
 	double gpu_s = 0; uint64_t nbatches = 0;
-	struct { uint64_t nwindows, tier_out[3], deep_windows, deep_out, last_windows, last_out, vdeep_windows, vdeep_out; double window_ms, tier_ms[3], deep_ms, last_ms, vdeep_ms; } tstat = {};
+	struct { uint64_t nwindows, tier_out[3], deep_windows, deep_out, last_windows, last_out, vdeep_windows, vdeep_out; double window_ms, tier_ms[3], deep_ms, last_ms, vdeep_ms, emit_ms; } tstat = {};
 	auto const deviceWorker = [&](int const g)
 	{
 		dacc_ctx * const ctx = ctxs[g];
@@ -531,7 +531,7 @@
 						{
 							tstat.nwindows += tm.nwindows; tstat.window_ms += tm.window_ms; tstat.deep_ms += tm.deep_ms; tstat.deep_windows += tm.deep_windows; tstat.deep_out += tm.deep_out;
 							tstat.last_ms += tm.last_ms; tstat.last_windows += tm.last_windows; tstat.last_out += tm.last_out;
-							tstat.vdeep_ms += tm.vdeep_ms; tstat.vdeep_windows += tm.vdeep_windows; tstat.vdeep_out += tm.vdeep_out;
+							tstat.vdeep_ms += tm.vdeep_ms; tstat.vdeep_windows += tm.vdeep_windows; tstat.vdeep_out += tm.vdeep_out; tstat.emit_ms += tm.emit_ms;
 							for ( int i = 0; i < 3; ++i ) { tstat.tier_out[i] += tm.tier_out[i]; tstat.tier_ms[i] += tm.tier_ms[i]; }
 						}
 					}
@@ -565,12 +565,13 @@
 		std::fprintf(stderr,"[V] %llu windows, window kernels %.1f ms: tier slots %.1f / %.1f / %.1f ms handed on %llu / %llu / %llu windows (the last to the last stage); "
 			"deep-window tier (97 ... 250 strings) %.1f ms, %llu windows finished, %llu handed on; "
 			"last stage (layout in device memory) %.1f ms, %llu windows finished, %llu handed on; "
-			"very deep stage (251 ... 1000 strings) %.1f ms, %llu windows finished, %llu handed on to the generic engine\n",
+			"very deep stage (251 ... 1000 strings) %.1f ms, %llu windows finished, %llu handed on to the generic engine; "
+			"consensus -> A alignment of the tiers' windows (k_emit, in front of the vote) %.1f ms\n",
 			static_cast<unsigned long long>(tstat.nwindows),tstat.window_ms,tstat.tier_ms[0],tstat.tier_ms[1],tstat.tier_ms[2],
 			static_cast<unsigned long long>(tstat.tier_out[0]),static_cast<unsigned long long>(tstat.tier_out[1]),static_cast<unsigned long long>(tstat.tier_out[2]),
 			tstat.deep_ms,static_cast<unsigned long long>(tstat.deep_windows),static_cast<unsigned long long>(tstat.deep_out),
 			tstat.last_ms,static_cast<unsigned long long>(tstat.last_windows),static_cast<unsigned long long>(tstat.last_out),
-			tstat.vdeep_ms,static_cast<unsigned long long>(tstat.vdeep_windows),static_cast<unsigned long long>(tstat.vdeep_out));
+			tstat.vdeep_ms,static_cast<unsigned long long>(tstat.vdeep_windows),static_cast<unsigned long long>(tstat.vdeep_out),tstat.emit_ms);
 	}
 	for ( int g = 0; g < nwork; ++g ) dacc_destroy(ctxs[g]);
 	dacc_las_close(las); dacc_db_close(A.h); if ( twodb ) dacc_db_close(B2.h);
diff --git a/daccord_amd/csrc/dev_types.hpp b/daccord_amd/csrc/dev_types.hpp
--- a/daccord_amd/csrc/dev_types.hpp
+++ b/daccord_amd/csrc/dev_types.hpp
@@ -78,6 +78,8 @@
 enum { LSTRMAX = 4096 };
 enum { WREC = 256 };
 enum { MAXCONS = 96 };
+enum { WREC_FINAL = 1, WREC_PENDING = 2 };
+enum { PEND_LEN = 1, PEND_PEQ = 8, PEND_CONS = 40 };
 enum { WRECW = 640 };
 enum { MAXCONSW = 224 };
 #define DACC_WIDE_W(w_) ((w_) > 64u)
diff --git a/daccord_amd/csrc/emit_record.hpp b/daccord_amd/csrc/emit_record.hpp
--- /dev/null
+++ b/daccord_amd/csrc/emit_record.hpp
@@ -0,0 +1,109 @@
+#ifndef DACC_EMIT_RECORD_HPP
+#define DACC_EMIT_RECORD_HPP
+#include <stdint.h>
+#include "dev_types.hpp"
+
+#if defined(__HIPCC__) && !defined(DACC_EMUL)
+#define DACC_EMIT_FN __host__ __device__ inline
+#else
+#define DACC_EMIT_FN inline
+#endif
+
+namespace dacc {
+
+DACC_EMIT_FN uint64_t emitEq(uint32_t const ch, uint64_t const e0, uint64_t const e1, uint64_t const e2, uint64_t const e3)
+{
+	return (ch & 2) ? ((ch & 1) ? e3 : e2) : ((ch & 1) ? e1 : e0);
+}
+DACC_EMIT_FN uint64_t emitPack8(uint64_t p)
+{
+	p &= 0x0303030303030303ull;
+	p = (p | (p>>6)) & 0x000F000F000F000Full;
+	p = (p | (p>>12)) & 0x000000FF000000FFull;
+	return (p | (p>>24)) & 0xFFFFull;
+}
+
+DACC_EMIT_FN void emitPendingRecord(uint8_t * const rec, uint32_t const m)
+{
+	if ( rec[0] != WREC_PENDING ) return;
+	uint64_t const * const R8 = reinterpret_cast<uint64_t const *>(rec);
+	uint32_t n = rec[PEND_LEN]; if ( n > MAXCONS ) n = MAXCONS;
+	uint64_t const e0 = R8[PEND_PEQ/8], e1 = R8[PEND_PEQ/8+1], e2 = R8[PEND_PEQ/8+2], e3 = R8[PEND_PEQ/8+3];
+	static_assert(MAXCONS == 96 && (PEND_PEQ & 7) == 0 && (PEND_CONS & 7) == 0 && PEND_CONS + MAXCONS <= WREC,"consensus packed into three 64 bit words");
+	uint64_t ck[3] = {0,0,0};
+	for ( uint32_t q = 0; q < MAXCONS/8; ++q )
+		if ( 8*q < n ) ck[q>>2] |= emitPack8(R8[PEND_CONS/8+q]) << (16*(q&3));
+	uint64_t const ck0 = ck[0], ck1 = ck[1], ck2 = ck[2];
+	#define DACC_EMIT_SYM(c_) (static_cast<uint32_t>(((c_) < 32 ? ck0 : ((c_) < 64 ? ck1 : ck2)) >> (2*((c_)&31))) & 3u)
+
+	uint64_t pvc[MAXCONS+1], mvc[MAXCONS+1]; uint8_t botc[MAXCONS+1];
+	uint64_t const mask = (m == 64) ? ~0ull : ((1ull<<m)-1);
+	uint64_t const top = 1ull<<(m-1);
+	uint64_t Pv = mask, Mv = 0; uint32_t score = m;
+	pvc[0] = Pv; mvc[0] = Mv; botc[0] = static_cast<uint8_t>(m);
+	for ( uint32_t c = 0; c < n; ++c )
+	{
+		uint64_t const Eq = emitEq(DACC_EMIT_SYM(c),e0,e1,e2,e3);
+		uint64_t const Xv = Eq | Mv;
+		uint64_t const Xh = (((Eq & Pv) + Pv) ^ Pv) | Eq;
+		uint64_t Ph = Mv | ~(Xh | Pv);
+		uint64_t Mh = Pv & Xh;
+		if ( Ph & top ) ++score; else if ( Mh & top ) --score;
+		Ph = (Ph<<1) | 1ull; Mh <<= 1;
+		Pv = (Mh | ~(Xv | Ph)) & mask;
+		Mv = (Ph & Xv) & mask;
+		pvc[c+1] = Pv; mvc[c+1] = Mv; botc[c+1] = static_cast<uint8_t>(score);
+	}
+
+	uint8_t ops[64+MAXCONS];
+	uint32_t i = m, j = n, d = score, nops = 0;
+	uint64_t pvj = Pv, pv1 = 0, mv1 = 0; uint32_t bot1 = 0;
+	if ( j ) { pv1 = pvc[j-1]; mv1 = mvc[j-1]; bot1 = botc[j-1]; }
+	while ( i || j )
+	{
+		uint32_t op = 2; bool done = false, left = false;
+		if ( i && j )
+		{
+			uint32_t const sh = i-1;
+			uint32_t const dd = bot1 - static_cast<uint32_t>(__builtin_popcountll(pv1>>sh)) + static_cast<uint32_t>(__builtin_popcountll(mv1>>sh));
+			uint32_t const neq = ((emitEq(DACC_EMIT_SYM(j-1),e0,e1,e2,e3) >> sh) & 1ull) ? 0u : 1u;
+			if ( dd + neq == d ) { op = neq; --i; --j; d = dd; done = true; left = true; }
+		}
+		if ( !done && i )
+		{
+			if ( (pvj >> (i-1)) & 1ull ) { op = 3; --i; d = d-1; done = true; }
+		}
+		if ( !done ) { op = 2; --j; d = d-1; left = true; }
+		if ( left )
+		{
+			pvj = pv1;
+			if ( j ) { pv1 = pvc[j-1]; mv1 = mvc[j-1]; bot1 = botc[j-1]; }
+		}
+		ops[nops++] = static_cast<uint8_t>(op);
+	}
+
+	uint64_t outw[WREC/8];
+	uint8_t * const out = reinterpret_cast<uint8_t *>(outw);
+	uint8_t * const off = out+1; uint8_t * const sym = out + 1 + (m+2);
+	out[0] = WREC_FINAL;
+	uint32_t so = 0, cpos = 0, t = nops;
+	for ( uint32_t r = 0; r <= m; ++r )
+	{
+		off[r] = static_cast<uint8_t>(so);
+		while ( t && ops[t-1] == 2 ) { sym[so++] = static_cast<uint8_t>(DACC_EMIT_SYM(cpos)); ++cpos; --t; }
+		if ( r < m )
+		{
+			uint32_t const op = ops[--t];
+			if ( op == 3 ) sym[so++] = 4; else { sym[so++] = static_cast<uint8_t>(DACC_EMIT_SYM(cpos)); ++cpos; }
+		}
+	}
+	off[m+1] = static_cast<uint8_t>(so);
+	#undef DACC_EMIT_SYM
+	uint32_t const nbytes = 1 + (m+2) + so;
+	static_assert(1 + 66 + 64 + MAXCONS <= WREC,"a final record fits its slot");
+	uint64_t * const W8 = reinterpret_cast<uint64_t *>(rec);
+	for ( uint32_t q = 0; 8*q < nbytes; ++q ) W8[q] = outw[q];
+}
+
+}
+#endif
diff --git a/daccord_amd/csrc/fast_window.hpp b/daccord_amd/csrc/fast_window.hpp
--- a/daccord_amd/csrc/fast_window.hpp
+++ b/daccord_amd/csrc/fast_window.hpp
@@ -5,6 +5,7 @@
 #include "arena.hpp"
 #include "window_main.hpp"
 #include "tier_pipeline.hpp"
+#include "emit_record.hpp"
 
 namespace dacc {
 
@@ -3437,122 +3438,39 @@
 		}
 		else return 0;
 	}
-	DEV uint32_t alignAndEmit(LDSQ uint8_t const * cons, uint32_t const n)
-	{
-		if constexpr ( CT::wide != 0 ) { if ( DACC_WIDE_W(P.w) ) return alignAndEmitWide(cons,n); }
-		uint32_t const m = P.w;
-		LDSQ uint64_t const * PEQ = L.peq();
+	DEV void emitRecordWide(LDSQ uint8_t const * cons, uint32_t const nops, uint8_t * rec)
+	{
+		if constexpr ( CT::wide != 0 )
+		{
+			uint32_t const m = P.w;
+			uint8_t * const off = rec+2; uint8_t * const sym = rec + 2 + 2*(m+2);
+			if ( lane == 0 ) { rec[0] = WREC_FINAL; rec[1] = 0; off[0] = 0; off[1] = 0; off[2*(m+1)] = nops & 0xFFu; off[2*(m+1)+1] = nops >> 8; }
+			uint32_t cbase = 0, abase = 0;
+			for ( uint32_t c0 = 0; c0 < nops; c0 += WSZ )
+			{
+				uint32_t const q = c0 + lane;
+				bool const act = q < nops;
+				uint32_t const op = act ? L.alops()[nops-1-q] : 2u;
+				uint32_t ctot, atot;
+				uint32_t const cpos = cbase + wv_scan_flag(act && op != 3,ctot);
+				uint32_t const arank = abase + wv_scan_flag(act && op != 2,atot);
+				if ( act )
+				{
+					sym[q] = (op == 3) ? 4 : cons[cpos];
+					if ( op != 2 ) { off[2*(arank+1)] = (q+1) & 0xFFu; off[2*(arank+1)+1] = (q+1) >> 8; }
+				}
+				cbase += ctot; abase += atot;
+			}
+		}
+	}
+	DEV void storePending(LDSQ uint8_t const * cons, uint32_t const n, uint8_t * rec)
+	{
 		enum { PW = FastLds<CT>::pw };
-		uint64_t const e0 = PEQ[0*PW], e1 = PEQ[1*PW], e2 = PEQ[2*PW], e3 = PEQ[3*PW];
+		static_assert(MAXCONS <= 96 && (FastLds<CT>::o_bestL & 7) == 0 && PEND_PEQ == 8 && PEND_CONS == 40,"one 64 bit word per lane: header, four masks, twelve words of consensus");
 		LDSQ uint64_t const * T8 = reinterpret_cast<LDSQ uint64_t const *>(cons);
-		static_assert(MAXCONS <= 96 && (FastLds<CT>::o_bestL & 7) == 0,"consensus packed into three 64 bit words");
-		uint64_t const mask = (m == 64) ? ~0ull : ((1ull<<m)-1);
-		uint64_t Pv = mask, Mv = 0; uint32_t score = m;
-		L.alpv()[0] = Pv; L.almv()[0] = Mv; L.albot()[0] = m;
-		uint64_t const top = 1ull<<(m-1);
-		uint64_t ck0 = 0, ck1 = 0, ck2 = 0;
-		uint64_t w = n ? T8[0] : 0ull;
-		for ( uint32_t c0 = 0; c0 < n; c0 += 8 )
-		{
-			uint64_t const wn = (c0+8 < n) ? T8[(c0>>3)+1] : 0ull;
-			uint32_t const cnt = (n-c0 < 8) ? (n-c0) : 8u;
-			for ( uint32_t u = 0; u < cnt; ++u )
-			{
-				uint32_t const c = c0+u;
-				uint64_t const ch = (w >> (8*u)) & 3u;
-				uint64_t const cs = ch << (2*(c&31));
-				ck0 |= c < 32 ? cs : 0ull; ck1 |= (c >= 32 && c < 64) ? cs : 0ull; ck2 |= c >= 64 ? cs : 0ull;
-				uint64_t const Eq = (ch & 2) ? ((ch & 1) ? e3 : e2) : ((ch & 1) ? e1 : e0);
-				uint64_t const Xv = Eq | Mv;
-				uint64_t const Xh = (((Eq & Pv) + Pv) ^ Pv) | Eq;
-				uint64_t Ph = Mv | ~(Xh | Pv);
-				uint64_t Mh = Pv & Xh;
-				if ( Ph & top ) ++score; else if ( Mh & top ) --score;
-				Ph = (Ph<<1) | 1ull; Mh <<= 1;
-				Pv = (Mh | ~(Xv | Ph)) & mask;
-				Mv = (Ph & Xv) & mask;
-				L.alpv()[c+1] = Pv; L.almv()[c+1] = Mv; L.albot()[c+1] = score;
-			}
-			w = wn;
-		}
-		uint32_t i = m, j = n; uint32_t d = score; uint32_t nops = 0;
-		uint64_t pvj = Pv, pv1 = 0, mv1 = 0; uint32_t bot1 = 0;
-		if ( j ) { pv1 = L.alpv()[j-1]; mv1 = L.almv()[j-1]; bot1 = L.albot()[j-1]; }
-		while ( i || j )
-		{
-			uint32_t op = 2; bool done = false; bool left = false;
-			if ( i && j )
-			{
-				uint64_t const sh = i-1;
-				uint32_t const dd = bot1 - dacc_popc64(pv1>>sh) + dacc_popc64(mv1>>sh);
-				uint32_t const jj = j-1;
-				uint64_t const ckw = jj < 32 ? ck0 : (jj < 64 ? ck1 : ck2);
-				uint32_t const ch = static_cast<uint32_t>(ckw >> (2*(jj&31))) & 3u;
-				uint64_t const Eq = (ch & 2) ? ((ch & 1) ? e3 : e2) : ((ch & 1) ? e1 : e0);
-				uint32_t const neq = ((Eq >> sh) & 1) ? 0u : 1u;
-				if ( dd + neq == d ) { op = neq ? 1 : 0; --i; --j; d = dd; done = true; left = true; }
-			}
-			if ( !done && i )
-			{
-				uint64_t const bit = 1ull<<(i-1);
-				if ( pvj & bit ) { op = 3; --i; d = d-1; done = true; }
-			}
-			if ( !done ) { op = 2; --j; d = d-1; left = true; }
-			if ( left )
-			{
-				pvj = pv1;
-				if ( j ) { pv1 = L.alpv()[j-1]; mv1 = L.almv()[j-1]; bot1 = L.albot()[j-1]; }
-			}
-			L.alops()[nops++] = op;
-		}
-		return nops;
-	}
-	DEV void emitRecord(LDSQ uint8_t const * cons, uint32_t const nops, uint8_t * rec)
-	{
-		uint32_t const m = P.w;
-		if constexpr ( CT::wide != 0 )
-		{
-			if ( DACC_WIDE_W(m) )
-			{
-				uint8_t * const off = rec+2; uint8_t * const sym = rec + 2 + 2*(m+2);
-				if ( lane == 0 ) { rec[0] = 1; rec[1] = 0; off[0] = 0; off[1] = 0; off[2*(m+1)] = nops & 0xFFu; off[2*(m+1)+1] = nops >> 8; }
-				uint32_t cbase = 0, abase = 0;
-				for ( uint32_t c0 = 0; c0 < nops; c0 += WSZ )
-				{
-					uint32_t const q = c0 + lane;
-					bool const act = q < nops;
-					uint32_t const op = act ? L.alops()[nops-1-q] : 2u;
-					uint32_t ctot, atot;
-					uint32_t const cpos = cbase + wv_scan_flag(act && op != 3,ctot);
-					uint32_t const arank = abase + wv_scan_flag(act && op != 2,atot);
-					if ( act )
-					{
-						sym[q] = (op == 3) ? 4 : cons[cpos];
-						if ( op != 2 ) { off[2*(arank+1)] = (q+1) & 0xFFu; off[2*(arank+1)+1] = (q+1) >> 8; }
-					}
-					cbase += ctot; abase += atot;
-				}
-				return;
-			}
-		}
-		uint8_t * off = rec+1; uint8_t * sym = rec + 1 + (m+2);
-		if ( lane == 0 ) { rec[0] = 1; off[0] = 0; off[m+1] = nops; }
-		uint32_t cbase = 0, abase = 0;
-		for ( uint32_t c0 = 0; c0 < nops; c0 += WSZ )
-		{
-			uint32_t const q = c0 + lane;
-			bool const act = q < nops;
-			uint32_t const op = act ? L.alops()[nops-1-q] : 2u;
-			uint32_t ctot, atot;
-			uint32_t const cpos = cbase + wv_scan_flag(act && op != 3,ctot);
-			uint32_t const arank = abase + wv_scan_flag(act && op != 2,atot);
-			if ( act )
-			{
-				sym[q] = (op == 3) ? 4 : cons[cpos];
-				if ( op != 2 ) off[arank+1] = q+1;
-			}
-			cbase += ctot; abase += atot;
-		}
+		uint64_t * const R8 = reinterpret_cast<uint64_t *>(rec);
+		for ( uint32_t q = lane; q < PEND_CONS/8 + (n+7)/8; q += WSZ )
+			R8[q] = (q == 0) ? (static_cast<uint64_t>(WREC_PENDING) | (static_cast<uint64_t>(n) << (8*PEND_LEN))) : ((q < PEND_CONS/8) ? L.peq()[(q-1)*PW] : T8[q-PEND_CONS/8]);
 	}
 };
 
@@ -3822,15 +3740,28 @@
 		{
 			out.status = WS_OK; out.conslen = bestlen; out.minrate = minrate;
 			PROF_T0
-			uint32_t nops = 0;
 			LEDGER_REPX(E,15)
 			{
-			nops = 0;
-			wv_sync();
-			if ( lane == 0 ) nops = E.alignAndEmit(best,bestlen);
-			wv_sync();
-			nops = wv_bcast(nops,0);
-			E.emitRecord(best,nops,rec);
+			bool wide = false;
+			if constexpr ( CT::wide != 0 ) wide = DACC_WIDE_W(B.P.w);
+			if ( wide )
+			{
+				uint32_t nops = 0;
+				wv_sync();
+				if ( lane == 0 ) nops = E.alignAndEmitWide(best,bestlen);
+				wv_sync();
+				nops = wv_bcast(nops,0);
+				E.emitRecordWide(best,nops,rec);
+			}
+			else
+			{
+				E.storePending(best,bestlen,rec);
+#if defined(DACC_EMUL)
+				wv_sync();
+				if ( lane == 0 ) emitPendingRecord(rec,B.P.w);
+				wv_sync();
+#endif
+			}
 			}
 			PROF(E,14)
 		}
diff --git a/include/daccord_hip.h b/include/daccord_hip.h
--- a/include/daccord_hip.h
+++ b/include/daccord_hip.h
@@ -135,7 +135,7 @@
 	float vdeep_ms;
 	uint32_t vdeep_windows;
 	uint32_t vdeep_out;
-	uint32_t pad5_;
+	float emit_ms;
 } dacc_timing;
 #define DACC_TIMING_SIZE_V1 128
 int  dacc_last_timing(dacc_ctx *ctx, dacc_timing *t);
```

Result: faster. 39.58 Mbase/s, median of 6 (+3.3%).
